# Nuralamsiddik16/Ultrafnd_git

Hardware: AMD Instinct MI355X
Metric: train-step samples/sec (FakeSV batch, seq128+224^2) (higher is better)
Workload: dtype bf16

## Files before the change

### include/ultrafnd_hip.h

```cpp
#ifndef ULTRAFND_HIP_H
#define ULTRAFND_HIP_H

#include <stddef.h>
#include <stdint.h>

#ifdef __cplusplus
extern "C" {
#endif

#define UFND_OK 0
#define UFND_ERR_INVALID 1
#define UFND_ERR_LAUNCH 2

#define UFND_ABI_VERSION 6

const char* ufnd_last_error(void);
int ufnd_abi_version(void);

typedef struct ufnd_step_state {
  uint64_t step;
  uint64_t seed;
  float lr;
  float weight_decay;
  float beta1, beta2, eps;
  float max_norm;
  float grad_scale;
  float loss;
  float grad_norm;
  float clip_coef;
  float bc1, bc2_sqrt;
  uint32_t micro;
  float reserved[2];
} ufnd_step_state;

typedef struct ufnd_dims {
  int hidden;
  int text_dim;
  int audio_dim;
  int visual_dim;
  int temporal_dim;
  int gnn_dim;
  int aux_dim;
  int trees;
  int depth;
  int classes;
  float fusion_dropout;
  float clf_dropout;
  float node_dropout;
} ufnd_dims;

typedef struct ufnd_fusion_params {
  float *text_w, *text_b;
  float *audio_w, *audio_b;
  float *visual_w, *visual_b;
  float *temporal_w, *temporal_b;
  float *gnn_w, *gnn_b;
  float *qkv_w, *qkv_b;
  float *ev0_w[3], *ev0_b[3];
  float *ev2_w[3], *ev2_b[3];
  float *fuse0_w, *fuse0_b;
  float *fuse3_w, *fuse3_b;
  float *cls_w, *cls_b;
} ufnd_fusion_params;

typedef struct ufnd_clf_params {
  float *pre0_w, *pre0_b;
  float *pre3_w, *pre3_b;
  float *gates, *thresh;
  float *leaf, *tau;
  float *bypass_w, *bypass_b;
  float *temperature;
} ufnd_clf_params;

size_t ufnd_fusion_workspace_floats(const ufnd_dims* d, int B);
size_t ufnd_clf_workspace_floats(const ufnd_dims* d, int B);

int ufnd_fusion_forward(const ufnd_dims* d, const ufnd_fusion_params* p, const float* text, const float* audio,
                        const float* visual, const float* temporal, const float* gnn, int B, int train,
                        float* workspace, float* fused, int ld_fused, float* logits, float* forensic,
                        const ufnd_step_state* state, void* stream);

int ufnd_fusion_backward(const ufnd_dims* d, const ufnd_fusion_params* p, const ufnd_fusion_params* g,
                         const float* text, const float* audio, const float* visual, const float* temporal,
                         const float* gnn, int B, int train, float* workspace, const float* d_fused,
                         int ld_dfused, const float* d_logits, const ufnd_step_state* state, void* stream,
                         void* side_stream, int join);

#define UFND_BWD_ALL 0
#define UFND_BWD_FUSE_MLP 1
#define UFND_BWD_REST 2
#define UFND_BWD_NO_LINEAR_GRADS 16
int ufnd_fusion_backward_phase(const ufnd_dims* d, const ufnd_fusion_params* p, const ufnd_fusion_params* g,
                               const float* text, const float* audio, const float* visual, const float* temporal,
                               const float* gnn, int B, int train, float* workspace, const float* d_fused,
                               int ld_dfused, const float* d_logits, const ufnd_step_state* state, void* stream,
                               void* side_stream, int join, int phase);

float* ufnd_clf_input_panel(const ufnd_dims* d, float* clf_workspace, int B, int* ld);
int ufnd_classifier_forward(const ufnd_dims* d, const ufnd_clf_params* p, const float* fused, int ld_fused,
                            const float* aux, int B, int train, float* workspace, float* logits, float* probs,
                            const ufnd_step_state* state, void* stream);
int ufnd_classifier_backward(const ufnd_dims* d, const ufnd_clf_params* p, const ufnd_clf_params* g, int B,
                             int train, float* workspace, const float* d_logits, float* d_fused, int ld_dfused,
                             const ufnd_step_state* state, void* stream, void* side_stream, int join);

int ufnd_classifier_backward_ex(const ufnd_dims* d, const ufnd_clf_params* p, const ufnd_clf_params* g, int B,
                                int train, float* workspace, const float* d_logits, float* d_fused, int ld_dfused,
                                const ufnd_step_state* state, void* stream, void* side_stream, int join, int flags);

size_t ufnd_head_factor_floats(const ufnd_dims* d, int B);
int ufnd_head_pack_factors(const ufnd_dims* d, const float* text, const float* audio, const float* visual, const float* temporal,
                           const float* gnn, int B, float* fusion_workspace, float* clf_workspace, float* pack, void* stream);
int ufnd_head_linear_grads_from_factors(const ufnd_dims* d, const ufnd_fusion_params* fusion_grads, const ufnd_clf_params* clf_grads,
                                        const float* packs, size_t rank_stride, int ranks, int B, void* stream);

typedef struct ufnd_head_io {
  const float *text, *audio, *visual, *temporal, *gnn, *aux;
  const int64_t* labels;
  float *fusion_workspace, *clf_workspace;
  float *logits, *probs, *forensic;
  float* d_logits;
} ufnd_head_io;
int ufnd_head_forward_loss(const ufnd_dims* d, const ufnd_fusion_params* fusion, const ufnd_clf_params* clf, const ufnd_head_io* io, int B,
                           int train, ufnd_step_state* state, void* stream);
int ufnd_head_backward(const ufnd_dims* d, const ufnd_fusion_params* fusion, const ufnd_fusion_params* fusion_grads, const ufnd_clf_params* clf,
                       const ufnd_clf_params* clf_grads, const ufnd_head_io* io, int B, int train, ufnd_step_state* state, void* stream,
                       void* side_stream, int join, int phase);

int ufnd_softmax_ce(const float* logits, const int64_t* labels, int B, float* loss_rows, float* d_logits,
                    ufnd_step_state* state, void* stream);

int ufnd_softmax_ce_weighted(const float* logits, const int64_t* labels, int B, float w0, float w1, float label_smoothing,
                             float* loss_rows, float* d_logits, ufnd_step_state* state, void* stream);

int ufnd_grad_norm(const float* grad, size_t n, float* partials, ufnd_step_state* state, void* stream);
int ufnd_adamw_step(float* param, const float* grad, float* exp_avg, float* exp_avg_sq, size_t n,
                    const ufnd_step_state* state, void* stream);
int ufnd_step_advance(ufnd_step_state* state, void* stream);
int ufnd_clip_adamw_step(float* param, const float* grad, float* exp_avg, float* exp_avg_sq, size_t n, float* partials,
                         ufnd_step_state* state, void* stream);
int ufnd_grad_accumulate(float* dst, const float* src, size_t n, int overwrite, ufnd_step_state* state ,
                         void* stream);

#define UFND_ACT_NONE 0
#define UFND_ACT_GELU 1
#define UFND_ACT_QUICK_GELU 2
#define UFND_ACT_GELU_BWD 3
#define UFND_ACT_QUICK_GELU_BWD 4

int ufnd_cast_bf16(const float* src, void* dst_bf16, size_t n, void* stream);

int ufnd_gemm_bf16(const void* A, const void* W, const float* bias, const float* residual, void* out_bf16,
                   float* out_f32, int M, int N, int K, int lda, int ldw, int ldr, int ldo, int ldf, int act,
                   void* stream);

#define UFND_GEMM_TILE_PERSISTENT 64
int ufnd_gemm_bf16_ex(const void* A, const void* W, const float* bias, const float* residual, void* out_bf16,
                      float* out_f32, int M, int N, int K, int lda, int ldw, int ldr, int ldo, int ldf, int act,
                      int tile_cfg, void* stream);

typedef struct ufnd_gemm_ln {
  const float* a_stats;
  const float* colsum;
  const float* r_stats;
  const float* r_gamma;
  const float* r_beta;
  float* out_stats;
  int a_parts, r_parts;
  float a_eps, r_eps;
  int width;
  int tile_cfg;
  const void* residual_bf16;
  int ldrb;
  float* guard;
} ufnd_gemm_ln;
#define UFND_FOLD_GUARD_SLOTS 1024
int ufnd_gemm_bf16_ln(const void* A, const void* W, const float* bias, const float* residual, void* out_bf16,
                      float* out_f32, int M, int N, int K, int lda, int ldw, int ldr, int ldo, int ldf, int act,
                      const ufnd_gemm_ln* ln, void* stream);
int ufnd_gemm_bf16_stat_parts(int M, int N, int K);

int ufnd_ln_fold_guard(const float* stats, int M, int parts, int width, float eps, float* guard, void* stream);

int ufnd_gemm_bf16_tile_count(void);
int ufnd_gemm_bf16_tile_info(int tile_cfg, int* bm, int* bn, int* ln_aware);

int ufnd_layernorm(const float* x, int ldx, const float* gamma, const float* beta, void* out_bf16, float* out_f32,
                   int M, int H, float eps, void* stream);

int ufnd_attention_bf16(const void* qkv, const int32_t* key_mask, void* ctx, int B, int L, int heads,
                        void* stream);

int ufnd_qkv_attention_bf16(const void* X, const void* Wqkv, const float* bqkv, const int32_t* key_mask, void* ctx, int B, int L,
                            int heads, int ldx, int ldw, const ufnd_gemm_ln* ln, void* stream);

int ufnd_text_pack(const int32_t* mask, int B, int L, int32_t* cu_seqlens, int32_t* row_src, void* stream);
int ufnd_text_pack_bins(const int32_t* mask, int B, int L, int32_t* cu_seqlens, int32_t* row_src, int32_t* bins, int32_t* nbins,
                        void* stream);
int ufnd_bert_embed_live(const int64_t* ids, const int32_t* row_src, const int* m_live, const float* word, const float* pos,
                         const float* type0, const float* gamma, const float* beta, void* x_bf16, float* x_f32, int capacity, int L,
                         int H, int vocab, float eps, void* stream);
int ufnd_gemm_bf16_live(const void* A, const void* W, const float* bias, const float* residual, void* out_bf16, float* out_f32,
                        int M, int N, int K, int lda, int ldw, int ldr, int ldo, int ldf, int act, int tile_cfg, const int* m_live,
                        void* stream);
int ufnd_gemm_bf16_ln_live(const void* A, const void* W, const float* bias, const float* residual, void* out_bf16, float* out_f32,
                           int M, int N, int K, int lda, int ldw, int ldr, int ldo, int ldf, int act, const ufnd_gemm_ln* ln,
                           const int* m_live, void* stream);
int ufnd_qkv_attention_bf16_packed(const void* X, const void* Wqkv, const float* bqkv, const int32_t* key_mask, const int32_t* cu_seqlens,
                                   void* ctx, int B, int L, int heads, int ldx, int ldw, const ufnd_gemm_ln* ln, void* stream);
int ufnd_qkv_attention_bf16_bins(const void* X, const void* Wqkv, const float* bqkv, const int32_t* key_mask, const int32_t* cu_seqlens,
                                 const int32_t* bins, const int32_t* nbins, void* ctx, int B, int L, int heads, int ldx, int ldw,
                                 const ufnd_gemm_ln* ln, void* stream);
int ufnd_attention_bf16_varlen_masked(const void* qkv, const int32_t* cu_seqlens, const int32_t* key_mask, void* ctx, int B, int max_len,
                                      int heads, void* stream);
#define UFND_TEXT_TILE_MAX_B 512
#define UFND_TEXT_TILE_SAMPLES 16
#define UFND_TEXT_TILE_UNITS 24
#define UFND_TEXT_TILE_UNIT0 36
#define UFND_TEXT_TILE_ROWMAP 64
#define UFND_TEXT_TILE_KBIAS 320
#define UFND_TEXT_TILE_INTS 576
int ufnd_text_pack_tiles(const int32_t* mask, int B, int L, int32_t* cu_seqlens, int32_t* row_src, int32_t* tiles, int32_t* ntiles,
                         int32_t* bins, int32_t* nbins, void* stream);
int ufnd_qkv_attention_bf16_tiles(const void* X, const void* Wqkv, const float* bqkv, const int32_t* tiles, const int32_t* ntiles, void* ctx,
                                  int cap_tiles, int heads, int ldx, int ldw, const ufnd_gemm_ln* ln, void* stream);

int ufnd_qkv_attention_bf16_vit(const void* X, const void* Wqkv, const float* bqkv, void* ctx, int N, int T, int heads, int ldx, int ldw,
                                const ufnd_gemm_ln* ln, void* stream);
int ufnd_layernorm_live(const float* x, int ldx, const float* gamma, const float* beta, void* out_bf16, float* out_f32, int capacity,
                        int H, float eps, const int* m_live, void* stream);
int ufnd_masked_meanpool_l2_live(const float* hidden, const int32_t* mask, const int32_t* cu_seqlens, float* out, int B, int L, int H,
                                 void* stream);
int ufnd_ln_masked_meanpool_l2_live(const float* y, const float* gamma, const float* beta, float eps, const int32_t* mask,
                                    const int32_t* cu_seqlens, float* out, int B, int L, int H, void* stream);

int ufnd_bert_embed(const int64_t* ids, const float* word, const float* pos, const float* type0, const float* gamma,
                    const float* beta, void* x_bf16, float* x_f32, int B, int L, int H, int vocab, float eps,
                    void* stream);

int ufnd_masked_meanpool_l2(const float* hidden, const int32_t* mask, float* out, int B, int L, int H,
                            void* stream);

int ufnd_field_mean_l2(const float* parts, const int32_t* valid, float* out, int N, int M, int D, void* stream);

int ufnd_vit_patchify(const float* frames, void* patches_bf16, int N, int image, int patch, void* stream);

int ufnd_vit_assemble(const float* patch_emb, const float* cls, const float* pos, const float* gamma,
                      const float* beta, float* x_f32, void* x_bf16, float* stats, int N, int P, int H, float eps,
                      void* stream);

int ufnd_l2norm_frames(const float* e, float* out, int B, int F, int D, void* stream);

#define UFND_GATHER_MAX_ITEMS 8
typedef struct ufnd_gather_item {
  const void* src;
  void* dst;
  int row_bytes;
  int64_t src_rows;
} ufnd_gather_item;
int ufnd_gather_rows(const int64_t* idx, int B, const ufnd_gather_item* items, int n_items, void* stream);

int ufnd_temporal_weight_ld(int in_dim);
size_t ufnd_temporal_workspace_floats(int B, int in_dim, int hidden);
int ufnd_temporal_align(const float* text, const float* visual, const float* w0, const float* b0, const float* w3,
                        const float* b3, float* workspace, float* out, int B, int in_dim, int vis_dim, int hidden,
                        int out_dim, float dropout_p, const ufnd_step_state* state, void* stream);

typedef struct ufnd_tcn_layer {
  const float *w, *b;
  const float *gamma, *beta;
  float *running_mean, *running_var;
} ufnd_tcn_layer;
int ufnd_tcn_weight_ld(int in_ch, int kernel);
size_t ufnd_tcn_workspace_floats(int B, int T, int in_ch, int hid, int kernel);
int ufnd_tcn_forward(const float* text_seq, int text_dim, const float* vis_seq, int vis_dim, int B, int T,
                     const ufnd_tcn_layer* layers, int n_layers, int kernel, int hid, const float* head_w,
                     const float* head_b, int out_dim, int train, float dropout_p, float momentum, float eps,
                     const ufnd_step_state* state, float* workspace, float* out, void* stream);


int ufnd_ocr_adjacency(const int32_t* offsets, const int32_t* tokens, int N, double thresh, float* adj, int ld, void* stream);

typedef struct ufnd_gcn_params {
  const float* w1;
  const float* b1;
  const float* w2;
  const float* b2;
} ufnd_gcn_params;

size_t ufnd_gcn_workspace_floats(int N, int in_dim, int hid, int out_dim, int train);

int ufnd_gcn_forward(const float* x, const float* adj, int ld_adj, const ufnd_gcn_params* p, float* z, float* workspace, int N,
                     int in_dim, int hid, int out_dim, float dropout_p, const ufnd_step_state* state, void* stream);

int ufnd_gcn_pretrain_step(const float* x, const float* adj, int ld_adj, const ufnd_gcn_params* p, float* exp_avg,
                           float* exp_avg_sq, const float* head_w, const float* head_b, float* z, float* workspace, int N,
                           int in_dim, int hid, int out_dim, float dropout_p, float lr, float weight_decay, int step,
                           const ufnd_step_state* state, float* loss, void* stream);


size_t ufnd_cosine_knn_workspace_floats(int N, int D, int k);

int ufnd_cosine_knn(const float* X, int ldx, int N, int D, int k, int32_t* idx, float* workspace, void* stream);

#define UFND_ADJ_KNN 1
#define UFND_ADJ_OCR 2
#define UFND_ADJ_TEMPORAL 4
int ufnd_dense_adj(const int32_t* idx, int k, const int32_t* offsets, const int32_t* tokens, const float* delay, double alpha,
                   double beta, int N, float* adj, int ld, int flags, void* stream);


int ufnd_ocr_adjacency_weighted(const int32_t* offsets, const int32_t* tokens, int N, double thresh, float* adj, int ld, void* stream);

int ufnd_node_features(const float* text, int ld_text, const float* audio, int ld_audio, const float* visual, int ld_visual,
                       const float* temporal, int ld_temporal, int n_text, int n_audio, int n_visual, int n_temporal, int B,
                       float* out, void* stream);

size_t ufnd_gnn_workspace_floats(int N, int in_dim, int hid, int out_dim);
int ufnd_gnn_forward(const float* x, const float* adj, int ld_adj, const ufnd_gcn_params* p, float* z, float* workspace, int N,
                     int in_dim, int hid, int out_dim, float dropout_p, const ufnd_step_state* state, void* stream);
int ufnd_gnn_backward(const float* x, const ufnd_gcn_params* p, float* g_w1, float* g_b1, float* g_w2, float* g_b2, const float* d_z,
                      float* workspace, int N, int in_dim, int hid, int out_dim, float dropout_p, const ufnd_step_state* state,
                      void* stream);
int ufnd_fusion_feature_grads(const ufnd_dims* d, const ufnd_fusion_params* p, float* workspace, int B, float* d_text, float* d_visual,
                              const ufnd_step_state* state, void* stream);

int ufnd_fusion_gnn_input_grad(const ufnd_dims* d, const ufnd_fusion_params* p, float* workspace, int B, float* d_gnn,
                               const ufnd_step_state* state, void* stream);

int ufnd_fusion_input_grads(const ufnd_dims* d, const ufnd_fusion_params* p, float* workspace, int B, float* d_text, float* d_audio,
                            float* d_visual, float* d_temporal, float* d_gnn, const ufnd_step_state* state, void* stream);

#define UFND_TARGET_LOGIT 0
#define UFND_TARGET_PROB 1
int ufnd_classifier_input_grad(const ufnd_dims* d, const ufnd_clf_params* p, const float* fused, int ld_fused, const float* aux,
                               int B, int train, int target, int class_idx, float* workspace, float* d_x, int ld_dx,
                               float* logits, float* probs, const ufnd_step_state* state, void* stream);

int ufnd_smoothgrad_points(const ufnd_dims* d, const float* x0, int ld_x0, const float* sigma, const float* noise, int ld_noise,
                           int B, int N, int step0, int steps, float* workspace, void* stream);

#define UFND_ATTR_SMOOTHGRAD 0
#define UFND_ATTR_GRAD_X_INPUT 1
#define UFND_ATTR_PATH_MEAN 3
int ufnd_attribution_reduce(int mode, const float* G, int ldg, const float* X, int ldx, int B, int W, int steps, int accumulate,
                            int divisor, float* out, int ldo, float* agg, float* partials, void* stream);

int ufnd_stream_create_cu_mask(const uint32_t* mask_words, int n_words, void** stream_out);
int ufnd_stream_destroy(void* stream);
int ufnd_device_cu_count(void);


int ufnd_gemm_bf16_dgrad(const void* dY, const void* Wt, const float* residual, const void* aux, void* out_bf16, float* out_f32,
                         int M, int N, int K, int lda, int ldw, int ldr, int ldaux, int ldo, int ldf, int act, void* stream);

size_t ufnd_gemm_bf16_wgrad_workspace_floats(int n_out, int k_in, int tokens);
int ufnd_gemm_bf16_wgrad(const void* dYt, const void* Xt, float* dW, int n_out, int k_in, int tokens, int lda, int ldb, int ldw,
                         float* workspace, int accumulate, void* stream);

typedef struct ufnd_partials_job {
  const float* part;
  int nblk, H;
  float *out0, *out1;
} ufnd_partials_job;
#define UFND_PARTIALS_DEFER 2

#define UFND_WGRAD_ALL 0
#define UFND_WGRAD_TRANSPOSE 1
#define UFND_WGRAD_PRODUCT 2
int ufnd_linear_wgrad(const void* dY, int lddy, const void* X, int ldx, int M, int N, int K, float* dW, float* db, void* dYt, void* Xt, int ldt,
                      float* slab_workspace, float* colsum_workspace, const ufnd_partials_job* extra, int part, void* stream);

typedef struct ufnd_refresh_item {
  const void* master;
  void* w;
  void* wt;
  int rows, cols, ld_master, ld_w, ld_wt, tile0;
} ufnd_refresh_item;
int ufnd_refresh_operands(const ufnd_refresh_item* items_device, int n_items, int total_tiles, void* stream);

size_t ufnd_transpose_colsum_workspace_floats(int rows_pad, int cols);
int ufnd_transpose_bf16(const void* src, int src_is_f32, int rows, int cols, int lds, void* dst, int ldd, int rows_pad, float* colsum,
                        float* colsum_ws, int colsum_accumulate, void* stream);

int ufnd_attention_bf16_lse(const void* qkv, const int32_t* key_mask, void* ctx, float* lse, int B, int L, int heads, void* stream);
size_t ufnd_attention_bwd_workspace_floats(int B, int L, int heads);
int ufnd_attention_bf16_bwd(const void* qkv, const void* ctx, const void* dctx, const float* lse, const int32_t* key_mask, void* dqkv,
                            float* workspace, int B, int L, int heads, void* stream);

size_t ufnd_layernorm_bwd_workspace_floats(int M, int H);
int ufnd_layernorm_bwd_blocks(int M);
int ufnd_row_partials_finish(const ufnd_partials_job* job, int accumulate, void* stream);
int ufnd_layernorm_bwd(const float* x, int ldx, const float* gamma, const float* dy, int lddy, const float* add, int ldadd, float* dx_f32,
                       void* dx_bf16, int lddx, float* dgamma, float* dbeta, float* workspace, int accumulate, int M, int H, float eps,
                       void* stream);

int ufnd_act_bf16(const void* x, void* out, size_t n, int act, void* stream);

int ufnd_masked_meanpool_l2_bwd(const float* hidden, const int32_t* mask, const float* dfeat, float* dhidden, int B, int L, int H, void* stream);
int ufnd_l2norm_frames_bwd(const float* e, const float* dfeat, float* de, int B, int F, int D, void* stream);
int ufnd_bert_embed_bwd(const int64_t* ids, const float* ds, float* dword, float* dpos, float* dtype, int B, int L, int H, int vocab,
                        int max_pos, int type_vocab, void* stream);
int ufnd_vit_assemble_bwd(const float* ds, float* dcls, float* dpos, void* dpe_bf16, int N, int P, int H, void* stream);

typedef struct ufnd_dropout {
  const ufnd_step_state* state;
  float p;
  uint32_t tag;
} ufnd_dropout;

#define UFND_LN_BWD_DROP_DXB 1
#define UFND_LN_BWD_DROP_DY 2

int ufnd_attention_bf16_lse_dropout(const void* qkv, const int32_t* key_mask, void* ctx, float* lse, int B, int L, int heads,
                                    const ufnd_dropout* drop, void* stream);
int ufnd_attention_bf16_bwd_dropout(const void* qkv, const void* ctx, const void* dctx, const float* lse, const int32_t* key_mask,
                                    void* dqkv, float* workspace, int B, int L, int heads, const ufnd_dropout* drop, void* stream);
int ufnd_dropout_residual_layernorm(const float* x, int ldx, const float* d, int ldd, const float* gamma, const float* beta, float* y,
                                    void* out_bf16, float* out_f32, int M, int H, float eps, const ufnd_dropout* drop, void* stream);
int ufnd_layernorm_dropout(const float* x, int ldx, const float* gamma, const float* beta, void* out_bf16, float* out_f32, int M, int H,
                           float eps, const ufnd_dropout* drop, void* stream);
int ufnd_layernorm_bwd_dropout(const float* x, int ldx, const float* gamma, const float* dy, int lddy, const float* add, int ldadd,
                               float* dx_f32, void* dx_bf16, int lddx, float* dgamma, float* dbeta, float* workspace, int accumulate,
                               int M, int H, float eps, const ufnd_dropout* drop, int where, void* stream);


#define UFND_PATH_MAX_POINTS 64
int ufnd_path_points(const float* x, const float* base, const float* alphas, int n_points, size_t rows, int width, float* out,
                     void* stream);

int ufnd_token_attribution(const float* g, int ldg, const float* s, int lds, const float* base, int ldb, const int32_t* mask, int R, int H,
                           float* score, float* grad_norm, void* stream);

int ufnd_vit_unpatchify_attribution(const float* dpatches, const float* x, const float* base, float* grad, float* pixels, float* patch_sums,
                                    int N, int image, int patch, void* stream);

#define UFND_AUDIO_MIN_SAMPLES 400
#define UFND_WAVE_CHUNK 4096
#define UFND_CONV0_CHUNK 256

int ufnd_wave_normalize(const float* wave, const int32_t* lengths, float* out, float* ws, int B, int n_max, void* stream);

int ufnd_w2v2_conv0(const float* wave, const int32_t* lengths, const float* w, const float* gamma, const float* beta, void* out_bf16,
                    float* out_f32, float* ws, int B, int n_max, int S1, float eps, void* stream);

int ufnd_conv1d_rows_bf16(const void* A, const void* W, const float* bias, void* out_bf16, float* out_f32, int M, int N, int K, int lda,
                          int ldw, int ldo, int ldf, int act, void* stream);

int ufnd_w2v2_pos_pack(const void* x_bf16, const int32_t* frames, void* packed, int B, int S, void* stream);
int ufnd_w2v2_pos_add(const float* x, const float* conv, const int32_t* frames, float* y, int B, int S, void* stream);

int ufnd_w2v2_frames(const int32_t* lengths, int32_t* frames, int32_t* key_mask, int B, int S, void* stream);

int ufnd_masked_meanpool(const float* hidden, const int32_t* mask, float* out, int B, int L, int H, void* stream);

int ufnd_linear_f32(const float* X, const float* W, const float* bias, float* Y, int M, int N, int K, void* stream);

int ufnd_attention_bf16_causal(const void* qkv, const int32_t* key_mask, void* ctx, int B, int L, int heads, void* stream);
int ufnd_attention_bf16_causal_varlen(const void* qkv, const int32_t* cu_seqlens, const int32_t* key_mask, void* ctx, int B, int max_len,
                                      int heads, void* stream);
int ufnd_clip_text_pack(const int64_t* ids, int B, int L, int eos_token_id, int32_t* e, int32_t* cu_seqlens, int32_t* row_src, void* stream);
int ufnd_clip_text_embed(const int64_t* ids, const float* token_embedding, const float* position_embedding, void* x_bf16, float* x_f32, int B,
                         int L, int H, int vocab, int max_position, void* stream);
int ufnd_clip_text_embed_live(const int64_t* ids, const int32_t* row_src, const int* m_live, const float* token_embedding,
                              const float* position_embedding, void* x_bf16, float* x_f32, int capacity, int L, int H, int vocab,
                              int max_position, void* stream);
int ufnd_clip_text_pool(const float* x, const int32_t* e, const int32_t* cu_seqlens, const float* gamma, const float* beta, void* out_bf16, int B,
                        int L, int H, float eps, void* stream);

int ufnd_semantic_head(const float* text, const float* image, const float* wt, const float* bt, const float* wi, const float* bi,
                       float* workspace, float* out_text, float* out_image, float* out_gap, int B, int D, int K, void* stream);

int ufnd_clip_similarity(const float* text, const float* image, float* similarity, float* conflict, int B, int D, void* stream);

int ufnd_roberta_pack(const int64_t* ids, const int32_t* mask, int B, int L, int pad_token_id, int32_t* cu_seqlens, int32_t* row_src,
                      int32_t* pos_ids, int32_t* valid, void* stream);
int ufnd_roberta_embed(const int64_t* ids, const int32_t* pos_ids, const float* word, const float* pos, const float* type0, const float* gamma,
                       const float* beta, void* x_bf16, float* x_f32, int B, int L, int H, int vocab, int max_position, int pad_token_id, float eps,
                       void* stream);
int ufnd_roberta_embed_live(const int64_t* ids, const int32_t* pos_ids, const int32_t* row_src, const int* m_live, const float* word, const float* pos,
                            const float* type0, const float* gamma, const float* beta, void* x_bf16, float* x_f32, int capacity, int L, int H,
                            int vocab, int max_position, int pad_token_id, float eps, void* stream);
int ufnd_gather_class_rows(const int32_t* cu_seqlens, const void* ctx, void* ctx_out, const void* res_bf16, void* res_bf16_out, const float* res_f32,
                           float* res_f32_out, const float* stats, float* stats_out, int B, int L, int H, int stat_floats, int capacity, void* stream);
int ufnd_emotion_head(const float* x, const float* wd, const float* bd, const float* wo, const float* bo, const int32_t* group,
                      const int32_t* text_valid, const float* arousal, float* workspace, float* logits, float* class_probs, float* probs,
                      float* text_intensity, float* intensity, float* valence, int B, int H, int C, void* stream);
int ufnd_audio_arousal(const float* waves, const int32_t* lengths, float* arousal, int B, int T, void* stream);

#ifdef __cplusplus
}
#endif
#endif
```

### ultrafnd_git_amd/_lib.py

```python
from __future__ import annotations

import ctypes as C
from pathlib import Path
from typing import Optional

import torch

_PKG = Path(__file__).resolve().parent
LIB_PATH = _PKG / "libultrafnd_hip.so"


class UltrafndHipError(RuntimeError):
    pass


class StepState(C.Structure):
    _fields_ = [("step", C.c_uint64), ("seed", C.c_uint64), ("lr", C.c_float), ("weight_decay", C.c_float),
                ("beta1", C.c_float), ("beta2", C.c_float), ("eps", C.c_float), ("max_norm", C.c_float),
                ("grad_scale", C.c_float), ("loss", C.c_float), ("grad_norm", C.c_float), ("clip_coef", C.c_float),
                ("bc1", C.c_float), ("bc2_sqrt", C.c_float), ("micro", C.c_uint32), ("reserved", C.c_float * 2)]


class Dims(C.Structure):
    _fields_ = [("hidden", C.c_int), ("text_dim", C.c_int), ("audio_dim", C.c_int), ("visual_dim", C.c_int),
                ("temporal_dim", C.c_int), ("gnn_dim", C.c_int), ("aux_dim", C.c_int), ("trees", C.c_int),
                ("depth", C.c_int), ("classes", C.c_int), ("fusion_dropout", C.c_float), ("clf_dropout", C.c_float),
                ("node_dropout", C.c_float)]


_FP = C.c_void_p


class FusionParams(C.Structure):
    _fields_ = [(n, _FP) for n in ("text_w", "text_b", "audio_w", "audio_b", "visual_w", "visual_b", "temporal_w",
                                   "temporal_b", "gnn_w", "gnn_b", "qkv_w", "qkv_b")] + \
               [("ev0_w", _FP * 3), ("ev0_b", _FP * 3), ("ev2_w", _FP * 3), ("ev2_b", _FP * 3)] + \
               [(n, _FP) for n in ("fuse0_w", "fuse0_b", "fuse3_w", "fuse3_b", "cls_w", "cls_b")]


class ClfParams(C.Structure):
    _fields_ = [(n, _FP) for n in ("pre0_w", "pre0_b", "pre3_w", "pre3_b", "gates", "thresh", "leaf", "tau",
                                   "bypass_w", "bypass_b", "temperature")]


class GcnParams(C.Structure):
    _fields_ = [(n, _FP) for n in ("w1", "b1", "w2", "b2")]


class GatherItem(C.Structure):
    _fields_ = [("src", _FP), ("dst", _FP), ("row_bytes", C.c_int), ("src_rows", C.c_int64)]


class TcnLayer(C.Structure):
    _fields_ = [(n, _FP) for n in ("w", "b", "gamma", "beta", "running_mean", "running_var")]


class HeadIO(C.Structure):
    _fields_ = [(n, C.c_void_p) for n in ("text", "audio", "visual", "temporal", "gnn", "aux", "labels", "fusion_workspace", "clf_workspace",
                                           "logits", "probs", "forensic", "d_logits")]


class PartialsJob(C.Structure):
    _fields_ = [("part", C.c_void_p), ("nblk", C.c_int), ("H", C.c_int), ("out0", C.c_void_p), ("out1", C.c_void_p)]


class RefreshItem(C.Structure):
    _fields_ = [("master", C.c_void_p), ("w", C.c_void_p), ("wt", C.c_void_p), ("rows", C.c_int), ("cols", C.c_int), ("ld_master", C.c_int),
                ("ld_w", C.c_int), ("ld_wt", C.c_int), ("tile0", C.c_int)]


class Dropout(C.Structure):
    _fields_ = [("state", C.c_void_p), ("p", C.c_float), ("tag", C.c_uint32)]


PARTIALS_DEFER = 2
LN_BWD_DROP_DXB, LN_BWD_DROP_DY = 1, 2
WGRAD_ALL, WGRAD_TRANSPOSE, WGRAD_PRODUCT = 0, 1, 2


class GemmLn(C.Structure):
    _fields_ = [("a_stats", _FP), ("colsum", _FP), ("r_stats", _FP), ("r_gamma", _FP), ("r_beta", _FP), ("out_stats", _FP),
                ("a_parts", C.c_int), ("r_parts", C.c_int), ("a_eps", C.c_float), ("r_eps", C.c_float), ("width", C.c_int),
                ("tile_cfg", C.c_int), ("residual_bf16", _FP), ("ldrb", C.c_int), ("guard", _FP)]

    def __init__(self, *a, **kw):
        super().__init__(*a, **kw)
        if "tile_cfg" not in kw:
            self.tile_cfg = -1


STEP_STATE_BYTES = C.sizeof(StepState)
BWD_ALL, BWD_FUSE_MLP, BWD_REST = 0, 1, 2
TARGET_LOGIT, TARGET_PROB = 0, 1
ATTR_SMOOTHGRAD, ATTR_GRAD_X_INPUT, ATTR_PATH_MEAN = 0, 1, 3
PATH_MAX_POINTS = 64
ATTR_SLICE_ROWS = 32
MAX_ROWS = 65536
BWD_NO_LINEAR_GRADS = 16
ADJ_KNN, ADJ_OCR, ADJ_TEMPORAL = 1, 2, 4
KNN_MAX_K = 64
ABI_VERSION = 6
FOLD_GUARD_SLOTS = 1024
AUDIO_MIN_SAMPLES, WAVE_CHUNK, CONV0_CHUNK = 400, 4096, 256

_lib: Optional[C.CDLL] = None


def _declare(lib: C.CDLL) -> None:
    P, I, S = C.c_void_p, C.c_int, C.c_size_t
    lib.ufnd_last_error.restype = C.c_char_p
    lib.ufnd_abi_version.restype = I
    lib.ufnd_fusion_workspace_floats.restype = S
    lib.ufnd_fusion_workspace_floats.argtypes = [C.POINTER(Dims), I]
    lib.ufnd_clf_workspace_floats.restype = S
    lib.ufnd_clf_workspace_floats.argtypes = [C.POINTER(Dims), I]
    lib.ufnd_clf_input_panel.restype = P
    lib.ufnd_clf_input_panel.argtypes = [C.POINTER(Dims), P, I, C.POINTER(I)]
    lib.ufnd_fusion_forward.argtypes = [C.POINTER(Dims), C.POINTER(FusionParams), P, P, P, P, P, I, I, P, P, I, P, P, P, P]
    lib.ufnd_fusion_backward.argtypes = [C.POINTER(Dims), C.POINTER(FusionParams), C.POINTER(FusionParams),
                                         P, P, P, P, P, I, I, P, P, I, P, P, P, P, I]
    lib.ufnd_fusion_backward_phase.argtypes = [C.POINTER(Dims), C.POINTER(FusionParams), C.POINTER(FusionParams),
                                               P, P, P, P, P, I, I, P, P, I, P, P, P, P, I, I]
    lib.ufnd_fusion_backward_phase.restype = I
    lib.ufnd_classifier_forward.argtypes = [C.POINTER(Dims), C.POINTER(ClfParams), P, I, P, I, I, P, P, P, P, P]
    lib.ufnd_classifier_backward.argtypes = [C.POINTER(Dims), C.POINTER(ClfParams), C.POINTER(ClfParams), I, I, P, P, P,
                                             I, P, P, P, I]
    lib.ufnd_classifier_backward_ex.argtypes = [C.POINTER(Dims), C.POINTER(ClfParams), C.POINTER(ClfParams), I, I, P, P, P,
                                                I, P, P, P, I, I]
    lib.ufnd_classifier_backward_ex.restype = I
    lib.ufnd_head_factor_floats.argtypes = [C.POINTER(Dims), I]
    lib.ufnd_head_factor_floats.restype = S
    lib.ufnd_head_pack_factors.argtypes = [C.POINTER(Dims), P, P, P, P, P, I, P, P, P, P]
    lib.ufnd_head_pack_factors.restype = I
    lib.ufnd_head_linear_grads_from_factors.argtypes = [C.POINTER(Dims), C.POINTER(FusionParams), C.POINTER(ClfParams), P, S, I, I, P]
    lib.ufnd_head_linear_grads_from_factors.restype = I
    lib.ufnd_head_forward_loss.argtypes = [C.POINTER(Dims), C.POINTER(FusionParams), C.POINTER(ClfParams), C.POINTER(HeadIO), I, I, P, P]
    lib.ufnd_head_forward_loss.restype = I
    lib.ufnd_head_backward.argtypes = [C.POINTER(Dims), C.POINTER(FusionParams), C.POINTER(FusionParams), C.POINTER(ClfParams), C.POINTER(ClfParams),
                                       C.POINTER(HeadIO), I, I, P, P, P, I, I]
    lib.ufnd_head_backward.restype = I
    lib.ufnd_softmax_ce.argtypes = [P, P, I, P, P, P, P]
    lib.ufnd_softmax_ce_weighted.argtypes = [P, P, I, C.c_float, C.c_float, C.c_float, P, P, P, P]
    lib.ufnd_softmax_ce_weighted.restype = I
    lib.ufnd_grad_norm.argtypes = [P, S, P, P, P]
    lib.ufnd_adamw_step.argtypes = [P, P, P, P, S, P, P]
    lib.ufnd_step_advance.argtypes = [P, P]
    lib.ufnd_clip_adamw_step.argtypes = [P, P, P, P, S, P, P, P]
    lib.ufnd_clip_adamw_step.restype = I
    lib.ufnd_grad_accumulate.argtypes = [P, P, S, I, P, P]
    lib.ufnd_grad_accumulate.restype = I
    for name in ("ufnd_fusion_forward", "ufnd_fusion_backward", "ufnd_classifier_forward", "ufnd_classifier_backward",
                 "ufnd_softmax_ce", "ufnd_grad_norm", "ufnd_adamw_step", "ufnd_step_advance"):
        getattr(lib, name).restype = I
    _declare_encoders(lib)


def _declare_encoders(lib: C.CDLL) -> None:
    P, I, S, F = C.c_void_p, C.c_int, C.c_size_t, C.c_float
    sigs = {
        "ufnd_cast_bf16": [P, P, S, P],
        "ufnd_gemm_bf16": [P] * 6 + [I] * 9 + [P],
        "ufnd_gemm_bf16_ex": [P] * 6 + [I] * 10 + [P],
        "ufnd_layernorm": [P, I, P, P, P, P, I, I, F, P],
        "ufnd_attention_bf16": [P, P, P, I, I, I, P],
        "ufnd_qkv_attention_bf16": [P, P, P, P, P, I, I, I, I, I, C.POINTER(GemmLn), P],
        "ufnd_bert_embed": [P] * 8 + [I, I, I, I, F, P],
        "ufnd_masked_meanpool_l2": [P, P, P, I, I, I, P],
        "ufnd_text_pack": [P, I, I, P, P, P],
        "ufnd_text_pack_bins": [P, I, I, P, P, P, P, P],
        "ufnd_text_pack_tiles": [P, I, I, P, P, P, P, P, P, P],
        "ufnd_bert_embed_live": [P] * 10 + [I, I, I, I, F, P],
        "ufnd_gemm_bf16_live": [P] * 6 + [I] * 10 + [P, P],
        "ufnd_gemm_bf16_ln_live": [P] * 6 + [I] * 9 + [C.POINTER(GemmLn), P, P],
        "ufnd_qkv_attention_bf16_packed": [P, P, P, P, P, P, I, I, I, I, I, C.POINTER(GemmLn), P],
        "ufnd_qkv_attention_bf16_bins": [P] * 8 + [I, I, I, I, I, C.POINTER(GemmLn), P],
        "ufnd_qkv_attention_bf16_tiles": [P] * 6 + [I, I, I, I, C.POINTER(GemmLn), P],
        "ufnd_qkv_attention_bf16_vit": [P, P, P, P, I, I, I, I, I, C.POINTER(GemmLn), P],
        "ufnd_attention_bf16_varlen_masked": [P, P, P, P, I, I, I, P],
        "ufnd_layernorm_live": [P, I, P, P, P, P, I, I, F, P, P],
        "ufnd_masked_meanpool_l2_live": [P, P, P, P, I, I, I, P],
        "ufnd_ln_masked_meanpool_l2_live": [P, P, P, F, P, P, P, I, I, I, P],
        "ufnd_vit_patchify": [P, P, I, I, I, P],
        "ufnd_vit_assemble": [P] * 8 + [I, I, I, F, P],
        "ufnd_gemm_bf16_ln": [P] * 6 + [I] * 9 + [C.POINTER(GemmLn), P],
        "ufnd_gemm_bf16_stat_parts": [I, I, I],
        "ufnd_ln_fold_guard": [P, I, I, I, F, P, P],
        "ufnd_gemm_bf16_tile_count": [],
        "ufnd_gemm_bf16_tile_info": [I, C.POINTER(I), C.POINTER(I), C.POINTER(I)],
        "ufnd_stream_create_cu_mask": [C.POINTER(C.c_uint32), I, C.POINTER(P)],
        "ufnd_stream_destroy": [P],
        "ufnd_device_cu_count": [],
        "ufnd_l2norm_frames": [P, P, I, I, I, P],
        "ufnd_field_mean_l2": [P, P, P, I, I, I, P],
        "ufnd_temporal_align": [P] * 8 + [I] * 5 + [F, P, P],
    }
    sigs.update({
        "ufnd_gemm_bf16_dgrad": [P] * 6 + [I] * 10 + [P],
        "ufnd_gemm_bf16_wgrad": [P, P, P, I, I, I, I, I, I, P, I, P],
        "ufnd_transpose_bf16": [P, I, I, I, I, P, I, I, P, P, I, P],
        "ufnd_linear_wgrad": [P, I, P, I, I, I, I, P, P, P, P, I, P, P, C.POINTER(PartialsJob), I, P],
        "ufnd_refresh_operands": [P, I, I, P],
        "ufnd_layernorm_bwd_blocks": [I],
        "ufnd_row_partials_finish": [C.POINTER(PartialsJob), I, P],
        "ufnd_attention_bf16_lse": [P, P, P, P, I, I, I, P],
        "ufnd_attention_bf16_bwd": [P, P, P, P, P, P, P, I, I, I, P],
        "ufnd_layernorm_bwd": [P, I, P, P, I, P, I, P, P, I, P, P, P, I, I, I, F, P],
        "ufnd_masked_meanpool_l2_bwd": [P, P, P, P, I, I, I, P],
        "ufnd_l2norm_frames_bwd": [P, P, P, I, I, I, P],
        "ufnd_bert_embed_bwd": [P, P, P, P, P, I, I, I, I, I, I, P],
        "ufnd_vit_assemble_bwd": [P, P, P, P, I, I, I, P],
        "ufnd_act_bf16": [P, P, S, I, P],
        "ufnd_attention_bf16_lse_dropout": [P, P, P, P, I, I, I, C.POINTER(Dropout), P],
        "ufnd_attention_bf16_bwd_dropout": [P, P, P, P, P, P, P, I, I, I, C.POINTER(Dropout), P],
        "ufnd_dropout_residual_layernorm": [P, I, P, I, P, P, P, P, P, I, I, F, C.POINTER(Dropout), P],
        "ufnd_layernorm_dropout": [P, I, P, P, P, P, I, I, F, C.POINTER(Dropout), P],
        "ufnd_layernorm_bwd_dropout": [P, I, P, P, I, P, I, P, P, I, P, P, P, I, I, I, F, C.POINTER(Dropout), I, P],
    })
    sigs.update({
        "ufnd_wave_normalize": [P, P, P, P, I, I, P],
        "ufnd_w2v2_conv0": [P] * 8 + [I, I, I, F, P],
        "ufnd_conv1d_rows_bf16": [P] * 5 + [I] * 8 + [P],
        "ufnd_w2v2_pos_pack": [P, P, P, I, I, P],
        "ufnd_w2v2_pos_add": [P, P, P, P, I, I, P],
        "ufnd_w2v2_frames": [P, P, P, I, I, P],
        "ufnd_masked_meanpool": [P, P, P, I, I, I, P],
        "ufnd_linear_f32": [P, P, P, P, I, I, I, P],
    })
    sigs.update({
        "ufnd_attention_bf16_causal": [P, P, P, I, I, I, P],
        "ufnd_attention_bf16_causal_varlen": [P, P, P, P, I, I, I, P],
        "ufnd_clip_text_pack": [P, I, I, I, P, P, P, P],
        "ufnd_clip_text_embed": [P] * 5 + [I] * 5 + [P],
        "ufnd_clip_text_embed_live": [P] * 7 + [I] * 5 + [P],
        "ufnd_clip_text_pool": [P] * 6 + [I, I, I, F, P],
        "ufnd_semantic_head": [P] * 10 + [I, I, I, P],
        "ufnd_clip_similarity": [P, P, P, P, I, I, P],
    })
    sigs.update({
        "ufnd_roberta_pack": [P, P, I, I, I, P, P, P, P, P],
        "ufnd_roberta_embed": [P] * 9 + [I] * 6 + [F, P],
        "ufnd_roberta_embed_live": [P] * 11 + [I] * 6 + [F, P],
        "ufnd_gather_class_rows": [P] * 9 + [I] * 5 + [P],
        "ufnd_emotion_head": [P] * 15 + [I, I, I, P],
        "ufnd_audio_arousal": [P, P, P, I, I, P],
    })
    for name, argtypes in sigs.items():
        fn = getattr(lib, name)
        fn.argtypes = argtypes
        fn.restype = I
    for name, argtypes in (("ufnd_gemm_bf16_wgrad_workspace_floats", [I, I, I]), ("ufnd_transpose_colsum_workspace_floats", [I, I]),
                           ("ufnd_attention_bwd_workspace_floats", [I, I, I]), ("ufnd_layernorm_bwd_workspace_floats", [I, I])):
        fn = getattr(lib, name)
        fn.argtypes = argtypes
        fn.restype = S
    D = C.c_double
    lib.ufnd_ocr_adjacency.argtypes = [P, P, I, D, P, I, P]
    lib.ufnd_ocr_adjacency.restype = I
    lib.ufnd_gcn_workspace_floats.argtypes = [I, I, I, I, I]
    lib.ufnd_gcn_workspace_floats.restype = S
    lib.ufnd_gcn_forward.argtypes = [P, P, I, C.POINTER(GcnParams), P, P, I, I, I, I, F, P, P]
    lib.ufnd_gcn_forward.restype = I
    lib.ufnd_gcn_pretrain_step.argtypes = [P, P, I, C.POINTER(GcnParams), P, P, P, P, P, P, I, I, I, I, F, F, F, I, P, P, P]
    lib.ufnd_gcn_pretrain_step.restype = I
    lib.ufnd_cosine_knn_workspace_floats.argtypes = [I, I, I]
    lib.ufnd_cosine_knn_workspace_floats.restype = S
    lib.ufnd_cosine_knn.argtypes = [P, I, I, I, I, P, P, P]
    lib.ufnd_cosine_knn.restype = I
    lib.ufnd_dense_adj.argtypes = [P, I, P, P, P, D, D, I, P, I, I, P]
    lib.ufnd_dense_adj.restype = I
    lib.ufnd_ocr_adjacency_weighted.argtypes = [P, P, I, D, P, I, P]
    lib.ufnd_ocr_adjacency_weighted.restype = I
    lib.ufnd_node_features.argtypes = [P, I, P, I, P, I, P, I, I, I, I, I, I, P, P]
    lib.ufnd_node_features.restype = I
    lib.ufnd_gnn_workspace_floats.argtypes = [I, I, I, I]
    lib.ufnd_gnn_workspace_floats.restype = S
    lib.ufnd_gnn_forward.argtypes = [P, P, I, C.POINTER(GcnParams), P, P, I, I, I, I, F, P, P]
    lib.ufnd_gnn_forward.restype = I
    lib.ufnd_gnn_backward.argtypes = [P, C.POINTER(GcnParams), P, P, P, P, P, P, I, I, I, I, F, P, P]
    lib.ufnd_gnn_backward.restype = I
    lib.ufnd_fusion_gnn_input_grad.argtypes = [C.POINTER(Dims), C.POINTER(FusionParams), P, I, P, P, P]
    lib.ufnd_fusion_gnn_input_grad.restype = I
    lib.ufnd_fusion_feature_grads.argtypes = [C.POINTER(Dims), C.POINTER(FusionParams), P, I, P, P, P, P]
    lib.ufnd_fusion_feature_grads.restype = I
    lib.ufnd_fusion_input_grads.argtypes = [C.POINTER(Dims), C.POINTER(FusionParams), P, I, P, P, P, P, P, P, P]
    lib.ufnd_fusion_input_grads.restype = I
    lib.ufnd_classifier_input_grad.argtypes = [C.POINTER(Dims), C.POINTER(ClfParams), P, I, P, I, I, I, I, P, P, I, P, P, P, P]
    lib.ufnd_classifier_input_grad.restype = I
    lib.ufnd_smoothgrad_points.argtypes = [C.POINTER(Dims), P, I, P, P, I, I, I, I, I, P, P]
    lib.ufnd_smoothgrad_points.restype = I
    lib.ufnd_attribution_reduce.argtypes = [I, P, I, P, I, I, I, I, I, I, P, I, P, P, P]
    lib.ufnd_attribution_reduce.restype = I
    lib.ufnd_path_points.argtypes = [P, P, C.POINTER(C.c_float), I, S, I, P, P]
    lib.ufnd_path_points.restype = I
    lib.ufnd_token_attribution.argtypes = [P, I, P, I, P, I, P, I, I, P, P, P]
    lib.ufnd_token_attribution.restype = I
    lib.ufnd_vit_unpatchify_attribution.argtypes = [P, P, P, P, P, P, I, I, I, P]
    lib.ufnd_vit_unpatchify_attribution.restype = I
    lib.ufnd_gather_rows.argtypes = [P, I, C.POINTER(GatherItem), I, P]
    lib.ufnd_gather_rows.restype = I
    lib.ufnd_tcn_weight_ld.argtypes = [I, I]
    lib.ufnd_tcn_weight_ld.restype = I
    lib.ufnd_tcn_workspace_floats.argtypes = [I, I, I, I, I]
    lib.ufnd_tcn_workspace_floats.restype = S
    lib.ufnd_tcn_forward.argtypes = [P, I, P, I, I, I, C.POINTER(TcnLayer), I, I, I, P, P, I, I, F, F, F, P, P, P, P]
    lib.ufnd_tcn_forward.restype = I
    lib.ufnd_temporal_weight_ld.argtypes = [I]
    lib.ufnd_temporal_weight_ld.restype = I
    lib.ufnd_temporal_workspace_floats.argtypes = [I, I, I]
    lib.ufnd_temporal_workspace_floats.restype = S


def lib() -> C.CDLL:
    global _lib
    if _lib is None:
        if not LIB_PATH.exists():
            raise UltrafndHipError(
                f"{LIB_PATH} is missing: run `python -m ultrafnd_git_amd.build` (hipcc, gfx950). "
                "This package has no CPU fallback.")
        l = C.CDLL(str(LIB_PATH))
        _declare(l)
        if l.ufnd_abi_version() != ABI_VERSION:
            raise UltrafndHipError("libultrafnd_hip.so ABI version mismatch; rebuild")
        _lib = l
    return _lib


def check(rc: int, what: str) -> None:
    if rc != 0:
        raise UltrafndHipError(f"{what} failed (code {rc}): {lib().ufnd_last_error().decode()}")


def ptr(t: Optional[torch.Tensor]) -> Optional[int]:
    return None if t is None else t.data_ptr()


def require_hip(*tensors: Optional[torch.Tensor]) -> torch.device:
    dev = None
    for t in tensors:
        if t is None:
            continue
        if t.device.type != "cuda":
            raise UltrafndHipError(
                f"tensor on {t.device}: the fusion hot path runs on a HIP device only (no CPU fallback); "
                "move the module and its inputs to 'cuda'")
        dev = dev or t.device
        if t.device != dev:
            raise UltrafndHipError("all tensors of one call must live on the same device")
    return dev


def stream_ptr(device: torch.device) -> int:
    return torch.cuda.current_stream(device).cuda_stream


def f32c(t: torch.Tensor) -> torch.Tensor:
    if t.dtype != torch.float32:
        t = t.float()
    return t if t.is_contiguous() else t.contiguous()
```

### ultrafnd_git_amd/csrc/diag/gemm_diag.hip

```cpp
#define UFND_DIAG 1
#include "../gemm_bf16_kernel.hpp"
#include "../gemm_bf16_checks.hpp"

extern "C" int ufnd_diag_gemm_bf16_ex(const void* A, const void* W, const float* bias, const float* residual, void* out_bf16,
                                      float* out_f32, int M, int N, int K, int lda, int ldw, int ldr, int ldo, int ldf, int act,
                                      int tile_cfg, void* stream_) {
  UFND_REQUIRE(A && W && (out_bf16 || out_f32), "diag gemm: null operand");
  UFND_REQUIRE(M >= 1 && N >= 64 && K >= 64 && N % 64 == 0 && K % 64 == 0, "diag gemm: M=%d N=%d K=%d", M, N, K);
  GemmArgs a{(const __bf16*)A, (const __bf16*)W, bias, residual, (__bf16*)out_bf16, out_f32, M, N, K, lda, ldw, ldr, ldo, ldf, act, 0, 0, nullptr};
  int mode = 0, cfg = tile_cfg < 0 ? auto_cfg(M, N, K) : tile_cfg;
  if (cfg >= 200) { mode = 2; cfg -= 200; } else if (cfg >= 100) { mode = 1; cfg -= 100; }
  UFND_REQUIRE(cfg < kNumTiles, "diag gemm: unknown tile config %d", cfg);
  UFND_REQUIRE(N % kTiles[cfg].bn == 0, "diag gemm: tile config %d needs N %% %d == 0", cfg, kTiles[cfg].bn);
  int rc = launch_cfg(cfg, mode, a, (hipStream_t)stream_);
  if (rc != UFND_OK) return rc;
  UFND_CHECK_LAUNCH();
  return UFND_OK;
}

extern "C" int ufnd_diag_gemm_bf16_stamps(const void* A, const void* W, void* out_bf16, int M, int N, int K, int tile_cfg,
                                     unsigned long long* stamps, const ufnd_gemm_ln* ln, const float* bias, const float* residual,
                                     float* out_f32, void* stream_) {
  UFND_REQUIRE(A && W && out_bf16 && stamps, "gemm_bf16_stamps: null operand");
  UFND_REQUIRE(M >= 1 && N >= 64 && K >= 64 && N % 64 == 0 && K % 64 == 0, "gemm_bf16_stamps: M=%d N=%d K=%d", M, N, K);
  UFND_REQUIRE(tile_cfg >= 0 && tile_cfg < kNumTiles && N % kTiles[tile_cfg].bn == 0, "gemm_bf16_stamps: tile config %d", tile_cfg);
  GemmArgs a{(const __bf16*)A, (const __bf16*)W, bias, residual, (__bf16*)out_bf16, out_f32, M, N, K, K, K, N, N, N, 0, 0, 0, stamps};
  int abl = 3;
  if (ln) {
    UFND_REQUIRE(kTiles[tile_cfg].lnx, "gemm_bf16_stamps: tile %d has no LayerNorm-aware kernel", tile_cfg);
    a.a_stats = ln->a_stats; a.colsum = ln->colsum; a.r_stats = ln->r_stats; a.r_gamma = ln->r_gamma; a.r_beta = ln->r_beta;
    a.out_stats = ln->out_stats; a.a_parts = ln->a_parts; a.r_parts = ln->r_parts; a.a_eps = ln->a_eps; a.r_eps = ln->r_eps;
    a.inv_h = 1.0f / (float)ln->width;
    a.residual_b = (const __bf16*)ln->residual_bf16;
    a.ldrb = ln->ldrb;
    a.guard = ln->a_stats ? ln->guard : nullptr;
    if (ln->tile_cfg > 0) a.act = ln->tile_cfg;
    abl = 5;
  }
  int rc = launch_cfg(tile_cfg, abl, a, (hipStream_t)stream_);
  if (rc != UFND_OK) return rc;
  UFND_CHECK_LAUNCH();
  return UFND_OK;
}

extern "C" int ufnd_diag_qkv_attention_stamps(const void* X, const void* Wqkv, const float* bqkv, const int32_t* key_mask, void* ctx, int B,
                                              int heads, const ufnd_gemm_ln* ln, unsigned long long* stamps, void* stream_) {
  UFND_REQUIRE(X && Wqkv && ctx && stamps && heads % 2 == 0, "diag qkv_attention: bad argument");
  const int H = heads * 64;
  GemmArgs a{(const __bf16*)X, (const __bf16*)Wqkv, bqkv, nullptr, nullptr, nullptr, B * 128, 3 * H, H, H, H, 0, 0, 0, UFND_ACT_NONE, 0, 0, stamps};
  if (ln && ln->a_stats) {
    a.a_stats = ln->a_stats; a.colsum = ln->colsum; a.a_parts = ln->a_parts; a.a_eps = ln->a_eps;
    a.inv_h = 1.0f / (float)ln->width;
    a.guard = ln->guard;
  }
  a.att_mask = key_mask;
  a.att_ctx = (__bf16*)ctx;
  a.att_h = H;
  a.att_scale_log2e = 0.125f * 1.44269504088896340736f;
  a.m_tiles = B;
  a.n_tiles = heads / 2;
  a.xcd_cols = (a.n_tiles % 2 == 0 && a.m_tiles >= 4) ? 2 : 1;
  hipLaunchKernelGGL((gemm_bf16_kernel<128, 384, 2, 4, 3, 2, 16, 0, 1, 1, 1>), dim3(a.m_tiles * a.n_tiles), dim3(512), 0, (hipStream_t)stream_, a);
  UFND_CHECK_LAUNCH();
  return UFND_OK;
}

extern "C" int ufnd_diag_qkv_attention_tiles_stamps(const void* X, const void* Wqkv, const float* bqkv, const int32_t* tiles, const int32_t* ntiles,
                                                    void* ctx, int cap_tiles, int heads, const ufnd_gemm_ln* ln, unsigned long long* stamps,
                                                    void* stream_) {
  UFND_REQUIRE(X && Wqkv && ctx && stamps && tiles && ntiles && cap_tiles >= 1 && heads >= 1, "diag qkv_attention_tiles: bad argument");
  const int H = heads * 64;
  GemmArgs a{(const __bf16*)X, (const __bf16*)Wqkv, bqkv, nullptr, nullptr, nullptr, cap_tiles * 256, 3 * H, H, H, H, 0, 0, 0, UFND_ACT_NONE, 0, 0, stamps};
  if (ln && ln->a_stats) {
    a.a_stats = ln->a_stats; a.colsum = ln->colsum; a.a_parts = ln->a_parts; a.a_eps = ln->a_eps;
    a.inv_h = 1.0f / (float)ln->width;
    a.guard = ln->guard;
  }
  a.att_bins = tiles;
  a.att_nbins = ntiles;
  a.att_ctx = (__bf16*)ctx;
  a.att_h = H;
  a.att_scale_log2e = 0.125f * 1.44269504088896340736f;
  a.m_tiles = cap_tiles;
  a.n_tiles = heads;
  a.xcd_cols = 1;
  hipLaunchKernelGGL((gemm_bf16_kernel<256, 192, 4, 2, 3, 2, 16, 0, 1, 1, 2>), dim3(a.m_tiles * a.n_tiles), dim3(512), 0, (hipStream_t)stream_, a);
  UFND_CHECK_LAUNCH();
  return UFND_OK;
}

int ufnd_diag_pp_shape_ok(int M, int N, int K);
extern "C" int ufnd_diag_gemm_bf16_plan(int entry, const void* A, const void* W, const float* bias, const float* residual, const void* aux,
                                        const void* out_bf16, const float* out_f32, int M, int N, int K, int lda, int ldw, int ldr, int ldaux,
                                        int ldo, int ldf, int act, int tile_cfg, const ufnd_gemm_ln* ln, int* out) {
  UFND_REQUIRE(out, "gemm_bf16_plan: null result pointer");
  UFND_REQUIRE(entry >= -1 && entry <= 3, "gemm_bf16_plan: entry %d", entry);
  int cfg = tile_cfg, rc = UFND_OK, parts = 0;
  if (entry == -1) {
    UFND_REQUIRE(cfg >= 0 && cfg < kNumTiles, "gemm_bf16_plan: no tile %d", cfg);
    M = N = K = 0;
  } else if (entry == 3) {
    rc = gemm_bf16_dgrad_check_args(A, W, residual, aux, out_bf16, out_f32, M, N, K, lda, ldw, ldr, ldaux, ldo, ldf, act);
    if (rc != UFND_OK) return rc;
    cfg = auto_cfg(M, N, K);
    rc = gemm_bf16_dgrad_check_tile(cfg, N);
    if (rc != UFND_OK) return rc;
  } else {
    if (entry == 2) {
      rc = gemm_bf16_ln_check_args(A, W, bias, residual, out_bf16, out_f32, M, N, K, lda, ldw, ldr, ldo, ldf, act, ln);
      if (rc != UFND_OK) return rc;
      cfg = ln->tile_cfg;
    } else {
      rc = gemm_bf16_check_args(A, W, bias, residual, out_bf16, out_f32, M, N, K, lda, ldw, ldr, ldo, ldf, act);
      if (rc != UFND_OK) return rc;
      if (entry == 0) cfg = -1;
    }
    UFND_REQUIRE(cfg != UFND_GEMM_TILE_PERSISTENT && !(cfg < 0 && ufnd_diag_pp_shape_ok(M, N, K)),
                 "gemm_bf16_plan: the persistent form may take this call (its choice needs the device): not planned here");
    if (cfg < 0) cfg = auto_cfg(M, N, K);
    rc = entry == 2 ? gemm_bf16_ln_check_tile(cfg, M, N, K, ln) : gemm_bf16_check_tile(cfg, N);
    if (rc != UFND_OK) return rc;
    if (entry == 2 && ln->out_stats) parts = stat_parts_for(cfg, N);
  }
  const TileCfg& t = kTiles[cfg];
  const int m_tiles = entry < 0 ? 0 : ufnd_cdiv(M, t.bm), n_tiles = entry < 0 ? 0 : N / t.bn;
  out[0] = cfg;
  out[1] = m_tiles;
  out[2] = n_tiles;
  out[3] = entry < 0 ? 0 : xcd_cols_for(M, N, K, m_tiles, n_tiles);
  out[4] = parts;
  out[5] = t.bm; out[6] = t.bn; out[7] = t.sta; out[8] = t.stb; out[9] = t.lnx; out[10] = t.prod; out[11] = gemm_bwd_tile(cfg) ? 1 : 0;
  return UFND_OK;
}
```

### ultrafnd_git_amd/csrc/gemm_bf16.hip

```cpp
#include "gemm_bf16_kernel.hpp"
#include "gemm_bf16_checks.hpp"

#define UFND_GEMM_TILE_PP UFND_GEMM_TILE_PERSISTENT
int ufnd_pp_pick(const void* gemm_args);
int ufnd_pp_launch(void* gemm_args, void* stream);
int ufnd_pp_stat_parts(int N);

namespace {
__global__ __launch_bounds__(256) void cast_bf16_kernel(const float* src, __bf16* dst, size_t n) {
  for (size_t i = (blockIdx.x * (size_t)256 + threadIdx.x) * 4; i < n; i += (size_t)gridDim.x * 256 * 4) {
    if (i + 4 <= n) {
      const f32x4 v = *reinterpret_cast<const f32x4*>(src + i);
      bf16x4 o = {(__bf16)v[0], (__bf16)v[1], (__bf16)v[2], (__bf16)v[3]};
      *reinterpret_cast<bf16x4*>(dst + i) = o;
    } else {
      for (size_t j = i; j < n; ++j) dst[j] = (__bf16)src[j];
    }
  }
}

}

extern "C" int ufnd_gemm_bf16_live(const void* A, const void* W, const float* bias, const float* residual, void* out_bf16,
                                   float* out_f32, int M, int N, int K, int lda, int ldw, int ldr, int ldo, int ldf, int act,
                                   int tile_cfg, const int* m_live, void* stream_) {
  int rc = gemm_bf16_check_args(A, W, bias, residual, out_bf16, out_f32, M, N, K, lda, ldw, ldr, ldo, ldf, act);
  if (rc != UFND_OK) return rc;
  GemmArgs a{(const __bf16*)A, (const __bf16*)W, bias, residual, (__bf16*)out_bf16, out_f32, M, N, K, lda, ldw, ldr, ldo, ldf, act, 0, 0, nullptr};
  a.m_live = m_live;
  if (tile_cfg == UFND_GEMM_TILE_PP || (tile_cfg < 0 && ufnd_pp_pick(&a))) return ufnd_pp_launch(&a, stream_);
  const int cfg = tile_cfg < 0 ? auto_cfg(M, N, K) : tile_cfg;
  rc = gemm_bf16_check_tile(cfg, N);
  if (rc != UFND_OK) return rc;
  rc = launch_cfg(cfg, 0, a, (hipStream_t)stream_);
  if (rc != UFND_OK) return rc;
  UFND_CHECK_LAUNCH();
  return UFND_OK;
}

extern "C" int ufnd_gemm_bf16_ex(const void* A, const void* W, const float* bias, const float* residual, void* out_bf16,
                                 float* out_f32, int M, int N, int K, int lda, int ldw, int ldr, int ldo, int ldf, int act,
                                 int tile_cfg, void* stream_) {
  return ufnd_gemm_bf16_live(A, W, bias, residual, out_bf16, out_f32, M, N, K, lda, ldw, ldr, ldo, ldf, act, tile_cfg, nullptr, stream_);
}

extern "C" int ufnd_conv1d_rows_bf16(const void* A, const void* W, const float* bias, void* out_bf16, float* out_f32, int M, int N, int K, int lda,
                                     int ldw, int ldo, int ldf, int act, void* stream_) {
  UFND_REQUIRE(A && W && (out_bf16 || out_f32), "conv1d_rows: null operand");
  UFND_REQUIRE(M >= 1 && N >= 64 && K >= 64 && N % 64 == 0 && K % 64 == 0, "conv1d_rows: M=%d N=%d K=%d (need N%%64==0, K%%64==0)", M, N, K);
  UFND_REQUIRE(lda >= 8 && lda % 8 == 0 && ldw % 8 == 0 && ldw >= K && ufnd_aligned(A, 16) && ufnd_aligned(W, 16),
               "conv1d_rows: lda=%d ldw=%d (multiples of 8, ldw >= K) and 16-B aligned pointers", lda, ldw);
  UFND_REQUIRE((long long)M * lda + K < (1ll << 31), "conv1d_rows: M=%d lda=%d K=%d (the A operand must stay below 2^31 elements)", M, lda, K);
  UFND_REQUIRE(!out_f32 || (ldf % 4 == 0 && ldf >= N && ufnd_aligned(out_f32, 16)), "conv1d_rows: out_f32 alignment");
  UFND_REQUIRE(!out_bf16 || (ldo % 8 == 0 && ldo >= N && ufnd_aligned(out_bf16, 16)), "conv1d_rows: out_bf16 alignment");
  UFND_REQUIRE(!bias || ufnd_aligned(bias, 4), "conv1d_rows: bias alignment");
  UFND_REQUIRE(act >= 0 && act <= 2, "conv1d_rows: act=%d", act);
  GemmArgs a{(const __bf16*)A, (const __bf16*)W, bias, nullptr, (__bf16*)out_bf16, out_f32, M, N, K, lda, ldw, 0, ldo, ldf, act, 0, 0, nullptr};
  const int cfg = auto_cfg(M, N, K);
  int rc = gemm_bf16_check_tile(cfg, N);
  if (rc != UFND_OK) return rc;
  rc = launch_cfg(cfg, 0, a, (hipStream_t)stream_);
  if (rc != UFND_OK) return rc;
  UFND_CHECK_LAUNCH();
  return UFND_OK;
}

extern "C" int ufnd_gemm_bf16_tile_info(int tile_cfg, int* bm, int* bn, int* ln_aware) {
  if (tile_cfg < 0 || tile_cfg >= kNumTiles || !kTiles[tile_cfg].built) return 0;
  if (bm) *bm = kTiles[tile_cfg].bm;
  if (bn) *bn = kTiles[tile_cfg].bn;
  if (ln_aware) *ln_aware = kTiles[tile_cfg].lnx;
  return 1;
}
extern "C" int ufnd_gemm_bf16_tile_count(void) { return kNumTiles; }

extern "C" int ufnd_gemm_bf16_stat_parts(int M, int N, int K) {
  static const __bf16 probe[8] = {};
  GemmArgs a{};
  a.A = a.W = probe;
  a.out_bf16 = const_cast<__bf16*>(probe);
  a.residual_b = probe;
  a.out_stats = reinterpret_cast<float*>(const_cast<__bf16*>(probe));
  a.M = M; a.N = N; a.K = K; a.lda = a.ldw = K; a.ldo = a.ldrb = N;
  if (ufnd_pp_pick(&a)) return ufnd_pp_stat_parts(N);
  return stat_parts_for(auto_cfg(M, N, K), N);
}

extern "C" int ufnd_gemm_bf16_ln_live(const void* A, const void* W, const float* bias, const float* residual, void* out_bf16,
                                      float* out_f32, int M, int N, int K, int lda, int ldw, int ldr, int ldo, int ldf, int act,
                                      const ufnd_gemm_ln* ln, const int* m_live, void* stream_) {
  int rc = gemm_bf16_ln_check_args(A, W, bias, residual, out_bf16, out_f32, M, N, K, lda, ldw, ldr, ldo, ldf, act, ln);
  if (rc != UFND_OK) return rc;
  GemmArgs a{(const __bf16*)A, (const __bf16*)W, bias, residual, (__bf16*)out_bf16, out_f32, M, N, K, lda, ldw, ldr, ldo, ldf, act, 0, 0, nullptr};
  a.a_stats = ln->a_stats; a.colsum = ln->colsum; a.r_stats = ln->r_stats; a.r_gamma = ln->r_gamma; a.r_beta = ln->r_beta;
  a.out_stats = ln->out_stats; a.a_parts = ln->a_parts; a.r_parts = ln->r_parts; a.a_eps = ln->a_eps; a.r_eps = ln->r_eps;
  a.inv_h = 1.0f / (float)ln->width;
  a.residual_b = (const __bf16*)ln->residual_bf16;
  a.ldrb = ln->ldrb;
  a.guard = ln->a_stats ? ln->guard : nullptr;
  a.m_live = m_live;
  if (ln->tile_cfg == UFND_GEMM_TILE_PP || (ln->tile_cfg < 0 && ufnd_pp_pick(&a))) return ufnd_pp_launch(&a, stream_);
  const int cfg = ln->tile_cfg < 0 ? auto_cfg(M, N, K) : ln->tile_cfg;
  rc = gemm_bf16_ln_check_tile(cfg, M, N, K, ln);
  if (rc != UFND_OK) return rc;
  rc = launch_cfg(cfg, 4, a, (hipStream_t)stream_);
  if (rc != UFND_OK) return rc;
  UFND_CHECK_LAUNCH();
  return UFND_OK;
}

extern "C" int ufnd_gemm_bf16_ln(const void* A, const void* W, const float* bias, const float* residual, void* out_bf16,
                                 float* out_f32, int M, int N, int K, int lda, int ldw, int ldr, int ldo, int ldf, int act,
                                 const ufnd_gemm_ln* ln, void* stream_) {
  return ufnd_gemm_bf16_ln_live(A, W, bias, residual, out_bf16, out_f32, M, N, K, lda, ldw, ldr, ldo, ldf, act, ln, nullptr, stream_);
}

static int qkv_attention_args(const char* name, GemmArgs& a, const void* X, const void* Wqkv, const float* bqkv, void* ctx, int M, int heads, int ldx,
                              int ldw, const ufnd_gemm_ln* ln) {
  const int H = heads * 64;
  UFND_REQUIRE(ldx % 8 == 0 && ldw % 8 == 0 && ldx >= H && ldw >= H && ufnd_aligned(X, 16) && ufnd_aligned(Wqkv, 16) && ufnd_aligned(ctx, 16),
               "%s: strides must be multiples of 8 and pointers 16-B aligned", name);
  UFND_REQUIRE(!bqkv || ufnd_aligned(bqkv, 16), "%s: bias alignment", name);
  a = GemmArgs{(const __bf16*)X, (const __bf16*)Wqkv, bqkv, nullptr, nullptr, nullptr, M, 3 * H, H, ldx, ldw, 0, 0, 0, UFND_ACT_NONE, 0, 0, nullptr};
  if (ln && ln->a_stats) {
    UFND_REQUIRE(ln->colsum && ufnd_aligned(ln->colsum, 16) && ufnd_aligned(ln->a_stats, 16), "%s: colsum / a_stats alignment", name);
    UFND_REQUIRE(ln->a_parts >= 2 && ln->a_parts <= 24 && ln->a_parts % 2 == 0 && ln->width > 0, "%s: a_parts=%d width=%d", name, ln->a_parts, ln->width);
    a.a_stats = ln->a_stats; a.colsum = ln->colsum; a.a_parts = ln->a_parts; a.a_eps = ln->a_eps;
    a.inv_h = 1.0f / (float)ln->width;
    a.guard = ln->guard;
  }
  a.att_ctx = (__bf16*)ctx;
  a.att_h = H;
  a.att_scale_log2e = 0.125f * 1.44269504088896340736f;
  return UFND_OK;
}

extern "C" int ufnd_qkv_attention_bf16_bins(const void* X, const void* Wqkv, const float* bqkv, const int32_t* key_mask,
                                            const int32_t* cu_seqlens, const int32_t* bins, const int32_t* nbins, void* ctx, int B,
                                            int L, int heads, int ldx, int ldw, const ufnd_gemm_ln* ln, void* stream_) {
  UFND_REQUIRE(X && Wqkv && ctx, "qkv_attention: null operand");
  UFND_REQUIRE(!bins == !nbins && (!bins || cu_seqlens), "qkv_attention: slot bins need cu_seqlens, bins and nbins");
  UFND_REQUIRE(L == 128 && heads >= 2 && heads % 2 == 0 && heads <= 64 && B >= 1 && B <= 16384,
               "qkv_attention: B=%d L=%d heads=%d (this kernel is built for 128-token samples and an even head count; "
               "use ufnd_gemm_bf16[_ln] + ufnd_attention_bf16 otherwise)", B, L, heads);
  GemmArgs a;
  const int rc = qkv_attention_args("qkv_attention", a, X, Wqkv, bqkv, ctx, B * L, heads, ldx, ldw, ln);
  if (rc != UFND_OK) return rc;
  a.att_mask = key_mask;
  a.att_cu = cu_seqlens;
  a.att_bins = bins;
  a.att_nbins = nbins;
  a.m_live = cu_seqlens ? cu_seqlens + B : nullptr;
  a.m_tiles = B;
  a.n_tiles = heads / 2;
  a.xcd_cols = (a.n_tiles % 2 == 0 && a.m_tiles >= 4) ? 2 : 1;
  hipLaunchKernelGGL((gemm_bf16_kernel<128, 384, 2, 4, 3, 2, 16, 0, 0, 1, 1>), dim3(a.m_tiles * a.n_tiles), dim3(512), 0, (hipStream_t)stream_, a);
  UFND_CHECK_LAUNCH();
  return UFND_OK;
}

extern "C" int ufnd_qkv_attention_bf16_packed(const void* X, const void* Wqkv, const float* bqkv, const int32_t* key_mask,
                                              const int32_t* cu_seqlens, void* ctx, int B, int L, int heads, int ldx, int ldw,
                                              const ufnd_gemm_ln* ln, void* stream_) {
  return ufnd_qkv_attention_bf16_bins(X, Wqkv, bqkv, key_mask, cu_seqlens, nullptr, nullptr, ctx, B, L, heads, ldx, ldw, ln, stream_);
}

extern "C" int ufnd_qkv_attention_bf16(const void* X, const void* Wqkv, const float* bqkv, const int32_t* key_mask, void* ctx,
                                       int B, int L, int heads, int ldx, int ldw, const ufnd_gemm_ln* ln, void* stream_) {
  return ufnd_qkv_attention_bf16_packed(X, Wqkv, bqkv, key_mask, nullptr, ctx, B, L, heads, ldx, ldw, ln, stream_);
}

extern "C" int ufnd_qkv_attention_bf16_tiles(const void* X, const void* Wqkv, const float* bqkv, const int32_t* tiles, const int32_t* ntiles,
                                             void* ctx, int cap_tiles, int heads, int ldx, int ldw, const ufnd_gemm_ln* ln, void* stream_) {
  UFND_REQUIRE(X && Wqkv && ctx && tiles && ntiles, "qkv_attention_tiles: null operand");
  UFND_REQUIRE(heads >= 1 && heads <= 64 && cap_tiles >= 1 && cap_tiles <= (UFND_TEXT_TILE_MAX_B + 1) / 2, "qkv_attention_tiles: cap_tiles=%d heads=%d",
               cap_tiles, heads);
  GemmArgs a;
  const int rc = qkv_attention_args("qkv_attention_tiles", a, X, Wqkv, bqkv, ctx, cap_tiles * 256, heads, ldx, ldw, ln);
  if (rc != UFND_OK) return rc;
  a.att_bins = tiles;
  a.att_nbins = ntiles;
  a.m_tiles = cap_tiles;
  a.n_tiles = heads;
  a.xcd_cols = 1;
  hipLaunchKernelGGL((gemm_bf16_kernel<256, 192, 4, 2, 3, 2, 16, 0, 0, 1, 2>), dim3(a.m_tiles * a.n_tiles), dim3(512), 0, (hipStream_t)stream_, a);
  UFND_CHECK_LAUNCH();
  return UFND_OK;
}

extern "C" int ufnd_qkv_attention_bf16_vit(const void* X, const void* Wqkv, const float* bqkv, void* ctx, int N, int T, int heads, int ldx,
                                           int ldw, const ufnd_gemm_ln* ln, void* stream_) {
  UFND_REQUIRE(X && Wqkv && ctx, "qkv_attention_vit: null operand");
  UFND_REQUIRE(T >= 1 && T <= 64, "qkv_attention_vit: T=%d (this kernel is built for samples of 1 to 64 rows; use ufnd_gemm_bf16[_ln] + "
               "ufnd_attention_bf16 otherwise)", T);
  UFND_REQUIRE(heads >= 1 && heads <= 64 && N >= 1 && (long long)N * T <= (1 << 24), "qkv_attention_vit: N=%d T=%d heads=%d", N, T, heads);
  GemmArgs a;
  const int rc = qkv_attention_args("qkv_attention_vit", a, X, Wqkv, bqkv, ctx, N * T, heads, ldx, ldw, ln);
  if (rc != UFND_OK) return rc;
  a.att_t = T;
  a.m_tiles = ufnd_cdiv(N, 256 / T);
  a.n_tiles = heads;
  a.xcd_cols = 1;
  hipLaunchKernelGGL((gemm_bf16_kernel<256, 192, 4, 2, 3, 2, 16, 0, 0, 1, 1>), dim3(a.m_tiles * a.n_tiles), dim3(512), 0, (hipStream_t)stream_, a);
  UFND_CHECK_LAUNCH();
  return UFND_OK;
}

extern "C" int ufnd_gemm_bf16(const void* A, const void* W, const float* bias, const float* residual, void* out_bf16,
                              float* out_f32, int M, int N, int K, int lda, int ldw, int ldr, int ldo, int ldf, int act,
                              void* stream_) {
  return ufnd_gemm_bf16_ex(A, W, bias, residual, out_bf16, out_f32, M, N, K, lda, ldw, ldr, ldo, ldf, act, -1, stream_);
}

extern "C" int ufnd_cast_bf16(const float* src, void* dst, size_t n, void* stream_) {
  UFND_REQUIRE(src && dst && n > 0, "cast_bf16: null argument");
  UFND_REQUIRE(ufnd_aligned(src, 16) && ufnd_aligned(dst, 8), "cast_bf16: alignment");
  size_t want = (n / 4 + 255) / 256;
  const int blocks = (int)(want < 1 ? 1 : (want > 4096 ? 4096 : want));
  hipLaunchKernelGGL(cast_bf16_kernel, dim3(blocks), dim3(256), 0, (hipStream_t)stream_, src, (__bf16*)dst, n);
  UFND_CHECK_LAUNCH();
  return UFND_OK;
}
```

### ultrafnd_git_amd/csrc/gemm_bf16_kernel.hpp

```cpp
#pragma once
#ifndef UFND_GEMM_OUT_NT
#define UFND_GEMM_OUT_NT 0
#endif

#include <type_traits>

#include "common.hpp"
#include "attn_softmax.hpp"

#pragma clang fp contract(off)

#ifndef UFND_GEMM_ILV
#define UFND_GEMM_ILV 1
#endif

namespace {

constexpr int BK = 64;

struct GemmArgs {
  const __bf16* A;
  const __bf16* W;
  const float* bias;
  const float* residual;
  __bf16* out_bf16;
  float* out_f32;
  int M, N, K, lda, ldw, ldr, ldo, ldf, act;
  int m_tiles, n_tiles;
  unsigned long long* stamps;
  const float* a_stats;
  const float* colsum;
  const float* r_stats;
  const float* r_gamma;
  const float* r_beta;
  float* out_stats;
  int a_parts, r_parts;
  float a_eps, r_eps, inv_h;
  const int32_t* att_mask;
  __bf16* att_ctx;
  int att_h;
  int xcd_cols;
  float att_scale_log2e;
  const __bf16* residual_b;
  int ldrb;
  int ksplit;
  size_t slab_stride;
  const __bf16* aux;
  int ldaux;
  float* guard;
  int pp_rows;
  const int* m_live;
  const int32_t* att_cu;
  const int32_t* att_bins;
  const int* att_nbins;
  int att_t;
};

__device__ __forceinline__ void dma16(const void* gsrc, void* lds_dst) {
  __builtin_amdgcn_global_load_lds((const void __attribute__((address_space(1)))*)gsrc,
                                   (void __attribute__((address_space(3)))*)lds_dst, 16, 0, 0);
}

__device__ __forceinline__ float opaque_f(float x) {
  asm volatile("" : "+v"(x));
  return x;
}
__device__ __forceinline__ f32x2 opaque_f2(f32x2 x) {
  asm volatile("" : "+v"(x));
  return x;
}


template <int N>
__device__ __forceinline__ void wait_vmcnt() {
  static_assert(N >= 0 && N <= 63, "vmcnt range");
  asm volatile("s_waitcnt vmcnt(%0)" ::"n"(N) : "memory");
}

template <int V> struct IntC { static constexpr int value = V; };

constexpr int gemm_waves_per_simd(int BM, int BN, int WM, int WN, int STA, int STB, int MI, int LNX, int ATT) {
  const int ring = (STA * BM + STB * BN) * 128, cbytes = WM * WN * MI * (BN / WN + 4) * 4;
  const int smem = (ring > cbytes ? ring : cbytes) + (LNX ? BM * 8 + 64 : 0);
  return (!ATT && smem <= 80 * 1024 ? 2 : 1) * WM * WN / 4;
}
template <int BM, int BN, int WM, int WN, int STA, int STB, int MI, int ABL = 0, int DBG = 0, int LNX = 0, int ATT = 0, int BWD = 0>
__global__ __launch_bounds__(WM * WN * 64) __attribute__((amdgpu_waves_per_eu(gemm_waves_per_simd(BM, BN, WM, WN, STA, STB, MI, LNX, ATT))))
void gemm_bf16_kernel(const GemmArgs a) {
  static_assert(!BWD || (!LNX && !ATT && !ABL && !DBG), "backward forms are plain kernels");
  static_assert(MI == 16 || MI == 32, "MFMA shape");
  static_assert(!ATT || (((BM == 128 && BN == 384 && ATT == 1) || (BM == 256 && BN == 192)) && MI == 16 && WM * WN == 8 && LNX == 1 && ATT <= 2),
                "fused attention tile");
  constexpr bool VIT = ATT == 1 && BM == 256;
  constexpr bool TIL = ATT == 2;
  constexpr bool ONEH = VIT || TIL;
  using acc_t = typename std::conditional<MI == 16, f32x4, f32x16>::type;
  constexpr int AR = MI * MI / 64;
  constexpr int KQ = MI == 16 ? 1 : 2;
  constexpr int NW = WM * WN;
  constexpr int TM = BM / WM, TN = BN / WN;
  constexpr int MT = TM / MI, NT = TN / MI;
  constexpr int ASLOT = BM * 128, BSLOT = BN * 128;
  constexpr int DA = STA - 1, DB = STB - 1;
  constexpr int APIECES = BM / 8, BPIECES = BN / 8;
  constexpr int PWA = APIECES / NW, PWB = (BPIECES + NW - 1) / NW;
  constexpr int WAITN = PWA * (DA - 1 > 0 ? DA - 1 : 0) + PWB * (DB - 1 > 0 ? DB - 1 : 0);
  constexpr int CP = TN + 4;
  constexpr int CBYTES = NW * MI * CP * 4;
  constexpr int RING = STA * ASLOT + STB * BSLOT;
  constexpr int ATT_OFF = (CBYTES + 1023) & ~1023;
  constexpr int ATT_IMG = BM * 128;
  constexpr int ATT_END = ATT ? ATT_OFF + (TIL ? 3 * ATT_IMG + 1024 + 8 * 512 : VIT ? 3 * ATT_IMG + 256 : 6 * ATT_IMG + 2048) : 0;
  constexpr int STAT_OFF0 = (RING > CBYTES) ? RING : CBYTES;
  constexpr int STAT_OFF = STAT_OFF0 > ATT_END ? STAT_OFF0 : ATT_END;
  constexpr int SMEM = STAT_OFF + (LNX ? BM * 8 + 64 : 0);
  static_assert(SMEM <= 160 * 1024, "LDS budget");
  static_assert(APIECES % NW == 0 && TM % MI == 0 && TN % MI == 0, "tile split");
  static_assert(STB >= 2 && (STA == STB || STA == STB + 1), "ring depths");
  static_assert(WAITN <= 63, "vmcnt range");
  __shared__ __attribute__((aligned(16))) char smem[SMEM];

  unsigned long long stamp[10];
  if constexpr (DBG) {
    stamp[0] = __builtin_amdgcn_s_memtime();
    stamp[1] = __builtin_amdgcn_s_memrealtime();
  }

  int mlive = a.M, m_tiles = a.m_tiles;
  if constexpr (!BWD && !ATT) {
    if (a.m_live) {
      const int v = __builtin_amdgcn_readfirstlane(*a.m_live);
      mlive = v < a.M ? (v > 0 ? v : 0) : a.M;
      m_tiles = (mlive + BM - 1) / BM;
      if ((int)blockIdx.x >= m_tiles * a.n_tiles) return;
    }
  }
  if constexpr (ATT) {
    if (a.att_bins) {
      const int v = __builtin_amdgcn_readfirstlane(*a.att_nbins);
      m_tiles = v < a.m_tiles ? (v > 0 ? v : 0) : a.m_tiles;
      if ((int)blockIdx.x >= m_tiles * a.n_tiles) return;
    }
  }
  const int nblk = m_tiles * a.n_tiles;
  int bid, kslice = 0;
  {
    const int ngrid = BWD ? nblk * (a.ksplit > 1 ? a.ksplit : 1) : nblk;
    const int q = ngrid >> 3, r = ngrid & 7, xcd = blockIdx.x & 7, idx = blockIdx.x >> 3;
    bid = (xcd < r ? xcd * (q + 1) : r * (q + 1) + (xcd - r) * q) + idx;
    if constexpr (BWD) {
      kslice = bid / nblk;
      bid -= kslice * nblk;
    }
  }
  int tm = bid / a.n_tiles, tn = bid % a.n_tiles;
  if (a.xcd_cols == 2) {
    const int nh = a.n_tiles >> 1, per_half = m_tiles * nh;
    const int half = bid / per_half, rem = bid - half * per_half;
    tm = rem / nh;
    tn = half * nh + (rem - tm * nh);
  }
  const int m0 = tm * BM, n0 = tn * BN;
  int arow0 = m0, alen = BM;
  int srow[4] = {0, 0, 0, 0}, scnt[4] = {0, 0, 0, 0}, smeta[4] = {-1, -1, -1, -1};
  const bool slots = ATT == 1 && !VIT && a.att_bins != nullptr;
  const int vit_s = VIT ? BM / a.att_t : 0, vit_st = vit_s * a.att_t;
  const int32_t* til = TIL ? a.att_bins + (size_t)tm * UFND_TEXT_TILE_INTS : nullptr;
  int til_rows = 0;
  if constexpr (TIL) til_rows = __builtin_amdgcn_readfirstlane(til[1]);
  if constexpr (VIT) {
    arow0 = tm * vit_st;
    alen = mlive - arow0 < vit_st ? mlive - arow0 : vit_st;
  } else if constexpr (TIL) {
  } else if constexpr (ATT) {
    if (slots) {
      const int32_t* bd = a.att_bins + (size_t)tm * 8;
#pragma unroll
      for (int j = 0; j < 4; ++j) {
        srow[j] = __builtin_amdgcn_readfirstlane(bd[2 * j]);
        smeta[j] = __builtin_amdgcn_readfirstlane(bd[2 * j + 1]);
        const int n = smeta[j] & 255, rest = n - 32 * ((smeta[j] >> 8) & 3);
        scnt[j] = smeta[j] < 0 ? 0 : (rest < 32 ? rest : 32);
      }
#pragma unroll
      for (int j = 1; j < 4; ++j) srow[j] = scnt[j] > 0 ? srow[j] : srow[0];
    } else if (a.att_cu) {
      mlive = __builtin_amdgcn_readfirstlane(*a.m_live);
      arow0 = __builtin_amdgcn_readfirstlane(a.att_cu[tm]);
      alen = __builtin_amdgcn_readfirstlane(a.att_cu[tm + 1]) - arow0;
      if (alen <= 0) return;
    }
  } else {
    alen = mlive - m0;
  }
  auto tile_row = [&](int tr) {
    if constexpr (TIL) return (int)til[UFND_TEXT_TILE_ROWMAP + tr];
    if (slots) {
      const int j = tr >> 5, q = tr & 31;
      const int r0 = j == 0 ? srow[0] : j == 1 ? srow[1] : j == 2 ? srow[2] : srow[3];
      const int c = j == 0 ? scnt[0] : j == 1 ? scnt[1] : j == 2 ? scnt[2] : scnt[3];
      return r0 + (q < c ? q : (c > 0 ? c - 1 : 0));
    }
    const int gr = arow0 + tr;
    return gr < mlive ? gr : mlive - 1;
  };
  auto tile_row_live = [&](int tr) {
    if constexpr (TIL) return tr < til_rows;
    if (slots) {
      const int j = tr >> 5;
      return (tr & 31) < (j == 0 ? scnt[0] : j == 1 ? scnt[1] : j == 2 ? scnt[2] : scnt[3]);
    }
    return tr < alen;
  };
  const int wave = __builtin_amdgcn_readfirstlane(threadIdx.x >> 6), lane = threadIdx.x & 63;
  const int wm = wave / WN, wn = wave % WN, fr = lane & (MI - 1), g = lane / MI;

  acc_t acc[MT][NT];
#pragma unroll
  for (int i = 0; i < MT; ++i)
#pragma unroll
    for (int j = 0; j < NT; ++j)
#pragma unroll
      for (int r = 0; r < AR; ++r) acc[i][j][r] = 0.f;

  int nk = a.K / BK, kbase = 0;
  if constexpr (BWD) {
    if (a.ksplit > 1) {
      const int per = (nk + a.ksplit - 1) / a.ksplit;
      kbase = kslice * per * BK;
      nk = nk - kslice * per < per ? nk - kslice * per : per;
    }
  }
  const int prow = lane >> 3, ppos = lane & 7;
  int arow_att[ATT ? PWA : 1];
  if constexpr (ATT) {
#pragma unroll
    for (int ii = 0; ii < PWA; ++ii) arow_att[ii] = tile_row(8 * (wave + NW * ii) + prow);
  }
  auto issueA = [&](int t, int kt) {
    char* buf = smem + (t % STA) * ASLOT;
    const int k0 = kbase + kt * BK;
#pragma unroll
    for (int ii = 0; ii < PWA; ++ii) {
      const int p = wave + NW * ii;
      const int r = 8 * p + prow;
      const int c = ppos ^ ((r >> 1) & 7);
      int gr = arow0 + r;
      gr = gr < mlive ? gr : mlive - 1;
      if constexpr (ATT) gr = arow_att[ii];
      dma16(a.A + (size_t)gr * a.lda + k0 + c * 8, buf + p * 1024);
    }
  };
  auto issueB = [&](int t, int kt) {
    char* buf = smem + STA * ASLOT + (t % STB) * BSLOT;
    const int k0 = kbase + kt * BK;
#pragma unroll
    for (int ii = 0; ii < PWB; ++ii) {
      int p = wave + NW * ii;
      if constexpr (BPIECES % NW != 0) p = p < BPIECES ? p : p - BPIECES;
      const int r = 8 * p + prow;
      const int c = ppos ^ ((r >> 1) & 7);
      int gr = n0 + r;
      gr = gr < a.N ? gr : a.N - 1;
      if constexpr (ONEH) gr = (r >> 6) * a.att_h + tn * 64 + (r & 63);
      else if constexpr (ATT) gr = (r >> 7) * a.att_h + tn * 128 + (r & 127);
      dma16(a.W + (size_t)gr * a.ldw + k0 + c * 8, buf + p * 1024);
    }
  };
  constexpr int TPR = NW * 64 / BM;
  static_assert(!LNX || TPR == 2 || TPR == 4, "threads per tile row");
  constexpr int GPT = 4 / (TPR < 4 ? TPR : 4);
  f32x4 sv[GPT][3];
  f32x2* st_lds = reinterpret_cast<f32x2*>(smem + STAT_OFF);
  const float* sp = nullptr;
  if constexpr (LNX) {
    sp = a.a_stats ? a.a_stats : a.r_stats;
    if (sp) {
      const int parts = a.a_stats ? a.a_parts : a.r_parts;
      int row = arow0 + (int)threadIdx.x / TPR;
      row = row < mlive ? row : mlive - 1;
      if constexpr (ATT) row = tile_row((int)threadIdx.x / TPR);
      const f32x4* base = reinterpret_cast<const f32x4*>(sp + (size_t)row * parts * 2);
      const int nq = parts >> 1, sub = threadIdx.x % TPR;
#pragma unroll
      for (int gi = 0; gi < GPT; ++gi)
#pragma unroll
        for (int u = 0; u < 3; ++u) {
          const int q = (sub + gi * TPR) + 4 * u;
          asm volatile("global_load_dwordx4 %0, %1, off" : "=v"(sv[gi][u]) : "v"(base + (q < nq ? q : 0)) : "memory");
        }
    }
  }
  float til_kb = 0.0f;
  if constexpr (TIL) {
    if (threadIdx.x < BM) til_kb = __int_as_float(til[UFND_TEXT_TILE_KBIAS + threadIdx.x]);
  }
  int att_mk = 1;
  if constexpr (ATT == 1 && !VIT) {
    if (slots) {
      const int j = (int)threadIdx.x >> 7, k = threadIdx.x & 127;
      const int mt = j == 0 ? smeta[0] : j == 1 ? smeta[1] : j == 2 ? smeta[2] : smeta[3];
      att_mk = mt >= 0 && k < (mt & 255);
      if (att_mk && a.att_mask) att_mk = a.att_mask[(size_t)(mt >> 10) * BM + k];
    } else if (a.att_mask && threadIdx.x < BM) {
      att_mk = a.att_mask[m0 + threadIdx.x];
    }
  }
#pragma unroll
  for (int s = 0; s < STA; ++s) {
    const int ks = s < nk ? s : nk - 1;
    if (s < STB && (LNX || s < nk)) issueB(s, ks);
    if (LNX || s < nk) issueA(s, ks);
  }

  if constexpr (LNX) {
    if (sp) {
      constexpr int NPRO = STA * PWA + STB * PWB;
      static_assert(NPRO <= 63, "vmcnt range");
      if constexpr (GPT == 1)
        asm volatile("s_waitcnt vmcnt(%3) ; STATRETIRE %0 %1 %2" : "+v"(sv[0][0]), "+v"(sv[0][1]), "+v"(sv[0][2]) : "n"(NPRO) : "memory");
      else
        asm volatile("s_waitcnt vmcnt(%6) ; STATRETIRE %0 %1 %2 %3 %4 %5" : "+v"(sv[0][0]), "+v"(sv[0][1]), "+v"(sv[0][2]), "+v"(sv[GPT - 1][0]),
                     "+v"(sv[GPT - 1][1]), "+v"(sv[GPT - 1][2]) : "n"(NPRO) : "memory");
      const int nq_ = (a.a_stats ? a.a_parts : a.r_parts) >> 1, sub_ = threadIdx.x % TPR;
      float gs[GPT], gq[GPT];
#pragma unroll
      for (int gi = 0; gi < GPT; ++gi) {
#pragma unroll
        for (int u = 0; u < 3; ++u) {
          if ((sub_ + gi * TPR) + 4 * u >= nq_) sv[gi][u] = f32x4{0.f, 0.f, 0.f, 0.f};
        }
        gs[gi] = sv[gi][0][0] + sv[gi][0][2];
        gq[gi] = sv[gi][0][1] + sv[gi][0][3];
#pragma unroll
        for (int u = 1; u < 3; ++u) { gs[gi] += sv[gi][u][0] + sv[gi][u][2]; gq[gi] += sv[gi][u][1] + sv[gi][u][3]; }
      }
      float sm, sq;
      if constexpr (TPR == 4) {
        sm = gs[0] + quad_xor1(gs[0]);
        sq = gq[0] + quad_xor1(gq[0]);
        sm += quad_xor2(sm);
        sq += quad_xor2(sq);
      } else {
        const float s01 = gs[0] + quad_xor1(gs[0]), s23 = gs[1] + quad_xor1(gs[1]);
        const float q01 = gq[0] + quad_xor1(gq[0]), q23 = gq[1] + quad_xor1(gq[1]);
        sm = s01 + s23;
        sq = q01 + q23;
      }
      const float mean = __fmul_rn(sm, a.inv_h);
      const float var = fmaxf(__fmaf_rn(-mean, mean, __fmul_rn(sq, a.inv_h)), 0.f);
      const float rstd = __builtin_amdgcn_rsqf(__fadd_rn(var, a.a_stats ? a.a_eps : a.r_eps));
      if (threadIdx.x % TPR == 0) st_lds[threadIdx.x / TPR] = f32x2{mean, rstd};
      if (a.guard && a.a_stats) {
        float ratio = __fmul_rn(fabsf(mean), rstd);
        ratio = ratio == ratio ? ratio : INFINITY;
        const float worst = wave_max(threadIdx.x % TPR == 0 && tile_row_live((int)threadIdx.x / TPR) ? ratio : 0.0f);
        if (lane == 0) reinterpret_cast<float*>(smem + STAT_OFF + BM * 8)[wave] = worst;
      }
      asm volatile("s_waitcnt lgkmcnt(0)" ::: "memory");
    }
  }

  bf16x8 af0[KQ][MT], bf0[KQ][NT], af1[KQ][MT], bf1[KQ][NT];
  auto read_half = [&](int t, auto kk_, bf16x8 (&af)[KQ][MT], bf16x8 (&bfr)[KQ][NT]) {
    constexpr int kk = decltype(kk_)::value;
    const char* At = smem + (t % STA) * ASLOT;
    const char* Bt = smem + STA * ASLOT + (t % STB) * BSLOT;
#pragma unroll
    for (int q = 0; q < KQ; ++q) {
      const int chunk = MI == 16 ? g + 4 * kk : g + 2 * q + 4 * kk;
#pragma unroll
      for (int i = 0; i < MT; ++i) af[q][i] = lds_frag(At, wm * TM + i * MI + fr, chunk);
#pragma unroll
      for (int j = 0; j < NT; ++j) bfr[q][j] = lds_frag(Bt, wn * TN + j * MI + fr, chunk);
    }
  };
  auto mma_half = [&](const bf16x8 (&af)[KQ][MT], const bf16x8 (&bfr)[KQ][NT]) {
#pragma unroll
    for (int q = 0; q < KQ; ++q)
#pragma unroll
      for (int i = 0; i < MT; ++i)
#pragma unroll
        for (int j = 0; j < NT; ++j) {
          if constexpr (MI == 16) acc[i][j] = __builtin_amdgcn_mfma_f32_16x16x32_bf16(af[q][i], bfr[q][j], acc[i][j], 0, 0, 0);
          else acc[i][j] = __builtin_amdgcn_mfma_f32_32x32x16_bf16(af[q][i], bfr[q][j], acc[i][j], 0, 0, 0);
        }
  };
  constexpr int NMF = KQ * MT * NT, NRD = KQ * (MT + NT);
  constexpr bool ILV = UFND_GEMM_ILV != 0;
  auto body = [&](int t, auto ia_, auto ib_, auto next_) {
    constexpr bool IA = decltype(ia_)::value != 0, IB = decltype(ib_)::value != 0, NEXT = decltype(next_)::value != 0;
    if constexpr (ABL != 1) {
      read_half(t, IntC<1>{}, af1, bf1);
      mma_half(af0, bf0);
      if constexpr (ILV) {
#pragma unroll
        for (int q = 0; q < (NRD < NMF ? NRD : NMF - 1); ++q) {
          __builtin_amdgcn_sched_group_barrier(0x008, 1, 0);
          __builtin_amdgcn_sched_group_barrier(0x100, 1, 0);
        }
        __builtin_amdgcn_sched_group_barrier(0x100, NRD - (NRD < NMF ? NRD : NMF - 1), 0);
        __builtin_amdgcn_sched_group_barrier(0x008, NMF - (NRD < NMF ? NRD : NMF - 1), 0);
      } else {
        __builtin_amdgcn_sched_group_barrier(0x008, 1, 0);
        __builtin_amdgcn_sched_group_barrier(0x100, NRD, 0);
        __builtin_amdgcn_sched_group_barrier(0x008, NMF - 1, 0);
      }
    }
    if constexpr (NEXT) {
      __builtin_amdgcn_sched_barrier(0);
      if (t + STA - 1 < nk) wait_vmcnt<WAITN>();
      else wait_vmcnt<0>();
      asm volatile("s_waitcnt lgkmcnt(0)" ::: "memory");
      __builtin_amdgcn_s_barrier();
      __builtin_amdgcn_sched_barrier(0);
      if constexpr (ABL != 1) read_half(t + 1, IntC<0>{}, af0, bf0);
      if constexpr (ABL != 2) {
        if constexpr (IB) issueB(t + STB, t + STB);
        if constexpr (IA) issueA(t + STA, t + STA);
      }
    }
    if constexpr (ABL != 1) {
      mma_half(af1, bf1);
      constexpr int PW = (ABL == 2 || !NEXT) ? 0 : (IA ? PWA : 0) + (IB ? PWB : 0);
      constexpr int GRP = (NMF - 1) / (PW + 1) > 0 ? (NMF - 1) / (PW + 1) : 1;
      if constexpr (ILV && NEXT && NRD + PW < NMF) {
#pragma unroll
        for (int q = 0; q < NRD; ++q) {
          __builtin_amdgcn_sched_group_barrier(0x008, 1, 0);
          __builtin_amdgcn_sched_group_barrier(0x100, 1, 0);
        }
        constexpr int REST = NMF - NRD, G2 = REST / (PW + 1) > 0 ? REST / (PW + 1) : 1;
#pragma unroll
        for (int q = 0; q < PW; ++q) {
          __builtin_amdgcn_sched_group_barrier(0x008, G2, 0);
          __builtin_amdgcn_sched_group_barrier(0x020, 1, 0);
        }
        __builtin_amdgcn_sched_group_barrier(0x008, REST - G2 * PW > 0 ? REST - G2 * PW : 0, 0);
      } else {
        __builtin_amdgcn_sched_group_barrier(0x008, 1, 0);
        if constexpr (NEXT) __builtin_amdgcn_sched_group_barrier(0x100, NRD, 0);
#pragma unroll
        for (int q = 0; q < PW; ++q) {
          __builtin_amdgcn_sched_group_barrier(0x008, GRP, 0);
          __builtin_amdgcn_sched_group_barrier(0x020, 1, 0);
        }
        __builtin_amdgcn_sched_group_barrier(0x008, NMF - 1 - GRP * PW > 0 ? NMF - 1 - GRP * PW : 0, 0);
      }
    }
  };

  if (STA <= nk) wait_vmcnt<PWA * (STA - 1) + PWB * (STB - 1)>();
  else wait_vmcnt<0>();
  __builtin_amdgcn_sched_barrier(0);
  __builtin_amdgcn_s_barrier();
  __builtin_amdgcn_sched_barrier(0);
  if constexpr (DBG) {
    stamp[2] = __builtin_amdgcn_s_memtime();
    stamp[3] = __builtin_amdgcn_s_memrealtime();
  }
  if constexpr (ABL != 1) read_half(0, IntC<0>{}, af0, bf0);
  int t = 0;
  for (; t + STA < nk; ++t) body(t, IntC<1>{}, IntC<1>{}, IntC<1>{});
  for (; t + STB < nk; ++t) body(t, IntC<0>{}, IntC<1>{}, IntC<1>{});
  for (; t + 1 < nk; ++t) body(t, IntC<0>{}, IntC<0>{}, IntC<1>{});
  body(t, IntC<0>{}, IntC<0>{}, IntC<0>{});
  __builtin_amdgcn_sched_barrier(0);
  __builtin_amdgcn_s_barrier();
  __builtin_amdgcn_sched_barrier(0);
  if constexpr (DBG) {
    stamp[4] = __builtin_amdgcn_s_memtime();
    stamp[5] = __builtin_amdgcn_s_memrealtime();
  }

  float bj[NT], csj[NT];
#pragma unroll
  for (int j = 0; j < NT; ++j) { bj[j] = 0.f; csj[j] = 0.f; }
  auto gcol = [&](int c) { return ONEH ? (c >> 6) * a.att_h + tn * 64 + (c & 63) : ATT ? (c >> 7) * a.att_h + tn * 128 + (c & 127) : n0 + c; };
  if (a.bias) {
#pragma unroll
    for (int j = 0; j < NT; ++j) bj[j] = a.bias[gcol(wn * TN + j * MI + fr)];
  }
  bool fold = false, rln = false;
  if constexpr (LNX) {
    fold = a.a_stats != nullptr;
    rln = a.r_stats != nullptr;
    if (fold) {
#pragma unroll
      for (int j = 0; j < NT; ++j) csj[j] = a.colsum[gcol(wn * TN + j * MI + fr)];
    }
  }
  float* cst = reinterpret_cast<float*>(smem) + wave * MI * CP;
  float* const outf = (BWD && a.out_f32) ? a.out_f32 + (size_t)kslice * a.slab_stride : a.out_f32;
  constexpr int CPR = TN / 8;
  constexpr int CHUNKS = MI * CPR;
  constexpr int NIT = (CHUNKS + 63) / 64;
  constexpr bool FIXCOL = (64 % CPR) == 0;
  auto ld8 = [&](const float* ptr, float (&o)[8]) {
    const f32x4 x0 = *reinterpret_cast<const f32x4*>(ptr), x1 = *reinterpret_cast<const f32x4*>(ptr + 4);
#pragma unroll
    for (int q = 0; q < 4; ++q) { o[q] = x0[q]; o[4 + q] = x1[q]; }
  };
  float g8[8], b8[8];
  if constexpr (LNX && FIXCOL) {
    if (rln) {
      const int col = n0 + wn * TN + (lane % CPR) * 8;
      ld8(a.r_gamma + col, g8);
      ld8(a.r_beta + col, b8);
    }
  }
  auto epilogue = [&](auto act_, auto mode_) {
    constexpr int ACT = decltype(act_)::value;
    constexpr bool FOLD = LNX && decltype(mode_)::value == 1, RLN = LNX && decltype(mode_)::value == 2;
    constexpr bool RES = !FOLD;
#pragma unroll
    for (int i = 0; i < MT; ++i) {
      float rr8[RES ? NIT : 1][8];
      if constexpr (RES) if (a.residual && !(BWD && a.aux)) {
#pragma unroll
        for (int it = 0; it < NIT; ++it) {
          const int id = lane + 64 * it;
          if (id < CHUNKS) {
            int row = m0 + wm * TM + i * MI + id / CPR;
            row = row < a.M ? row : a.M - 1;
            ld8(a.residual + (size_t)row * a.ldr + n0 + wn * TN + (id % CPR) * 8, rr8[it]);
          }
        }
      }
      if constexpr (BWD) {
        if (a.aux) {
#pragma unroll
          for (int it = 0; it < NIT; ++it) {
            const int id = lane + 64 * it;
            if (id < CHUNKS) {
              int row = m0 + wm * TM + i * MI + id / CPR;
              row = row < a.M ? row : a.M - 1;
              const bf16x8 xb = *reinterpret_cast<const bf16x8*>(a.aux + (size_t)row * a.ldaux + n0 + wn * TN + (id % CPR) * 8);
#pragma unroll
              for (int q = 0; q < 8; ++q) rr8[it][q] = (float)xb[q];
            }
          }
        }
      }
      if constexpr (LNX && RES) {
        if (a.residual_b) {
#pragma unroll
          for (int it = 0; it < NIT; ++it) {
            const int id = lane + 64 * it;
            if (id < CHUNKS) {
              int row = m0 + wm * TM + i * MI + id / CPR;
              row = row < a.M ? row : a.M - 1;
              const bf16x8 rb = *reinterpret_cast<const bf16x8*>(a.residual_b + (size_t)row * a.ldrb + n0 + wn * TN + (id % CPR) * 8);
#pragma unroll
              for (int q = 0; q < 8; ++q) rr8[it][q] = (float)rb[q];
            }
          }
        }
      }
#pragma unroll
      for (int r = 0; r < AR; r += 2) {
        const int prow_ = MI == 16 ? 4 * g + r : 8 * (r >> 2) + 4 * g + (r & 3);
        f32x2 mean2 = {0.f, 0.f}, rstd2 = {1.f, 1.f};
        if constexpr (FOLD) {
          const f32x2 a0 = st_lds[wm * TM + i * MI + prow_], a1 = st_lds[wm * TM + i * MI + prow_ + 1];
          mean2 = f32x2{a0[0], a1[0]};
          rstd2 = f32x2{a0[1], a1[1]};
        }
#pragma unroll
        for (int j = 0; j < NT; ++j) {
          f32x2 v = {acc[i][j][r], acc[i][j][r + 1]};
          if constexpr (FOLD) v = opaque_f2(rstd2 * __builtin_elementwise_fma(-mean2, f32x2{csj[j], csj[j]}, v));
          v = v + f32x2{bj[j], bj[j]};
          if constexpr (ACT == UFND_ACT_GELU) v = gelu_fast_f2(v);
          else if constexpr (ACT == UFND_ACT_QUICK_GELU) v = quick_gelu_fast_f2(v);
          cst[prow_ * CP + j * MI + fr] = v.x;
          cst[(prow_ + 1) * CP + j * MI + fr] = v.y;
        }
      }
      asm volatile("s_waitcnt lgkmcnt(0)" ::: "memory");
#pragma unroll
      for (int it = 0; it < NIT; ++it) {
        const int id = lane + 64 * it;
        if (id >= CHUNKS) break;
        const int rr = id / CPR, cl = (id % CPR) * 8;
        const int row = m0 + wm * TM + i * MI + rr;
        const int col = n0 + wn * TN + cl;
        const bool live = row < mlive;
        const f32x4 v0 = *reinterpret_cast<const f32x4*>(cst + rr * CP + cl);
        const f32x4 v1 = *reinterpret_cast<const f32x4*>(cst + rr * CP + cl + 4);
        float v[8] = {v0[0], v0[1], v0[2], v0[3], v1[0], v1[1], v1[2], v1[3]};
        if constexpr (BWD) {
          if (a.aux) {
            if (a.act == UFND_ACT_GELU_BWD) {
#pragma unroll
              for (int q = 0; q < 8; ++q) v[q] = v[q] * gelu_grad_f(rr8[it][q]);
            } else {
#pragma unroll
              for (int q = 0; q < 8; ++q) v[q] = v[q] * quick_gelu_grad_f(rr8[it][q]);
            }
          }
        }
        if constexpr (RES) if ((a.residual && !(BWD && a.aux)) || (LNX && a.residual_b)) {
          if constexpr (RLN) {
            const f32x2 ms = st_lds[wm * TM + i * MI + rr];
            if constexpr (!FIXCOL) {
              ld8(a.r_gamma + col, g8);
              ld8(a.r_beta + col, b8);
            }
#pragma unroll
            for (int q = 0; q < 8; ++q) rr8[it][q] = __fmaf_rn(__fmul_rn(__fsub_rn(rr8[it][q], ms[0]), ms[1]), g8[q], b8[q]);
          }
#pragma unroll
          for (int q = 0; q < 8; ++q) v[q] = __fadd_rn(v[q], rr8[it][q]);
        }
        if constexpr (LNX && RES) {
          if (a.out_stats) {
            if constexpr (CPR % 4 == 0) {
              float sm = 0.f, sq = 0.f;
#pragma unroll
              for (int q = 0; q < 8; ++q) { sm = __fadd_rn(sm, v[q]); sq = __fmaf_rn(v[q], v[q], sq); }
              sm += quad_xor1(sm);
              sq += quad_xor1(sq);
              sm += quad_xor2(sm);
              sq += quad_xor2(sq);
              if (live && (id & 3) == 0)
                *reinterpret_cast<f32x2*>(a.out_stats + ((size_t)row * (a.N >> 5) + (col >> 5)) * 2) = f32x2{sm, sq};
            }
          }
        }
        if constexpr (ATT) {
          const int ct = wn * TN + cl;
          const int trow = wm * TM + i * MI + rr, img = ct >> 6, ch = (ct & 63) >> 3;
          bf16x8 o;
#pragma unroll
          for (int q = 0; q < 8; ++q) o[q] = (__bf16)v[q];
          const int sw = img >= (ONEH ? 2 : 4) ? (ch ^ (((trow >> 1) & 3) << 1)) : (ch ^ ((trow >> 1) & 7));
          *reinterpret_cast<bf16x8*>(smem + ATT_OFF + img * ATT_IMG + trow * 128 + (sw << 4)) = o;
          continue;
        }
        if (!live) continue;
        if (a.out_f32) {
          float* op = outf + (size_t)row * a.ldf + col;
          *reinterpret_cast<f32x4*>(op) = f32x4{v[0], v[1], v[2], v[3]};
          *reinterpret_cast<f32x4*>(op + 4) = f32x4{v[4], v[5], v[6], v[7]};
        }
        if (a.out_bf16) {
          bf16x8 o;
#pragma unroll
          for (int q = 0; q < 8; ++q) o[q] = (__bf16)v[q];
          if constexpr (UFND_GEMM_OUT_NT && !BWD) __builtin_nontemporal_store(o, reinterpret_cast<bf16x8*>(a.out_bf16 + (size_t)row * a.ldo + col));
          else *reinterpret_cast<bf16x8*>(a.out_bf16 + (size_t)row * a.ldo + col) = o;
        }
      }
      asm volatile("s_waitcnt lgkmcnt(0)" ::: "memory");
    }
  };
  if constexpr (LNX) {
    if (fold) {
      if (a.act == UFND_ACT_GELU) epilogue(IntC<UFND_ACT_GELU>{}, IntC<1>{});
      else if (a.act == UFND_ACT_QUICK_GELU) epilogue(IntC<UFND_ACT_QUICK_GELU>{}, IntC<1>{});
      else epilogue(IntC<UFND_ACT_NONE>{}, IntC<1>{});
    } else if (rln) {
      epilogue(IntC<UFND_ACT_NONE>{}, IntC<2>{});
    } else {
      epilogue(IntC<UFND_ACT_NONE>{}, IntC<0>{});
    }
  } else {
    if (a.act == UFND_ACT_GELU) epilogue(IntC<UFND_ACT_GELU>{}, IntC<0>{});
    else if (a.act == UFND_ACT_QUICK_GELU) epilogue(IntC<UFND_ACT_QUICK_GELU>{}, IntC<0>{});
    else epilogue(IntC<UFND_ACT_NONE>{}, IntC<0>{});
  }
  if constexpr (ATT && DBG) {
    stamp[8] = __builtin_amdgcn_s_memtime();
    stamp[9] = __builtin_amdgcn_s_memrealtime();
  }
  if constexpr (VIT) {
    const int T = a.att_t;
    float* kbias = reinterpret_cast<float*>(smem + ATT_OFF + 3 * ATT_IMG);
    if (threadIdx.x < 64) kbias[threadIdx.x] = (int)threadIdx.x < T ? 0.0f : -INFINITY;
    __syncthreads();
    const int g4 = lane >> 4, f16 = lane & 15;
    const char* qimg = smem + ATT_OFF;
    const char* kimg = smem + ATT_OFF + ATT_IMG;
    const char* vimg = smem + ATT_OFF + 2 * ATT_IMG;
    const int nqb = (T + 31) >> 5, nsamp = alen > 0 ? alen / T : 0;
    const bool any_masked = __any(kbias[lane] != 0.0f);
    constexpr int KT = 4;
    for (int u = wave; u < nsamp * nqb; u += NW) {
      const int smp = u / nqb, q0 = (u - smp * nqb) * 32, r0 = smp * T;
      const auto row = [&](int k) { return r0 + (k < T ? k : T - 1); };
      bf16x8 qf[2][2];
      attn_q_frags(qimg, [&](int q) { return row(q0 + q); }, f16, g4, qf);
      f32x4 o[4][2], sc[KT][2];
      float m_run[2], l_run[2];
      bf16x8 pf[KT / 2][2];
      attn_init(o, m_run, l_run);
      attn_scores<KT>(kimg, row, qf, f16, g4, sc);
#pragma unroll
      for (int qt = 0; qt < 2; ++qt) attn_softmax_rescale<KT>(sc, qt, kbias, any_masked, g4, a.att_scale_log2e, m_run, l_run, pf, o);
      attn_pv<KT>(vimg, row, pf, o, f16, g4);
#pragma unroll
      for (int qt = 0; qt < 2; ++qt) {
        const float inv = attn_finish(l_run[qt]);
        const int q = q0 + qt * 16 + f16;
        if (q < T) attn_store_ctx(a.att_ctx + (size_t)(arow0 + r0 + q) * a.att_h + tn * 64 + 4 * g4, o, qt, inv);
      }
    }
  } else if constexpr (TIL) {
    constexpr float NEG_MASK = -3.0e38f;
    float* kbias = reinterpret_cast<float*>(smem + ATT_OFF + 3 * ATT_IMG);
    float* wbias = kbias + BM + wave * 128;
    if (threadIdx.x < BM) kbias[threadIdx.x] = til_kb;
    __syncthreads();
    const int g4 = lane >> 4, f16 = lane & 15;
    const char* qimg = smem + ATT_OFF;
    const char* kimg = smem + ATT_OFF + ATT_IMG;
    const char* vimg = smem + ATT_OFF + 2 * ATT_IMG;
    int nunits = __builtin_amdgcn_readfirstlane(til[2]);
    nunits = nunits < UFND_TEXT_TILE_UNITS ? nunits : UFND_TEXT_TILE_UNITS;
    constexpr int KB = 64, KT = KB / 16;
    for (int u = wave; u < nunits; u += NW) {
      const int unit = __builtin_amdgcn_readfirstlane(til[UFND_TEXT_TILE_UNIT0 + u]);
      const int sj = unit & (UFND_TEXT_TILE_SAMPLES - 1), q0 = ((unit >> 8) & 3) * 32;
      const int grow0 = __builtin_amdgcn_readfirstlane(til[4 + 2 * sj]);
      const int meta = __builtin_amdgcn_readfirstlane(til[5 + 2 * sj]);
      const int r0 = (meta >> 8) & 255;
      int n = meta & 255;
      n = n < 1 ? 1 : (n < BM - r0 ? n : BM - r0);
      n = n < 128 ? n : 128;
#pragma unroll
      for (int h = 0; h < 2; ++h) {
        const int k = lane + 64 * h;
        wbias[k] = k < n ? kbias[r0 + k] : NEG_MASK;
      }
      asm volatile("s_waitcnt lgkmcnt(0)" ::: "memory");
      const auto row = [&](int k) { return r0 + (k < n ? k : n - 1); };
      bf16x8 qf[2][2];
      attn_q_frags(qimg, [&](int q) { return row(q0 + q); }, f16, g4, qf);
      f32x4 o[4][2];
      float m_run[2], l_run[2];
      attn_init(o, m_run, l_run);
#pragma unroll
      for (int kb0 = 0; kb0 < 128; kb0 += KB) {
        if (masked_block_is_noop(wbias + kb0, lane, m_run)) continue;
        const auto key_row = [&](int k) { return row(kb0 + k); };
        f32x4 sc[KT][2];
        attn_scores<KT>(kimg, key_row, qf, f16, g4, sc);
        const bool any_masked = __any(wbias[kb0 + lane] != 0.0f);
        bf16x8 pf[KT / 2][2];
#pragma unroll
        for (int qt = 0; qt < 2; ++qt) attn_softmax_rescale<KT>(sc, qt, wbias + kb0, any_masked, g4, a.att_scale_log2e, m_run, l_run, pf, o);
        attn_pv<KT>(vimg, key_row, pf, o, f16, g4);
      }
#pragma unroll
      for (int qt = 0; qt < 2; ++qt) {
        const float inv = attn_finish(l_run[qt]);
        const int q = q0 + qt * 16 + f16;
        if (q < n) attn_store_ctx(a.att_ctx + (size_t)(grow0 + q) * a.att_h + tn * 64 + 4 * g4, o, qt, inv);
      }
    }
  } else if constexpr (ATT) {
    constexpr float NEG_MASK = -3.0e38f;
    float* kbias = reinterpret_cast<float*>(smem + ATT_OFF + 6 * 16384);
    if (slots || threadIdx.x < BM) kbias[threadIdx.x] = att_mk != 0 ? 0.0f : NEG_MASK;
    __syncthreads();
    const int hh = wave >> 2, wq = wave & 3, g4 = lane >> 4, f16 = lane & 15;
    int wrow0 = arow0 + 32 * wq, wcnt = alen - 32 * wq, koff = 0;
    const float* wbias = kbias;
    if (slots) {
      const int mt = wq == 0 ? smeta[0] : wq == 1 ? smeta[1] : wq == 2 ? smeta[2] : smeta[3];
      wrow0 = wq == 0 ? srow[0] : wq == 1 ? srow[1] : wq == 2 ? srow[2] : srow[3];
      wcnt = wq == 0 ? scnt[0] : wq == 1 ? scnt[1] : wq == 2 ? scnt[2] : scnt[3];
      koff = 32 * (wq - ((mt >> 8) & 3));
      wbias = kbias + wq * BM;
    }
    const char* qimg = smem + ATT_OFF + hh * 16384;
    const char* kimg = smem + ATT_OFF + (2 + hh) * 16384;
    const char* vimg = smem + ATT_OFF + (4 + hh) * 16384;
    bf16x8 qf[2][2];
    attn_q_frags(qimg, [&](int q) { return wq * 32 + q; }, f16, g4, qf);
    f32x4 o[4][2];
    float m_run[2], l_run[2];
    attn_init(o, m_run, l_run);
    constexpr int KB = 64, KT = KB / 16;
    if (wcnt > 0) {
#pragma unroll
      for (int kb0 = 0; kb0 < BM; kb0 += KB) {
        if (masked_block_is_noop(wbias + kb0, lane, m_run)) continue;
        const int kr0 = koff + kb0;
        const auto key_row = [&](int k) { return (kr0 + k) & (BM - 1); };
        f32x4 sc[KT][2];
        attn_scores<KT>(kimg, key_row, qf, f16, g4, sc);
        const bool any_masked = __any(wbias[kb0 + lane] != 0.0f);
        bf16x8 pf[KT / 2][2];
#pragma unroll
        for (int qt = 0; qt < 2; ++qt) attn_softmax_rescale<KT>(sc, qt, wbias + kb0, any_masked, g4, a.att_scale_log2e, m_run, l_run, pf, o);
        attn_pv<KT>(vimg, key_row, pf, o, f16, g4);
      }
    }
#pragma unroll
    for (int qt = 0; qt < 2; ++qt) {
      const float inv = attn_finish(l_run[qt]);
      const int q = qt * 16 + f16;
      if (q < wcnt) attn_store_ctx(a.att_ctx + (size_t)(wrow0 + q) * a.att_h + (tn * 2 + hh) * 64 + 4 * g4, o, qt, inv);
    }
  }
  if constexpr (LNX) {
    if (a.guard && a.a_stats && threadIdx.x == 0) {
      const float* gw = reinterpret_cast<const float*>(smem + STAT_OFF + BM * 8);
      float worst = gw[0];
#pragma unroll
      for (int w = 1; w < NW; ++w) worst = fmaxf(worst, gw[w]);
      atomicMax(reinterpret_cast<int*>(a.guard + (blockIdx.x & 1023)), __float_as_int(worst));
    }
  }
  if constexpr (DBG) {
    asm volatile("s_waitcnt vmcnt(0)" ::: "memory");
    stamp[6] = __builtin_amdgcn_s_memtime();
    stamp[7] = __builtin_amdgcn_s_memrealtime();
    if (threadIdx.x == 0) {
      constexpr int NS = ATT ? 10 : 8;
#pragma unroll
      for (int i = 0; i < NS; ++i) a.stamps[(size_t)blockIdx.x * NS + i] = stamp[i];
    }
  }
}

}

#define UFND_GEMM_TILES(X)                                                                             \
  X(0, 128, 128, 2, 2, 3, 3, 16, 0, 0)                                                              \
  X(1, 128, 64, 2, 2, 3, 3, 16, 0, 0)                                                 \
  X(2, 256, 128, 4, 2, 3, 3, 16, 1, 1)                                                              \
  X(3, 128, 128, 2, 2, 2, 2, 16, 1, 0)                                                \
  X(4, 128, 64, 2, 2, 4, 4, 16, 0, 0)                                                               \
  X(5, 256, 64, 4, 2, 3, 3, 16, 0, 0)                                                               \
  X(6, 128, 288, 2, 2, 3, 3, 16, 0, 0)                                   \
  X(7, 128, 96, 2, 2, 3, 3, 16, 0, 0)                                     \
  X(8, 256, 192, 4, 2, 2, 2, 16, 1, 1)                                  \
  X(9, 128, 384, 2, 2, 2, 2, 16, 0, 0)                                                              \
  X(10, 128, 192, 2, 2, 3, 3, 16, 0, 0)                                                             \
  X(11, 128, 96, 2, 2, 4, 4, 16, 0, 0)                                                              \
  X(12, 64, 96, 1, 2, 4, 4, 16, 0, 0)                     \
  X(13, 64, 192, 1, 2, 3, 3, 16, 0, 0)                                                              \
  X(14, 128, 256, 2, 2, 2, 2, 16, 0, 0)                                                             \
  X(15, 256, 256, 4, 2, 2, 2, 16, 1, 1)                                                             \
  X(16, 128, 128, 4, 2, 3, 3, 16, 1, 1)                                  \
  X(17, 128, 192, 4, 2, 3, 3, 16, 1, 1)                                  \
  X(18, 256, 64, 4, 2, 4, 4, 16, 0, 0)                                                              \
  X(19, 64, 64, 1, 2, 4, 4, 16, 0, 0)                                                 \
  X(20, 128, 64, 4, 2, 4, 4, 16, 1, 1)                                   \
  X(21, 256, 192, 2, 4, 2, 2, 16, 0, 0)                                          \
  X(22, 256, 192, 4, 2, 3, 2, 16, 1, 1)                                 \
  X(23, 256, 256, 4, 2, 3, 2, 16, 0, 0)                                                             \
  X(24, 128, 192, 4, 2, 4, 4, 16, 0, 0)                                                             \
  X(25, 128, 256, 4, 2, 3, 3, 16, 0, 0)                                 \
  X(26, 256, 192, 4, 2, 2, 2, 32, 0, 0)   \
  X(27, 128, 128, 4, 2, 3, 3, 32, 0, 0)                                                                    \
  X(28, 256, 144, 8, 1, 2, 2, 16, 1, 1)   \
  X(29, 128, 128, 4, 2, 2, 2, 16, 1, 0)

#ifdef UFND_DIAG
#define UFND_TILE_BUILT(PROD_) 1
#else
#define UFND_TILE_BUILT(PROD_) (PROD_)
#endif

struct TileCfg { int bm, bn, threads, wn, lnx, built, sta, stb, prod; };
static const TileCfg kTiles[] = {
#define X(id, BM_, BN_, WM_, WN_, SA_, SB_, MI_, LN_, PROD_) {BM_, BN_, WM_ * WN_ * 64, WN_, LN_, UFND_TILE_BUILT(PROD_), SA_, SB_, PROD_},
    UFND_GEMM_TILES(X)
#undef X
};
constexpr int kNumTiles = sizeof(kTiles) / sizeof(kTiles[0]);
constexpr bool gemm_bwd_tile(int id) { return id == 15 || id == 16 || id == 17 || id == 20 || id == 22; }

static int xcd_cols_for(int M, int N, int K, int m_tiles, int n_tiles) {
#ifdef UFND_DIAG
  static const int forced = [] { const char* e = getenv("UFND_GEMM_XCD_COLS"); return e ? atoi(e) : 0; }();
  if (forced == 1) return 1;
  if (forced == 2) return (n_tiles % 2 == 0) ? 2 : 1;
#endif
  (void)K;
  return (4LL * N > (long long)M && n_tiles % 2 == 0 && m_tiles >= 4) ? 2 : 1;
}

static int launch_cfg(int cfg, int mode, GemmArgs& a, hipStream_t stream) {
  if (cfg < 0 || cfg >= kNumTiles || !kTiles[cfg].built) {
    ufnd_set_error("gemm_bf16: tile config %d is not part of this library", cfg);
    return UFND_ERR_INVALID;
  }
  const TileCfg& t = kTiles[cfg];
  a.m_tiles = ufnd_cdiv(a.M, t.bm);
  a.n_tiles = a.N / t.bn;
  a.xcd_cols = xcd_cols_for(a.M, a.N, a.K, a.m_tiles, a.n_tiles);
  const dim3 grid(a.m_tiles * a.n_tiles * (mode == 6 && a.ksplit > 1 ? a.ksplit : 1)), block(t.threads);
#ifdef UFND_GEMM_ONLY_BWD
#define X(id, BM_, BN_, WM_, WN_, SA_, SB_, MI_, LN_, PROD_)                                                                      \
  case id:                                                                                                                        \
    if constexpr (gemm_bwd_tile(id)) {                                                                                            \
      hipLaunchKernelGGL((gemm_bf16_kernel<BM_, BN_, WM_, WN_, SA_, SB_, MI_, 0, 0, 0, 0, 1>), grid, block, 0, stream, a);        \
    } else {                                                                                                                      \
      ufnd_set_error("gemm_bf16 backward: tile %d has no backward kernel", id);                                                   \
      return UFND_ERR_INVALID;                                                                                                    \
    }                                                                                                                             \
    break;
  (void)mode;
  switch (cfg) {
    UFND_GEMM_TILES(X)
    default: ufnd_set_error("gemm_bf16: unknown tile config %d", cfg); return UFND_ERR_INVALID;
  }
#undef X
  return UFND_OK;
#else
#ifdef UFND_DIAG
#define UFND_DIAG_LAUNCH(BM_, BN_, WM_, WN_, SA_, SB_, MI_)                                                                             \
  else if (mode == 5) hipLaunchKernelGGL((gemm_bf16_kernel<BM_, BN_, WM_, WN_, SA_, SB_, MI_, 0, 1, 1>), grid, block, 0, stream, a);   \
  else if (mode == 1) hipLaunchKernelGGL((gemm_bf16_kernel<BM_, BN_, WM_, WN_, SA_, SB_, MI_, 1, 0>), grid, block, 0, stream, a);      \
  else if (mode == 2) hipLaunchKernelGGL((gemm_bf16_kernel<BM_, BN_, WM_, WN_, SA_, SB_, MI_, 2, 0>), grid, block, 0, stream, a);      \
  else if (mode == 3) hipLaunchKernelGGL((gemm_bf16_kernel<BM_, BN_, WM_, WN_, SA_, SB_, MI_, 0, 1>), grid, block, 0, stream, a);
#else
#define UFND_DIAG_LAUNCH(BM_, BN_, WM_, WN_, SA_, SB_, MI_)
#endif
#define X(id, BM_, BN_, WM_, WN_, SA_, SB_, MI_, LN_, PROD_)                                                        \
  case id:                                                                                                          \
    if constexpr (UFND_TILE_BUILT(PROD_) != 0) {                                                                    \
      if (mode == 0) {                                                                                              \
        hipLaunchKernelGGL((gemm_bf16_kernel<BM_, BN_, WM_, WN_, SA_, SB_, MI_, 0, 0>), grid, block, 0, stream, a); \
      } else if constexpr (LN_ != 0) {    \
        if (mode == 4) hipLaunchKernelGGL((gemm_bf16_kernel<BM_, BN_, WM_, WN_, SA_, SB_, MI_, 0, 0, 1>), grid, block, 0, stream, a); \
        UFND_DIAG_LAUNCH(BM_, BN_, WM_, WN_, SA_, SB_, MI_)                                                         \
        else {                                                                                                      \
          ufnd_set_error("gemm_bf16: tile %d has no kernel for mode %d in this library", id, mode);                 \
          return UFND_ERR_INVALID;                                                                                  \
        }                                                                                                           \
      } else {                                                                                                      \
        ufnd_set_error("gemm_bf16: tile %d has no diagnostics / LayerNorm-aware build", id);                        \
        return UFND_ERR_INVALID;                                                                                    \
      }                                                                                                             \
    }                                                                                                               \
    break;
  switch (cfg) {
    UFND_GEMM_TILES(X)
    default: ufnd_set_error("gemm_bf16: unknown tile config %d", cfg); return UFND_ERR_INVALID;
  }
#undef X
#undef UFND_DIAG_LAUNCH
  return UFND_OK;
#endif
}

static int auto_cfg(int M, int N, int K) {
#ifdef UFND_DIAG
  static const int forced = [] { const char* e = getenv("UFND_GEMM_FORCE_CFG"); return e ? atoi(e) : -1; }();
  if (forced >= 0 && forced < kNumTiles && N % kTiles[forced].bn == 0) return forced;
#endif
  auto tiles = [&](int cfg) { return (long long)ufnd_cdiv(M, kTiles[cfg].bm) * (N / kTiles[cfg].bn); };
  if (N % 256 == 0 && N >= 3072 && tiles(15) >= 512) return 15;
  if (N % 256 == 0 && N >= 2048 && tiles(15) >= 190 && tiles(15) <= 256) return 15;
  if (N % 192 == 0 && tiles(22) >= 160) return 22;
  if (N >= 2048) {
    if (N % 192 == 0 && N >= 3072) return 17;
    if (N % 128 == 0) return 16;
  }
  if (N < 2048 && N % 192 == 0 && tiles(17) >= 150 && tiles(17) <= 256) return 17;
  if (N % 128 == 0 && tiles(16) >= 150) return 16;
  return 20;
}
```

### ultrafnd_git_amd/encoders.py

```python
from __future__ import annotations

import ctypes
import warnings
from collections import OrderedDict
from typing import Dict, Optional, Tuple

import torch
import torch.nn as nn

from . import _lib as L

ACT_NONE, ACT_GELU, ACT_QUICK_GELU = 0, 1, 2


def _bf16(t: torch.Tensor) -> torch.Tensor:
    t = t.contiguous()
    out = torch.empty(t.shape, dtype=torch.bfloat16, device=t.device)
    L.check(L.lib().ufnd_cast_bf16(t.data_ptr(), out.data_ptr(), t.numel(), L.stream_ptr(t.device)), "ufnd_cast_bf16")
    return out


def dropout_prob(name: str, p) -> float:
    p = float(p)
    if not 0.0 <= p < 1.0:
        raise ValueError(f"{name}={p!r}: a dropout probability in [0, 1)")
    return p


def text_slot_bins(n_rows) -> list:
    cls = {c: [b for b, n in enumerate(n_rows) if (int(n) + 31) // 32 == c] for c in (1, 2, 3, 4)}
    one, two, three = cls[1], cls[2], cls[3]
    p = min(len(one), len(three))
    ones = one[p:]
    u = min(2, len(ones)) if len(two) % 2 else 0
    slots = lambda *bs: [(b, s) for b in bs for s in range((int(n_rows[b]) + 31) // 32)]
    full = [slots(b) for b in cls[4]] + [slots(three[k], one[k]) for k in range(p)]
    full += [slots(two[k], two[k + 1]) for k in range(0, len(two) - 1, 2)]
    odd = slots(two[-1], *ones[:u]) if len(two) % 2 else None
    rest = ones[u:]
    if odd is not None and u == 2:
        full.append(odd)
    full += [slots(*rest[k:k + 4]) for k in range(0, len(rest) - len(rest) % 4, 4)]
    part = [slots(b) for b in three[p:]]
    if odd is not None and u < 2:
        part.append(odd)
    if len(rest) % 4:
        part.append(slots(*rest[len(rest) - len(rest) % 4:]))
    return [x + [None] * (4 - len(x)) for x in full + part]


def text_slot_bin_count(n_rows) -> int:
    return len(text_slot_bins(n_rows))


TEXT_TILE_ROWS, TEXT_TILE_SAMPLES, TEXT_TILE_MAX_B = 256, 16, 512
TEXT_TILE_INTS, TEXT_TILE_UNIT0, TEXT_TILE_ROWMAP, TEXT_TILE_KBIAS = 576, 36, 64, 320


def text_tiles(n_rows) -> list:
    tiles, used = [], []
    for b in sorted((b for b, n in enumerate(n_rows) if int(n) > 0), key=lambda b: (-int(n_rows[b]), b)):
        n = int(n_rows[b])
        if n > 128:
            raise ValueError(f"text_tiles: n_b={n} (samples of at most 128 rows)")
        for t, u in enumerate(used):
            if u + n <= TEXT_TILE_ROWS and len(tiles[t]) < TEXT_TILE_SAMPLES:
                break
        else:
            t = len(tiles)
            tiles.append([])
            used.append(0)
        tiles[t].append((b, used[t]))
        used[t] += n
    return tiles


def text_tile_count(n_rows) -> int:
    return len(text_tiles(n_rows))


class _EncoderBase(nn.Module):

    FOLD_GUARD_MAX = 4.0

    def __init__(self, hidden: int, heads: int, fold_ln: bool, residual_dtype: str):
        super().__init__()
        if residual_dtype not in ("fp32", "bf16"):
            raise ValueError(f"residual_dtype={residual_dtype!r}: 'fp32' or 'bf16'")
        if hidden != heads * 64:
            raise ValueError("head_dim must be 64 (hidden == heads * 64)")
        self.hidden, self.heads, self.fold_ln, self.residual_dtype = hidden, heads, fold_ln, residual_dtype
        self.tiles: Dict[str, int] = {}
        self._guard: Optional[torch.Tensor] = None
        self._w: "OrderedDict[str, torch.Tensor]" = OrderedDict()
        self._packed: Optional[dict] = None
        self._layer_keys: Dict[int, dict] = {}
        self._bufs: Dict[Tuple, dict] = {}
        self.weights_version = 0

    @staticmethod
    def _seeded_init():
        g = torch.Generator().manual_seed(0)

        def init(shape, std=0.02):
            return torch.randn(shape, generator=g) * std
        return init

    LAYER_PREFIX: str
    LAYER_NAMES: Dict[str, list]

    def layer_keys(self, i: int) -> Dict[str, list]:
        k = self._layer_keys.get(i)
        if k is None:
            P = self.LAYER_PREFIX.format(i)
            k = self._layer_keys[i] = {name: [P + sfx for sfx in sfxs] for name, sfxs in self.LAYER_NAMES.items()}
        return k

    def _pack_layers(self, extra=None) -> list:
        w, layers = self._w, []
        for i in range(self.layers):
            k = self.layer_keys(i)
            wq = torch.cat([w[n] for n in k["qkv_w"]], 0)
            layers.append({"wqkv": _bf16(wq), "bqkv": torch.cat([w[n] for n in k["qkv_b"]], 0).contiguous(),
                           "wo": _bf16(w[k["o_w"][0]]), "bo": w[k["o_b"][0]], "g1": w[k["g1"][0]], "b1": w[k["b1n"][0]],
                           "w1": _bf16(w[k["w1"][0]]), "bi": w[k["b1"][0]], "w2": _bf16(w[k["w2"][0]]), "b2": w[k["b2"][0]],
                           "g2": w[k["g2"][0]], "b2n": w[k["b2n"][0]]})
            if extra is not None:
                extra(layers, wq, w[k["w1"][0]])
        return layers

    def state_dict(self, *args, **kwargs):
        return OrderedDict((k, v.detach().clone()) for k, v in self._w.items())

    def load_state_dict(self, sd, strict: bool = True):
        missing = [k for k in self._w if k not in sd]
        unexpected = [k for k in sd if k not in self._w]
        if strict and missing:
            raise RuntimeError(f"missing keys: {missing[:5]}{'...' if len(missing) > 5 else ''}")
        for k in self._w:
            if k in sd:
                if tuple(sd[k].shape) != tuple(self._w[k].shape):
                    raise RuntimeError(f"shape mismatch for {k}: {tuple(sd[k].shape)} vs {tuple(self._w[k].shape)}")
                self._w[k].copy_(sd[k].to(self._w[k].device, torch.float32))
        self._packed = None
        self.weights_version += 1
        return missing, unexpected

    def _apply(self, fn, recurse=True):
        super()._apply(fn, recurse)
        for k in self._w:
            self._w[k] = fn(self._w[k]).float()
        self._packed = None
        self._bufs.clear()
        self.weights_version += 1
        return self

    @property
    def device(self) -> torch.device:
        return next(iter(self._w.values())).device

    def _require_hip(self):
        if self.device.type != "cuda":
            raise L.UltrafndHipError(f"{type(self).__name__} runs on a HIP device only: call .to('cuda') (no CPU fallback)")

    def _strict(self, run):
        rd, self.residual_dtype = self.residual_dtype, "fp32"
        try:
            if self.fold_ln:
                out = run()
                if not self.check_fold():
                    return out
            return run()
        finally:
            self.residual_dtype = rd

    def _fold_parts(self, M: int) -> int:
        p1 = L.lib().ufnd_gemm_bf16_stat_parts(M, self.hidden, self.hidden)
        p2 = L.lib().ufnd_gemm_bf16_stat_parts(M, self.hidden, self.inter)
        return p1 if (self.fold_ln and p1 > 0 and p1 == p2 and p1 % 2 == 0) else 0

    def _gemm(self, A, W, bias, out_bf16=None, out_f32=None, residual=None, act=ACT_NONE, which=None, m_live=None):
        M = A.shape[0]
        N, K = W.shape
        L.check(L.lib().ufnd_gemm_bf16_live(A.data_ptr(), W.data_ptr(), L.ptr(bias), L.ptr(residual), L.ptr(out_bf16),
                                            L.ptr(out_f32), M, N, K, A.stride(0), W.stride(0),
                                            residual.stride(0) if residual is not None else 0,
                                            out_bf16.stride(0) if out_bf16 is not None else 0,
                                            out_f32.stride(0) if out_f32 is not None else 0, act, self.tiles.get(which, -1),
                                            m_live, L.stream_ptr(A.device)), "ufnd_gemm_bf16_live")

    def _gemm_ln(self, A, W, bias, out_bf16=None, out_f32=None, residual=None, act=ACT_NONE, a_stats=None, colsum=None,
                 r_stats=None, r_gamma=None, r_beta=None, out_stats=None, eps=1e-5, which=None, residual_bf16=None, m_live=None):
        M = A.shape[0]
        N, K = W.shape
        ln = L.GemmLn()
        ln.a_stats, ln.colsum = L.ptr(a_stats), L.ptr(colsum)
        ln.r_stats, ln.r_gamma, ln.r_beta = L.ptr(r_stats), L.ptr(r_gamma), L.ptr(r_beta)
        ln.out_stats = L.ptr(out_stats)
        ln.a_parts = a_stats.shape[1] if a_stats is not None else 0
        ln.r_parts = r_stats.shape[1] if r_stats is not None else 0
        ln.a_eps = ln.r_eps = eps
        ln.width = self.hidden
        ln.tile_cfg = self.tiles.get(which, -1)
        if residual_bf16 is not None:
            ln.residual_bf16, ln.ldrb = residual_bf16.data_ptr(), residual_bf16.stride(0)
        if a_stats is not None:
            ln.guard = self._guard_buf(A.device).data_ptr()
        L.check(L.lib().ufnd_gemm_bf16_ln_live(A.data_ptr(), W.data_ptr(), L.ptr(bias), L.ptr(residual), L.ptr(out_bf16),
                                               L.ptr(out_f32), M, N, K, A.stride(0), W.stride(0),
                                               residual.stride(0) if residual is not None else 0,
                                               out_bf16.stride(0) if out_bf16 is not None else 0,
                                               out_f32.stride(0) if out_f32 is not None else 0, act, ctypes.byref(ln),
                                               m_live, L.stream_ptr(A.device)), "ufnd_gemm_bf16_ln_live")

    def _guard_buf(self, dev) -> torch.Tensor:
        if self._guard is None or self._guard.device != dev:
            self._guard = torch.zeros(L.FOLD_GUARD_SLOTS, dtype=torch.float32, device=dev)
        return self._guard

    def fold_ratio(self) -> float:
        return 0.0 if self._guard is None else float(self._guard.max().cpu())

    def check_fold(self, reset: bool = True, ratio: Optional[float] = None) -> bool:
        r = self.fold_ratio() if ratio is None else float(ratio)
        if reset and self._guard is not None:
            self._guard.zero_()
        if self.fold_ln and r > self.FOLD_GUARD_MAX:
            warnings.warn(f"{type(self).__name__}: a residual-stream row with |mean|/std = {r:.1f} (> {self.FOLD_GUARD_MAX}) went through a "
                          "folded LayerNorm; switching to materialised LayerNorms (fold_ln=False)")
            self.fold_ln = False
            self._bufs.clear()
            return True
        return False

    @staticmethod
    def _fold(W, b, gamma, beta):
        Wp = _bf16(W * gamma[None, :])
        return Wp, Wp.float().sum(1).contiguous(), (b + (W * beta[None, :]).sum(1)).contiguous()

    def _ln(self, x, ldx, gamma, beta, out_bf16, out_f32, M, H, eps, m_live=None):
        if m_live is not None:
            L.check(L.lib().ufnd_layernorm_live(x.data_ptr(), ldx, gamma.data_ptr(), beta.data_ptr(), L.ptr(out_bf16),
                                                L.ptr(out_f32), M, H, eps, m_live, L.stream_ptr(x.device)), "ufnd_layernorm_live")
            return
        L.check(L.lib().ufnd_layernorm(x.data_ptr(), ldx, gamma.data_ptr(), beta.data_ptr(), L.ptr(out_bf16),
                                       L.ptr(out_f32), M, H, eps, L.stream_ptr(x.device)), "ufnd_layernorm")

    def _qkv_attn(self, A, W, bias, mask_i32, ctx, B, Lq, heads, a_stats=None, colsum=None, eps=1e-5, cu=None, bins=None, nbins=None, tiles=None,
                  ntiles=None):
        ln = None
        if a_stats is not None:
            ln = L.GemmLn()
            ln.a_stats, ln.colsum, ln.a_parts, ln.a_eps, ln.r_eps, ln.width = a_stats.data_ptr(), colsum.data_ptr(), a_stats.shape[1], eps, eps, self.hidden
            ln.guard = self._guard_buf(A.device).data_ptr()
        if Lq <= 64:
            if mask_i32 is not None or cu is not None or bins is not None:
                raise L.UltrafndHipError("_qkv_attn: the short-sample kernel (Lq <= 64) takes no key mask, cu or bins")
            L.check(L.lib().ufnd_qkv_attention_bf16_vit(A.data_ptr(), W.data_ptr(), L.ptr(bias), ctx.data_ptr(), B, Lq, heads, A.stride(0),
                                                        W.stride(0), ctypes.byref(ln) if ln is not None else None, L.stream_ptr(A.device)),
                    "ufnd_qkv_attention_bf16_vit")
            return
        if tiles is not None:
            L.check(L.lib().ufnd_qkv_attention_bf16_tiles(A.data_ptr(), W.data_ptr(), L.ptr(bias), tiles.data_ptr(), ntiles.data_ptr(), ctx.data_ptr(),
                                                          tiles.shape[0], heads, A.stride(0), W.stride(0),
                                                          ctypes.byref(ln) if ln is not None else None, L.stream_ptr(A.device)),
                    "ufnd_qkv_attention_bf16_tiles")
            return
        L.check(L.lib().ufnd_qkv_attention_bf16_bins(A.data_ptr(), W.data_ptr(), L.ptr(bias), L.ptr(mask_i32), L.ptr(cu), L.ptr(bins),
                                                     L.ptr(nbins), ctx.data_ptr(), B, Lq, heads, A.stride(0), W.stride(0),
                                                     ctypes.byref(ln) if ln is not None else None, L.stream_ptr(A.device)),
                "ufnd_qkv_attention_bf16_bins")

    def _two_launch(self, b, entry: str, operands: tuple, B: int, Lq: int, live=None):
        fn = getattr(L.lib(), entry)
        call = (b["qkv"].data_ptr(), *(L.ptr(t) for t in operands), b["ctx"].data_ptr(), B, Lq, self.heads, L.stream_ptr(self.device))

        def attend(A, W, bias, a_stats=None, colsum=None):
            if a_stats is None:
                self._gemm(A, W, bias, out_bf16=b["qkv"], which="qkv", m_live=live)
            else:
                self._gemm_ln(A, W, bias, out_bf16=b["qkv"], a_stats=a_stats, colsum=colsum, eps=self.eps, which="qkv", m_live=live)
            L.check(fn(*call), entry)
        return attend

    def _post_ln_layers(self, layers, b, attend, M: int, live=None, tail=None) -> None:
        H, eps = self.hidden, self.eps
        for i, ly in enumerate(layers):
            attend(b["xb"], ly["wqkv"], ly["bqkv"])
            r, res = b, b["xf"]
            if tail is not None and i == len(layers) - 1:
                r = tail(None, b["xf"], None)
                res, M, live = r["rf"], r["y"].shape[0], None
            self._gemm(r["ctx"], ly["wo"], ly["bo"], out_f32=r["y"], residual=res, which="out", m_live=live)
            self._ln(r["y"], H, ly["g1"], ly["b1"], r["x1b"], r["x1f"], M, H, eps, m_live=live)
            self._gemm(r["x1b"], ly["w1"], ly["bi"], out_bf16=r["h"], act=ACT_GELU, which="ffn1", m_live=live)
            self._gemm(r["h"], ly["w2"], ly["b2"], out_f32=r["y"], residual=r["x1f"], which="ffn2", m_live=live)
            self._ln(r["y"], H, ly["g2"], ly["b2n"], r["xb"], r["xf"], M, H, eps, m_live=live)

    def _pre_ln_blocks(self, layers, b, attend, M: int, act: int, live=None, tail=None) -> None:
        H, eps = self.hidden, self.eps
        for i, ly in enumerate(layers):
            self._ln(b["xf"], H, ly["g1"], ly["b1"], b["hb"], None, M, H, eps, m_live=live)
            attend(b["hb"], ly["wqkv"], ly["bqkv"])
            r = tail() if (tail is not None and i == len(layers) - 1) else b
            xf = r["xf"]
            self._gemm(r["ctx"], ly["wo"], ly["bo"], out_f32=xf, residual=xf, which="out", m_live=live)
            self._ln(xf, xf.stride(0), ly["g2"], ly["b2n"], r["hb"], None, xf.shape[0], H, eps, m_live=live)
            self._gemm(r["hb"], ly["w1"], ly["bi"], out_bf16=r["m"], act=act, which="ffn1", m_live=live)
            self._gemm(r["m"], ly["w2"], ly["b2"], out_f32=xf, residual=xf, which="ffn2", m_live=live)


def _live_ptr(cu: torch.Tensor) -> int:
    return cu.data_ptr() + 4 * (cu.numel() - 1)


_CLIP_LAYER = {"qkv_w": [f"self_attn.{n}.weight" for n in ("q_proj", "k_proj", "v_proj")],
               "qkv_b": [f"self_attn.{n}.bias" for n in ("q_proj", "k_proj", "v_proj")],
               "o_w": ["self_attn.out_proj.weight"], "o_b": ["self_attn.out_proj.bias"], "g1": ["layer_norm1.weight"], "b1n": ["layer_norm1.bias"],
               "w1": ["mlp.fc1.weight"], "b1": ["mlp.fc1.bias"], "w2": ["mlp.fc2.weight"], "b2": ["mlp.fc2.bias"],
               "g2": ["layer_norm2.weight"], "b2n": ["layer_norm2.bias"]}


class BertTextEncoder(_EncoderBase):
    LAYER_PREFIX = "encoder.layer.{}."
    LAYER_NAMES = {"qkv_w": [f"attention.self.{n}.weight" for n in ("query", "key", "value")],
                   "qkv_b": [f"attention.self.{n}.bias" for n in ("query", "key", "value")],
                   "o_w": ["attention.output.dense.weight"], "o_b": ["attention.output.dense.bias"],
                   "g1": ["attention.output.LayerNorm.weight"], "b1n": ["attention.output.LayerNorm.bias"],
                   "w1": ["intermediate.dense.weight"], "b1": ["intermediate.dense.bias"], "w2": ["output.dense.weight"], "b2": ["output.dense.bias"],
                   "g2": ["output.LayerNorm.weight"], "b2n": ["output.LayerNorm.bias"]}

    def __init__(self, layers: int = 12, hidden: int = 768, heads: int = 12, intermediate: int = 3072,
                 vocab_size: int = 30522, max_position: int = 512, type_vocab: int = 2, eps: float = 1e-12,
                 fold_ln: bool = True, residual_dtype: str = "bf16", hidden_dropout_prob: float = 0.0,
                 attention_probs_dropout_prob: float = 0.0):
        super().__init__(hidden, heads, fold_ln, residual_dtype)
        self.hidden_dropout_prob = dropout_prob("hidden_dropout_prob", hidden_dropout_prob)
        self.attention_probs_dropout_prob = dropout_prob("attention_probs_dropout_prob", attention_probs_dropout_prob)
        self.fuse_qkv_attention = True
        self.text_sample_tiles = True
        self.text_tile_min_grid = 257
        self.layers, self.inter, self.vocab, self.eps = layers, intermediate, vocab_size, eps
        self.max_position = max_position
        w, init = self._w, self._seeded_init()
        w["embeddings.word_embeddings.weight"] = init((vocab_size, hidden))
        w["embeddings.position_embeddings.weight"] = init((max_position, hidden))
        w["embeddings.token_type_embeddings.weight"] = init((type_vocab, hidden))
        w["embeddings.LayerNorm.weight"] = torch.ones(hidden)
        w["embeddings.LayerNorm.bias"] = torch.zeros(hidden)
        for i in range(layers):
            P = f"encoder.layer.{i}."
            for n in ("query", "key", "value"):
                w[P + f"attention.self.{n}.weight"] = init((hidden, hidden))
                w[P + f"attention.self.{n}.bias"] = torch.zeros(hidden)
            w[P + "attention.output.dense.weight"] = init((hidden, hidden))
            w[P + "attention.output.dense.bias"] = torch.zeros(hidden)
            w[P + "attention.output.LayerNorm.weight"] = torch.ones(hidden)
            w[P + "attention.output.LayerNorm.bias"] = torch.zeros(hidden)
            w[P + "intermediate.dense.weight"] = init((intermediate, hidden))
            w[P + "intermediate.dense.bias"] = torch.zeros(intermediate)
            w[P + "output.dense.weight"] = init((hidden, intermediate))
            w[P + "output.dense.bias"] = torch.zeros(hidden)
            w[P + "output.LayerNorm.weight"] = torch.ones(hidden)
            w[P + "output.LayerNorm.bias"] = torch.zeros(hidden)

    def _fold_layer(self, layers, wq, w1) -> None:
        ly = layers[-1]
        ly["w1f"], ly["cs1"], ly["bif"] = self._fold(w1, ly["bi"], ly["g1"], ly["b1"])
        if len(layers) > 1:
            prev = layers[-2]
            ly["wqkvf"], ly["csqkv"], ly["bqkvf"] = self._fold(wq, ly["bqkv"], prev["g2"], prev["b2n"])

    def _pack(self):
        if self._packed is None:
            self._packed = {"layers": self._pack_layers(self._fold_layer)}
        return self._packed

    def _workbufs(self, B: int, Lq: int) -> dict:
        key = (B, Lq)
        if key not in self._bufs:
            dev, M, H = self.device, B * Lq, self.hidden
            bf, f32 = dict(dtype=torch.bfloat16, device=dev), dict(dtype=torch.float32, device=dev)
            self._bufs[key] = {"xb": torch.empty(M, H, **bf), "xf": torch.empty(M, H, **f32), "y": torch.empty(M, H, **f32),
                               "x1b": torch.empty(M, H, **bf), "x1f": torch.empty(M, H, **f32),
                               "qkv": torch.empty(M, 3 * H, **bf), "ctx": torch.empty(M, H, **bf),
                               "h": torch.empty(M, self.inter, **bf), "feat": torch.empty(B, H, **f32),
                               "cu": torch.zeros(B + 1, dtype=torch.int32, device=dev), "row_src": torch.zeros(M, dtype=torch.int32, device=dev),
                               "bins": torch.zeros(B, 8, dtype=torch.int32, device=dev), "nbins": torch.zeros(1, dtype=torch.int32, device=dev)}
            if Lq <= 128 and B <= TEXT_TILE_MAX_B:
                self._bufs[key].update({"tiles": torch.zeros((B + 1) // 2, TEXT_TILE_INTS, dtype=torch.int32, device=dev),
                                        "ntiles": torch.zeros(1, dtype=torch.int32, device=dev)})
            p1 = self._fold_parts(M)
            if p1:
                self._bufs[key].update({"y2": torch.empty(M, H, **f32), "y1b": torch.empty(M, H, **bf), "y2b": torch.empty(M, H, **bf),
                                        "st": torch.zeros(2 * self.layers, M, p1, 2, **f32)})
                self._guard_buf(dev)
        return self._bufs[key]

    def _check_length(self, Lq: int) -> None:
        if Lq > self.max_position:
            raise RuntimeError(f"sequence length {Lq} exceeds max_position_embeddings {self.max_position}")

    def _pass(self, input_ids: torch.Tensor, attention_mask: torch.Tensor, packed: bool, n_layers: Optional[int] = None, pool: bool = True,
              tail=None) -> dict:
        self._require_hip()
        dev = self.device
        B, Lq = input_ids.shape
        self._check_length(Lq)
        ids = input_ids.to(dev, torch.int64).contiguous()
        mask = attention_mask.to(dev, torch.int32).contiguous()
        p, b = self._pack(), self._workbufs(B, Lq)
        M = B * Lq
        fuse = self.fuse_qkv_attention and Lq == 128 and self.heads % 2 == 0
        cu = b["cu"] if packed else None
        live = _live_ptr(cu) if packed else None
        tiled = packed and fuse and self.text_sample_tiles and "tiles" in b and B * (self.heads // 2) >= self.text_tile_min_grid
        self._pack_embed(ids, mask, b, B, Lq, packed, fuse, tiled, live)
        layers = p["layers"] if n_layers is None else p["layers"][:max(1, int(n_layers))]
        ln_pool = pool and packed and "st" in b
        if tiled:
            attend = lambda A, W, bias, **fold: self._qkv_attn(A, W, bias, None, b["ctx"], B, Lq, self.heads, eps=self.eps, tiles=b["tiles"],
                                                               ntiles=b["ntiles"], **fold)
        elif fuse:
            bins, nbins = (b["bins"], b["nbins"]) if packed else (None, None)
            attend = lambda A, W, bias, **fold: self._qkv_attn(A, W, bias, mask, b["ctx"], B, Lq, self.heads, eps=self.eps, cu=cu, bins=bins,
                                                               nbins=nbins, **fold)
        elif packed:
            attend = self._two_launch(b, "ufnd_attention_bf16_varlen_masked", operands=(cu, mask), B=B, Lq=Lq, live=live)
        else:
            attend = self._two_launch(b, "ufnd_attention_bf16", operands=(mask,), B=B, Lq=Lq)
        tail = None if tail is None else tail(b, cu, B, Lq)
        if "st" in b:
            self._layers_folded(layers, b, attend, M, live, final_ln=not ln_pool, tail=tail)
        else:
            self._post_ln_layers(layers, b, attend, M, live, tail=tail)
        H, s = self.hidden, L.stream_ptr(dev)
        if ln_pool:
            L.check(L.lib().ufnd_ln_masked_meanpool_l2_live(b["y2"].data_ptr(), layers[-1]["g2"].data_ptr(), layers[-1]["b2n"].data_ptr(), self.eps,
                                                            mask.data_ptr(), b["cu"].data_ptr(), b["feat"].data_ptr(), B, Lq, H, s),
                    "ufnd_ln_masked_meanpool_l2_live")
        elif pool and packed:
            L.check(L.lib().ufnd_masked_meanpool_l2_live(b["xf"].data_ptr(), mask.data_ptr(), b["cu"].data_ptr(), b["feat"].data_ptr(), B, Lq, H, s),
                    "ufnd_masked_meanpool_l2_live")
        elif pool:
            L.check(L.lib().ufnd_masked_meanpool_l2(b["xf"].data_ptr(), mask.data_ptr(), b["feat"].data_ptr(), B, Lq, H, s), "ufnd_masked_meanpool_l2")
        return b

    def _pack_rows(self, mask, b, B: int, Lq: int, fuse: bool, tiled: bool) -> None:
        s = L.stream_ptr(self.device)
        cu = b["cu"]
        if tiled:
            L.check(L.lib().ufnd_text_pack_tiles(mask.data_ptr(), B, Lq, cu.data_ptr(), b["row_src"].data_ptr(), b["tiles"].data_ptr(),
                                                 b["ntiles"].data_ptr(), b["bins"].data_ptr(), b["nbins"].data_ptr(), s), "ufnd_text_pack_tiles")
        elif fuse:
            L.check(L.lib().ufnd_text_pack_bins(mask.data_ptr(), B, Lq, cu.data_ptr(), b["row_src"].data_ptr(), b["bins"].data_ptr(),
                                                b["nbins"].data_ptr(), s), "ufnd_text_pack_bins")
        else:
            L.check(L.lib().ufnd_text_pack(mask.data_ptr(), B, Lq, cu.data_ptr(), b["row_src"].data_ptr(), s), "ufnd_text_pack")

    def _embed_outs(self, b) -> tuple:
        return b["xb"].data_ptr(), None if ("st" in b and self.residual_dtype == "bf16") else b["xf"].data_ptr()

    def _pack_embed(self, ids, mask, b, B: int, Lq: int, packed: bool, fuse: bool, tiled: bool, live) -> None:
        w, H, s = self._w, self.hidden, L.stream_ptr(self.device)
        if packed:
            self._pack_rows(mask, b, B, Lq, fuse, tiled)
        tables = [w["embeddings." + n].data_ptr() for n in ("word_embeddings.weight", "position_embeddings.weight", "token_type_embeddings.weight",
                                                            "LayerNorm.weight", "LayerNorm.bias")]
        outs = self._embed_outs(b)
        if packed:
            L.check(L.lib().ufnd_bert_embed_live(ids.data_ptr(), b["row_src"].data_ptr(), live, *tables, *outs, B * Lq, Lq, H, self.vocab, self.eps, s),
                    "ufnd_bert_embed_live")
        else:
            L.check(L.lib().ufnd_bert_embed(ids.data_ptr(), *tables, *outs, B, Lq, H, self.vocab, self.eps, s), "ufnd_bert_embed")

    def _layers_folded(self, layers, b, attend, M: int, live=None, final_ln: bool = True, tail=None) -> None:
        H, eps = self.hidden, self.eps
        st = b["st"]
        rb = self.residual_dtype == "bf16"
        prev, r = None, b
        for i, ly in enumerate(layers):
            st1, st2 = st[2 * i], st[2 * i + 1]
            last = i == len(layers) - 1
            if prev is None:
                attend(b["xb"], ly["wqkv"], ly["bqkv"])
                res_b, res_f, stp, rg, rbeta = b["xb"], b["xf"], None, None, None
            else:
                stp = st[2 * i - 1]
                attend(b["y2b"], ly["wqkvf"], ly["bqkvf"], a_stats=stp, colsum=ly["csqkv"])
                res_b, res_f, rg, rbeta = b["y2b"], b["y2"], prev["g2"], prev["b2n"]
            if last and tail is not None:
                r = tail(res_b if rb else None, None if rb else res_f, stp)
                res_b, res_f, stp = r["rb"], r["rf"], (r["rst"] if stp is not None else None)
                st1, st2, M, live = r["st1"], r["st2"], r["y"].shape[0], None
            y1, y2 = r["y"], r["y2"]
            self._gemm_ln(r["ctx"], ly["wo"], ly["bo"], out_f32=None if rb else y1, out_bf16=r["y1b"], residual=None if rb else res_f,
                          residual_bf16=res_b if rb else None, r_stats=stp, r_gamma=rg, r_beta=rbeta, out_stats=st1,
                          eps=eps, which="out", m_live=live)
            self._gemm_ln(r["y1b"], ly["w1f"], ly["bif"], out_bf16=r["h"], act=ACT_GELU, a_stats=st1, colsum=ly["cs1"], eps=eps, which="ffn1",
                          m_live=live)
            self._gemm_ln(r["h"], ly["w2"], ly["b2"], out_f32=y2 if (last or not rb) else None, out_bf16=r["y2b"], residual=None if rb else y1,
                          residual_bf16=r["y1b"] if rb else None, r_stats=st1, r_gamma=ly["g1"], r_beta=ly["b1"], out_stats=st2, eps=eps,
                          which="ffn2", m_live=live)
            prev = ly
        if final_ln:
            self._ln(r["y2"], H, prev["g2"], prev["b2n"], None, r["xf"], M, H, eps, m_live=live)

    @torch.no_grad()
    def last_hidden_state(self, input_ids: torch.Tensor, attention_mask: torch.Tensor, n_layers: Optional[int] = None) -> torch.Tensor:
        b = self._pass(input_ids, attention_mask, packed=False, n_layers=n_layers, pool=False)
        return b["xf"].view(*input_ids.shape, self.hidden)

    @torch.no_grad()
    def forward(self, input_ids: torch.Tensor, attention_mask: torch.Tensor, unpad: bool = True, strict: bool = False) -> torch.Tensor:
        if strict:
            return self._strict(lambda: self.forward(input_ids, attention_mask, unpad=unpad))
        return self._pass(input_ids, attention_mask, packed=unpad)["feat"]

    encode_batch = forward

    @torch.no_grad()
    def encode_fields(self, input_ids: torch.Tensor, attention_mask: torch.Tensor, part_valid: torch.Tensor,
                      chunk: int = 1024, unpad: bool = True) -> torch.Tensor:
        self._require_hip()
        dev = self.device
        N, Mx, Lq = input_ids.shape
        valid = part_valid.to(dev, torch.int32).contiguous()
        ids = input_ids.to(dev, torch.int64).reshape(N * Mx, Lq)
        mask = attention_mask.to(dev, torch.int32).reshape(N * Mx, Lq)
        rows = torch.nonzero(valid.reshape(-1), as_tuple=False).flatten()
        parts = torch.zeros(N * Mx, self.hidden, dtype=torch.float32, device=dev)
        for s0 in range(0, rows.numel(), chunk):
            r = rows[s0:s0 + chunk]
            parts[r] = self.forward(ids[r], mask[r], unpad=unpad, strict=True)
        out = torch.empty(N, self.hidden, dtype=torch.float32, device=dev)
        L.check(L.lib().ufnd_field_mean_l2(parts.data_ptr(), valid.data_ptr(), out.data_ptr(), N, Mx, self.hidden,
                                           L.stream_ptr(dev)), "ufnd_field_mean_l2")
        return out


class ClipVisualEncoder(_EncoderBase):
    LAYER_PREFIX, LAYER_NAMES = "vision_model.encoder.layers.{}.", _CLIP_LAYER

    def __init__(self, layers: int = 12, hidden: int = 768, heads: int = 12, intermediate: int = 3072, patch: int = 32,
                 image: int = 224, projection_dim: int = 512, eps: float = 1e-5, fold_ln: bool = True, residual_dtype: str = "bf16",
                 attention_dropout: float = 0.0):
        super().__init__(hidden, heads, fold_ln, residual_dtype)
        self.attention_dropout = dropout_prob("attention_dropout", attention_dropout)
        self.layers, self.inter = layers, intermediate
        self.patch, self.image, self.proj, self.eps = patch, image, projection_dim, eps
        self.n_patches = (image // patch) ** 2
        self.fuse_qkv_attention = True
        self.cls_tail = True
        w, V, init = self._w, "vision_model.", self._seeded_init()
        w[V + "embeddings.class_embedding"] = init((hidden,))
        w[V + "embeddings.patch_embedding.weight"] = init((hidden, 3, patch, patch))
        w[V + "embeddings.position_embedding.weight"] = init((self.n_patches + 1, hidden))
        w[V + "pre_layrnorm.weight"], w[V + "pre_layrnorm.bias"] = torch.ones(hidden), torch.zeros(hidden)
        for i in range(layers):
            P = V + f"encoder.layers.{i}."
            for n in ("k_proj", "v_proj", "q_proj", "out_proj"):
                w[P + f"self_attn.{n}.weight"] = init((hidden, hidden))
                w[P + f"self_attn.{n}.bias"] = torch.zeros(hidden)
            w[P + "layer_norm1.weight"], w[P + "layer_norm1.bias"] = torch.ones(hidden), torch.zeros(hidden)
            w[P + "mlp.fc1.weight"], w[P + "mlp.fc1.bias"] = init((intermediate, hidden)), torch.zeros(intermediate)
            w[P + "mlp.fc2.weight"], w[P + "mlp.fc2.bias"] = init((hidden, intermediate)), torch.zeros(hidden)
            w[P + "layer_norm2.weight"], w[P + "layer_norm2.bias"] = torch.ones(hidden), torch.zeros(hidden)
        w[V + "post_layernorm.weight"], w[V + "post_layernorm.bias"] = torch.ones(hidden), torch.zeros(hidden)
        w["visual_projection.weight"] = init((projection_dim, hidden))

    def _fold_layer(self, layers, wq, w1) -> None:
        ly = layers[-1]
        ly["wqkvf"], ly["csqkv"], ly["bqkvf"] = self._fold(wq, ly["bqkv"], ly["g1"], ly["b1"])
        ly["w1f"], ly["cs1"], ly["bif"] = self._fold(w1, ly["bi"], ly["g2"], ly["b2n"])

    def _pack(self):
        if self._packed is None:
            w = self._w
            self._packed = {"layers": self._pack_layers(self._fold_layer),
                            "wpatch": _bf16(w["vision_model.embeddings.patch_embedding.weight"].reshape(self.hidden, -1)),
                            "wproj": _bf16(w["visual_projection.weight"])}
        return self._packed

    def _workbufs(self, B: int, Fr: int) -> dict:
        key = (B, Fr)
        if key not in self._bufs:
            dev, H, N = self.device, self.hidden, B * Fr
            T = self.n_patches + 1
            M = N * T
            bf, f32 = dict(dtype=torch.bfloat16, device=dev), dict(dtype=torch.float32, device=dev)
            self._bufs[key] = {"patches": torch.empty(N * self.n_patches, 3 * self.patch ** 2, **bf),
                               "pe": torch.empty(N * self.n_patches, H, **f32), "xf": torch.empty(M, H, **f32),
                               "hb": torch.empty(M, H, **bf), "qkv": torch.empty(M, 3 * H, **bf),
                               "ctx": torch.empty(M, H, **bf), "m": torch.empty(M, self.inter, **bf),
                               "pooled": torch.empty(N, H, **bf), "e": torch.empty(N, self.proj, **f32),
                               "feat": torch.empty(B, self.proj, **f32)}
            p1 = self._fold_parts(M)
            if p1:
                self._bufs[key].update({"st0": torch.zeros(M, 2, 2, **f32), "st": torch.zeros(2 * self.layers, M, p1, 2, **f32),
                                        "stc": torch.zeros(2, N, p1, 2, **f32)})
                self._guard_buf(dev)
            else:
                self._bufs[key]["hc"] = torch.empty(N, H, **bf)
        return self._bufs[key]

    @torch.no_grad()
    def image_embeds(self, frames: torch.Tensor) -> torch.Tensor:
        return self._run(frames[:, None], cls_tail=self.cls_tail)[0]

    @torch.no_grad()
    def hidden_state(self, frames: torch.Tensor, n_layers: Optional[int] = None) -> torch.Tensor:
        if frames.dim() == 4:
            frames = frames[:, None]
        _, b = self._run(frames, n_layers)
        N = frames.shape[0] * frames.shape[1]
        return b["xf"].view(N, self.n_patches + 1, self.hidden)

    def _embed(self, fr, p, b, N) -> None:
        w, V, s = self._w, "vision_model.", L.stream_ptr(self.device)
        L.check(L.lib().ufnd_vit_patchify(fr.data_ptr(), b["patches"].data_ptr(), N, self.image, self.patch, s), "ufnd_vit_patchify")
        self._gemm(b["patches"], p["wpatch"], None, out_f32=b["pe"])
        L.check(L.lib().ufnd_vit_assemble(b["pe"].data_ptr(), w[V + "embeddings.class_embedding"].data_ptr(),
                                          w[V + "embeddings.position_embedding.weight"].data_ptr(),
                                          w[V + "pre_layrnorm.weight"].data_ptr(), w[V + "pre_layrnorm.bias"].data_ptr(),
                                          None if ("st0" in b and self.residual_dtype == "bf16") else b["xf"].data_ptr(),
                                          L.ptr(b["hb"]) if "st0" in b else None, L.ptr(b.get("st0")),
                                          N, self.n_patches, self.hidden, self.eps, s), "ufnd_vit_assemble")

    def _cls_rows(self, b, N) -> dict:
        T = self.n_patches + 1
        r = {k: b[k].view(N, T * self.hidden)[:, :self.hidden] for k in ("ctx", "hb", "xf")}
        r["m"] = b["m"][:N]
        if "stc" in b:
            r["st1"], r["st2"] = b["stc"][0], b["stc"][1]
        else:
            r["hb"] = b["hc"]
        return r

    def _blocks_folded(self, layers, b, attend, tail=None) -> None:
        eps, stA, st = self.eps, b["st0"], b["st"]
        rb = self.residual_dtype == "bf16"
        for i, ly in enumerate(layers):
            st1, st2 = st[2 * i], st[2 * i + 1]
            last = i == len(layers) - 1
            attend(b["hb"], ly["wqkvf"], ly["bqkvf"], a_stats=stA, colsum=ly["csqkv"])
            r = b
            if last and tail is not None:
                r = tail()
                st1, st2 = r["st1"], r["st2"]
            self._gemm_ln(r["ctx"], ly["wo"], ly["bo"], out_f32=None if rb else r["xf"], out_bf16=r["hb"], residual=None if rb else r["xf"],
                          residual_bf16=r["hb"] if rb else None, out_stats=st1, eps=eps, which="out")
            self._gemm_ln(r["hb"], ly["w1f"], ly["bif"], out_bf16=r["m"], act=ACT_QUICK_GELU, a_stats=st1, colsum=ly["cs1"], eps=eps, which="ffn1")
            self._gemm_ln(r["m"], ly["w2"], ly["b2"], out_f32=r["xf"] if (last or not rb) else None, out_bf16=r["hb"],
                          residual=None if rb else r["xf"], residual_bf16=r["hb"] if rb else None, out_stats=st2, eps=eps, which="ffn2")
            stA = st2

    def _pooled_projection(self, p, b, N) -> None:
        w, V, H = self._w, "vision_model.", self.hidden
        self._ln(b["xf"], (self.n_patches + 1) * H, w[V + "post_layernorm.weight"], w[V + "post_layernorm.bias"], b["pooled"], None, N, H, self.eps)
        self._gemm(b["pooled"], p["wproj"], None, out_f32=b["e"])

    def _run(self, frames5: torch.Tensor, n_layers: Optional[int] = None, cls_tail: bool = False):
        self._require_hip()
        B, Fr = frames5.shape[:2]
        if tuple(frames5.shape[2:]) != (3, self.image, self.image):
            raise RuntimeError(f"frames: expected (B,F,3,{self.image},{self.image}), got {tuple(frames5.shape)}")
        fr = L.f32c(frames5.to(self.device)).view(B * Fr, 3, self.image, self.image)
        p, b = self._pack(), self._workbufs(B, Fr)
        layers = p["layers"] if n_layers is None else p["layers"][:max(1, int(n_layers))]
        N, T = B * Fr, self.n_patches + 1
        self._embed(fr, p, b, N)
        if self.fuse_qkv_attention and T <= 64:
            attend = lambda A, W, bias, **fold: self._qkv_attn(A, W, bias, None, b["ctx"], N, T, self.heads, eps=self.eps, **fold)
        else:
            attend = self._two_launch(b, "ufnd_attention_bf16", operands=(None,), B=N, Lq=T)
        tail = (lambda: self._cls_rows(b, N)) if cls_tail else None
        if "st0" in b:
            self._blocks_folded(layers, b, attend, tail)
        else:
            self._pre_ln_blocks(layers, b, attend, N * T, ACT_QUICK_GELU, tail=tail)
        self._pooled_projection(p, b, N)
        return b["e"], b

    @torch.no_grad()
    def forward(self, frames: torch.Tensor, strict: bool = False) -> torch.Tensor:
        if frames.dim() == 4:
            frames = frames[:, None]
        if strict:
            return self._strict(lambda: self.forward(frames))
        B, Fr = frames.shape[:2]
        e, b = self._run(frames, cls_tail=self.cls_tail)
        L.check(L.lib().ufnd_l2norm_frames(e.data_ptr(), b["feat"].data_ptr(), B, Fr, self.proj, L.stream_ptr(self.device)),
                "ufnd_l2norm_frames")
        return b["feat"]
```

Measured before the change: 30540.

## Process two attention heads per workgroup in fused QKV-attention kernels

Adds a head-pair mode to the one-head fused QKV+attention kernels (ViT and text tiles). Each workgroup loops over two heads, reusing the already-loaded row tiles, LN stats and key bias, and reissues the weight and activation loads for the second head. The host picks pairing when the one-head grid exceeds the CU count, halving the grid to cut workgroup launch and tail-wave overhead. In exchange, per-workgroup serial work doubles and register pressure rises from the goto-based loop, which could hurt occupancy or load balance.

```diff
diff --git a/include/ultrafnd_hip.h b/include/ultrafnd_hip.h
--- a/include/ultrafnd_hip.h
+++ b/include/ultrafnd_hip.h
@@ -224,9 +224,13 @@
                          int32_t* bins, int32_t* nbins, void* stream);
 int ufnd_qkv_attention_bf16_tiles(const void* X, const void* Wqkv, const float* bqkv, const int32_t* tiles, const int32_t* ntiles, void* ctx,
                                   int cap_tiles, int heads, int ldx, int ldw, const ufnd_gemm_ln* ln, void* stream);
+int ufnd_qkv_attention_bf16_tiles_hp(const void* X, const void* Wqkv, const float* bqkv, const int32_t* tiles, const int32_t* ntiles, void* ctx,
+                                     int cap_tiles, int heads, int heads_per_wg, int ldx, int ldw, const ufnd_gemm_ln* ln, void* stream);
 
 int ufnd_qkv_attention_bf16_vit(const void* X, const void* Wqkv, const float* bqkv, void* ctx, int N, int T, int heads, int ldx, int ldw,
                                 const ufnd_gemm_ln* ln, void* stream);
+int ufnd_qkv_attention_bf16_vit_hp(const void* X, const void* Wqkv, const float* bqkv, void* ctx, int N, int T, int heads, int heads_per_wg,
+                                   int ldx, int ldw, const ufnd_gemm_ln* ln, void* stream);
 int ufnd_layernorm_live(const float* x, int ldx, const float* gamma, const float* beta, void* out_bf16, float* out_f32, int capacity,
                         int H, float eps, const int* m_live, void* stream);
 int ufnd_masked_meanpool_l2_live(const float* hidden, const int32_t* mask, const int32_t* cu_seqlens, float* out, int B, int L, int H,
diff --git a/ultrafnd_git_amd/_lib.py b/ultrafnd_git_amd/_lib.py
--- a/ultrafnd_git_amd/_lib.py
+++ b/ultrafnd_git_amd/_lib.py
@@ -176,6 +176,8 @@
         "ufnd_qkv_attention_bf16_bins": [P] * 8 + [I, I, I, I, I, C.POINTER(GemmLn), P],
         "ufnd_qkv_attention_bf16_tiles": [P] * 6 + [I, I, I, I, C.POINTER(GemmLn), P],
         "ufnd_qkv_attention_bf16_vit": [P, P, P, P, I, I, I, I, I, C.POINTER(GemmLn), P],
+        "ufnd_qkv_attention_bf16_tiles_hp": [P] * 6 + [I, I, I, I, I, C.POINTER(GemmLn), P],
+        "ufnd_qkv_attention_bf16_vit_hp": [P, P, P, P, I, I, I, I, I, I, C.POINTER(GemmLn), P],
         "ufnd_attention_bf16_varlen_masked": [P, P, P, P, I, I, I, P],
         "ufnd_layernorm_live": [P, I, P, P, P, P, I, I, F, P, P],
         "ufnd_masked_meanpool_l2_live": [P, P, P, P, I, I, I, P],
diff --git a/ultrafnd_git_amd/csrc/diag/gemm_diag.hip b/ultrafnd_git_amd/csrc/diag/gemm_diag.hip
--- a/ultrafnd_git_amd/csrc/diag/gemm_diag.hip
+++ b/ultrafnd_git_amd/csrc/diag/gemm_diag.hip
@@ -65,10 +65,11 @@
   return UFND_OK;
 }
 
-extern "C" int ufnd_diag_qkv_attention_tiles_stamps(const void* X, const void* Wqkv, const float* bqkv, const int32_t* tiles, const int32_t* ntiles,
-                                                    void* ctx, int cap_tiles, int heads, const ufnd_gemm_ln* ln, unsigned long long* stamps,
-                                                    void* stream_) {
+extern "C" int ufnd_diag_qkv_attention_tiles_hp_stamps(const void* X, const void* Wqkv, const float* bqkv, const int32_t* tiles, const int32_t* ntiles,
+                                                       void* ctx, int cap_tiles, int heads, int heads_per_wg, const ufnd_gemm_ln* ln,
+                                                       unsigned long long* stamps, void* stream_) {
   UFND_REQUIRE(X && Wqkv && ctx && stamps && tiles && ntiles && cap_tiles >= 1 && heads >= 1, "diag qkv_attention_tiles: bad argument");
+  UFND_REQUIRE(heads_per_wg == 1 || (heads_per_wg == 2 && heads % 2 == 0), "diag qkv_attention_tiles: heads=%d heads_per_wg=%d", heads, heads_per_wg);
   const int H = heads * 64;
   GemmArgs a{(const __bf16*)X, (const __bf16*)Wqkv, bqkv, nullptr, nullptr, nullptr, cap_tiles * 256, 3 * H, H, H, H, 0, 0, 0, UFND_ACT_NONE, 0, 0, stamps};
   if (ln && ln->a_stats) {
@@ -82,11 +83,19 @@
   a.att_h = H;
   a.att_scale_log2e = 0.125f * 1.44269504088896340736f;
   a.m_tiles = cap_tiles;
-  a.n_tiles = heads;
+  a.n_tiles = heads / heads_per_wg;
   a.xcd_cols = 1;
-  hipLaunchKernelGGL((gemm_bf16_kernel<256, 192, 4, 2, 3, 2, 16, 0, 1, 1, 2>), dim3(a.m_tiles * a.n_tiles), dim3(512), 0, (hipStream_t)stream_, a);
+  const dim3 grid(a.m_tiles * a.n_tiles);
+  if (heads_per_wg == 2) hipLaunchKernelGGL((gemm_bf16_kernel<256, 192, 4, 2, 3, 2, 16, 0, 1, 1, 2 + 4>), grid, dim3(512), 0, (hipStream_t)stream_, a);
+  else hipLaunchKernelGGL((gemm_bf16_kernel<256, 192, 4, 2, 3, 2, 16, 0, 1, 1, 2>), grid, dim3(512), 0, (hipStream_t)stream_, a);
   UFND_CHECK_LAUNCH();
   return UFND_OK;
+}
+
+extern "C" int ufnd_diag_qkv_attention_tiles_stamps(const void* X, const void* Wqkv, const float* bqkv, const int32_t* tiles, const int32_t* ntiles,
+                                                    void* ctx, int cap_tiles, int heads, const ufnd_gemm_ln* ln, unsigned long long* stamps,
+                                                    void* stream_) {
+  return ufnd_diag_qkv_attention_tiles_hp_stamps(X, Wqkv, bqkv, tiles, ntiles, ctx, cap_tiles, heads, 1, ln, stamps, stream_);
 }
 
 int ufnd_diag_pp_shape_ok(int M, int N, int K);
diff --git a/ultrafnd_git_amd/csrc/gemm_bf16.hip b/ultrafnd_git_amd/csrc/gemm_bf16.hip
--- a/ultrafnd_git_amd/csrc/gemm_bf16.hip
+++ b/ultrafnd_git_amd/csrc/gemm_bf16.hip
@@ -170,40 +170,66 @@
   return ufnd_qkv_attention_bf16_packed(X, Wqkv, bqkv, key_mask, nullptr, ctx, B, L, heads, ldx, ldw, ln, stream_);
 }
 
-extern "C" int ufnd_qkv_attention_bf16_tiles(const void* X, const void* Wqkv, const float* bqkv, const int32_t* tiles, const int32_t* ntiles,
-                                             void* ctx, int cap_tiles, int heads, int ldx, int ldw, const ufnd_gemm_ln* ln, void* stream_) {
+static int qkv_attention_head_tiles(const char* name, int heads, int heads_per_wg, int* n_tiles) {
+  UFND_REQUIRE(heads_per_wg == 1 || heads_per_wg == 2, "%s: heads_per_wg=%d (1 or 2)", name, heads_per_wg);
+  UFND_REQUIRE(heads_per_wg == 1 || heads % 2 == 0, "%s: heads=%d is odd: head pairs (heads_per_wg = 2) need an even head count", name, heads);
+  *n_tiles = heads / heads_per_wg;
+  return UFND_OK;
+}
+
+extern "C" int ufnd_qkv_attention_bf16_tiles_hp(const void* X, const void* Wqkv, const float* bqkv, const int32_t* tiles, const int32_t* ntiles,
+                                                void* ctx, int cap_tiles, int heads, int heads_per_wg, int ldx, int ldw, const ufnd_gemm_ln* ln,
+                                                void* stream_) {
   UFND_REQUIRE(X && Wqkv && ctx && tiles && ntiles, "qkv_attention_tiles: null operand");
   UFND_REQUIRE(heads >= 1 && heads <= 64 && cap_tiles >= 1 && cap_tiles <= (UFND_TEXT_TILE_MAX_B + 1) / 2, "qkv_attention_tiles: cap_tiles=%d heads=%d",
                cap_tiles, heads);
   GemmArgs a;
-  const int rc = qkv_attention_args("qkv_attention_tiles", a, X, Wqkv, bqkv, ctx, cap_tiles * 256, heads, ldx, ldw, ln);
+  int rc = qkv_attention_head_tiles("qkv_attention_tiles", heads, heads_per_wg, &a.n_tiles), n_tiles = a.n_tiles;
+  if (rc != UFND_OK) return rc;
+  rc = qkv_attention_args("qkv_attention_tiles", a, X, Wqkv, bqkv, ctx, cap_tiles * 256, heads, ldx, ldw, ln);
   if (rc != UFND_OK) return rc;
   a.att_bins = tiles;
   a.att_nbins = ntiles;
   a.m_tiles = cap_tiles;
-  a.n_tiles = heads;
+  a.n_tiles = n_tiles;
   a.xcd_cols = 1;
-  hipLaunchKernelGGL((gemm_bf16_kernel<256, 192, 4, 2, 3, 2, 16, 0, 0, 1, 2>), dim3(a.m_tiles * a.n_tiles), dim3(512), 0, (hipStream_t)stream_, a);
-  UFND_CHECK_LAUNCH();
-  return UFND_OK;
-}
-
-extern "C" int ufnd_qkv_attention_bf16_vit(const void* X, const void* Wqkv, const float* bqkv, void* ctx, int N, int T, int heads, int ldx,
-                                           int ldw, const ufnd_gemm_ln* ln, void* stream_) {
+  const dim3 grid(a.m_tiles * a.n_tiles);
+  if (heads_per_wg == 2) hipLaunchKernelGGL((gemm_bf16_kernel<256, 192, 4, 2, 3, 2, 16, 0, 0, 1, 2 + 4>), grid, dim3(512), 0, (hipStream_t)stream_, a);
+  else hipLaunchKernelGGL((gemm_bf16_kernel<256, 192, 4, 2, 3, 2, 16, 0, 0, 1, 2>), grid, dim3(512), 0, (hipStream_t)stream_, a);
+  UFND_CHECK_LAUNCH();
+  return UFND_OK;
+}
+
+extern "C" int ufnd_qkv_attention_bf16_tiles(const void* X, const void* Wqkv, const float* bqkv, const int32_t* tiles, const int32_t* ntiles,
+                                             void* ctx, int cap_tiles, int heads, int ldx, int ldw, const ufnd_gemm_ln* ln, void* stream_) {
+  return ufnd_qkv_attention_bf16_tiles_hp(X, Wqkv, bqkv, tiles, ntiles, ctx, cap_tiles, heads, 1, ldx, ldw, ln, stream_);
+}
+
+extern "C" int ufnd_qkv_attention_bf16_vit_hp(const void* X, const void* Wqkv, const float* bqkv, void* ctx, int N, int T, int heads, int heads_per_wg,
+                                              int ldx, int ldw, const ufnd_gemm_ln* ln, void* stream_) {
   UFND_REQUIRE(X && Wqkv && ctx, "qkv_attention_vit: null operand");
   UFND_REQUIRE(T >= 1 && T <= 64, "qkv_attention_vit: T=%d (this kernel is built for samples of 1 to 64 rows; use ufnd_gemm_bf16[_ln] + "
                "ufnd_attention_bf16 otherwise)", T);
   UFND_REQUIRE(heads >= 1 && heads <= 64 && N >= 1 && (long long)N * T <= (1 << 24), "qkv_attention_vit: N=%d T=%d heads=%d", N, T, heads);
   GemmArgs a;
-  const int rc = qkv_attention_args("qkv_attention_vit", a, X, Wqkv, bqkv, ctx, N * T, heads, ldx, ldw, ln);
+  int rc = qkv_attention_head_tiles("qkv_attention_vit", heads, heads_per_wg, &a.n_tiles), n_tiles = a.n_tiles;
+  if (rc != UFND_OK) return rc;
+  rc = qkv_attention_args("qkv_attention_vit", a, X, Wqkv, bqkv, ctx, N * T, heads, ldx, ldw, ln);
   if (rc != UFND_OK) return rc;
   a.att_t = T;
   a.m_tiles = ufnd_cdiv(N, 256 / T);
-  a.n_tiles = heads;
+  a.n_tiles = n_tiles;
   a.xcd_cols = 1;
-  hipLaunchKernelGGL((gemm_bf16_kernel<256, 192, 4, 2, 3, 2, 16, 0, 0, 1, 1>), dim3(a.m_tiles * a.n_tiles), dim3(512), 0, (hipStream_t)stream_, a);
-  UFND_CHECK_LAUNCH();
-  return UFND_OK;
+  const dim3 grid(a.m_tiles * a.n_tiles);
+  if (heads_per_wg == 2) hipLaunchKernelGGL((gemm_bf16_kernel<256, 192, 4, 2, 3, 2, 16, 0, 0, 1, 1 + 4>), grid, dim3(512), 0, (hipStream_t)stream_, a);
+  else hipLaunchKernelGGL((gemm_bf16_kernel<256, 192, 4, 2, 3, 2, 16, 0, 0, 1, 1>), grid, dim3(512), 0, (hipStream_t)stream_, a);
+  UFND_CHECK_LAUNCH();
+  return UFND_OK;
+}
+
+extern "C" int ufnd_qkv_attention_bf16_vit(const void* X, const void* Wqkv, const float* bqkv, void* ctx, int N, int T, int heads, int ldx,
+                                           int ldw, const ufnd_gemm_ln* ln, void* stream_) {
+  return ufnd_qkv_attention_bf16_vit_hp(X, Wqkv, bqkv, ctx, N, T, heads, 1, ldx, ldw, ln, stream_);
 }
 
 extern "C" int ufnd_gemm_bf16(const void* A, const void* W, const float* bias, const float* residual, void* out_bf16,
diff --git a/ultrafnd_git_amd/csrc/gemm_bf16_kernel.hpp b/ultrafnd_git_amd/csrc/gemm_bf16_kernel.hpp
--- a/ultrafnd_git_amd/csrc/gemm_bf16_kernel.hpp
+++ b/ultrafnd_git_amd/csrc/gemm_bf16_kernel.hpp
@@ -84,9 +84,10 @@
   const int smem = (ring > cbytes ? ring : cbytes) + (LNX ? BM * 8 + 64 : 0);
   return (!ATT && smem <= 80 * 1024 ? 2 : 1) * WM * WN / 4;
 }
-template <int BM, int BN, int WM, int WN, int STA, int STB, int MI, int ABL = 0, int DBG = 0, int LNX = 0, int ATT = 0, int BWD = 0>
-__global__ __launch_bounds__(WM * WN * 64) __attribute__((amdgpu_waves_per_eu(gemm_waves_per_simd(BM, BN, WM, WN, STA, STB, MI, LNX, ATT))))
+template <int BM, int BN, int WM, int WN, int STA, int STB, int MI, int ABL = 0, int DBG = 0, int LNX = 0, int ATT_ = 0, int BWD = 0>
+__global__ __launch_bounds__(WM * WN * 64) __attribute__((amdgpu_waves_per_eu(gemm_waves_per_simd(BM, BN, WM, WN, STA, STB, MI, LNX, ATT_))))
 void gemm_bf16_kernel(const GemmArgs a) {
+  constexpr int ATT = ATT_ & 3, HP = (ATT_ & 4) ? 2 : 1;
   static_assert(!BWD || (!LNX && !ATT && !ABL && !DBG), "backward forms are plain kernels");
   static_assert(MI == 16 || MI == 32, "MFMA shape");
   static_assert(!ATT || (((BM == 128 && BN == 384 && ATT == 1) || (BM == 256 && BN == 192)) && MI == 16 && WM * WN == 8 && LNX == 1 && ATT <= 2),
@@ -94,6 +95,7 @@
   constexpr bool VIT = ATT == 1 && BM == 256;
   constexpr bool TIL = ATT == 2;
   constexpr bool ONEH = VIT || TIL;
+  static_assert(HP == 1 || (HP == 2 && ONEH), "head pairs: the one-head geometries only");
   using acc_t = typename std::conditional<MI == 16, f32x4, f32x16>::type;
   constexpr int AR = MI * MI / 64;
   constexpr int KQ = MI == 16 ? 1 : 2;
@@ -161,6 +163,7 @@
     tn = half * nh + (rem - tm * nh);
   }
   const int m0 = tm * BM, n0 = tn * BN;
+  int hd = tn * HP;
   int arow0 = m0, alen = BM;
   int srow[4] = {0, 0, 0, 0}, scnt[4] = {0, 0, 0, 0}, smeta[4] = {-1, -1, -1, -1};
   const bool slots = ATT == 1 && !VIT && a.att_bins != nullptr;
@@ -212,16 +215,20 @@
     }
     return tr < alen;
   };
-  const int wave = __builtin_amdgcn_readfirstlane(threadIdx.x >> 6), lane = threadIdx.x & 63;
-  const int wm = wave / WN, wn = wave % WN, fr = lane & (MI - 1), g = lane / MI;
+  const int wave = __builtin_amdgcn_readfirstlane(threadIdx.x >> 6);
+  int lane = threadIdx.x & 63;
+  const int wm = wave / WN, wn = wave % WN;
+  int fr = lane & (MI - 1), g = lane / MI;
 
   acc_t acc[MT][NT];
-#pragma unroll
-  for (int i = 0; i < MT; ++i)
-#pragma unroll
-    for (int j = 0; j < NT; ++j)
-#pragma unroll
-      for (int r = 0; r < AR; ++r) acc[i][j][r] = 0.f;
+  if constexpr (HP == 1) {
+#pragma unroll
+    for (int i = 0; i < MT; ++i)
+#pragma unroll
+      for (int j = 0; j < NT; ++j)
+#pragma unroll
+        for (int r = 0; r < AR; ++r) acc[i][j][r] = 0.f;
+  }
 
   int nk = a.K / BK, kbase = 0;
   if constexpr (BWD) {
@@ -231,7 +238,7 @@
       nk = nk - kslice * per < per ? nk - kslice * per : per;
     }
   }
-  const int prow = lane >> 3, ppos = lane & 7;
+  int prow = lane >> 3, ppos = lane & 7;
   int arow_att[ATT ? PWA : 1];
   if constexpr (ATT) {
 #pragma unroll
@@ -262,7 +269,7 @@
       const int c = ppos ^ ((r >> 1) & 7);
       int gr = n0 + r;
       gr = gr < a.N ? gr : a.N - 1;
-      if constexpr (ONEH) gr = (r >> 6) * a.att_h + tn * 64 + (r & 63);
+      if constexpr (ONEH) gr = (r >> 6) * a.att_h + hd * 64 + (r & 63);
       else if constexpr (ATT) gr = (r >> 7) * a.att_h + tn * 128 + (r & 127);
       dma16(a.W + (size_t)gr * a.ldw + k0 + c * 8, buf + p * 1024);
     }
@@ -292,7 +299,7 @@
     }
   }
   float til_kb = 0.0f;
-  if constexpr (TIL) {
+  if constexpr (TIL && HP == 1) {
     if (threadIdx.x < BM) til_kb = __int_as_float(til[UFND_TEXT_TILE_KBIAS + threadIdx.x]);
   }
   int att_mk = 1;
@@ -450,6 +457,31 @@
     }
   };
 
+  [[maybe_unused]] auto write_stamps = [&](size_t slot) {
+    if constexpr (DBG) {
+      asm volatile("s_waitcnt vmcnt(0)" ::: "memory");
+      stamp[6] = __builtin_amdgcn_s_memtime();
+      stamp[7] = __builtin_amdgcn_s_memrealtime();
+      if (threadIdx.x == 0) {
+        constexpr int NS = ATT ? 10 : 8;
+#pragma unroll
+        for (int i = 0; i < NS; ++i) a.stamps[slot * NS + i] = stamp[i];
+      }
+      stamp[0] = stamp[6];
+      stamp[1] = stamp[7];
+    }
+  };
+  [[maybe_unused]] int hh = 0;
+  [[maybe_unused]] int tid = threadIdx.x;
+next_head:
+  if constexpr (HP > 1) {
+#pragma unroll
+    for (int i = 0; i < MT; ++i)
+#pragma unroll
+      for (int j = 0; j < NT; ++j)
+#pragma unroll
+        for (int r = 0; r < AR; ++r) acc[i][j][r] = 0.f;
+  }
   if (STA <= nk) wait_vmcnt<PWA * (STA - 1) + PWB * (STB - 1)>();
   else wait_vmcnt<0>();
   __builtin_amdgcn_sched_barrier(0);
@@ -468,6 +500,14 @@
   __builtin_amdgcn_sched_barrier(0);
   __builtin_amdgcn_s_barrier();
   __builtin_amdgcn_sched_barrier(0);
+  if constexpr (HP > 1) {
+    asm volatile("" : "+v"(lane));
+    lane &= 63;
+    fr = lane & (MI - 1), g = lane / MI, tid = wave * 64 + lane;
+    if constexpr (TIL) {
+      if (hh == 0 && tid < BM) til_kb = __int_as_float(til[UFND_TEXT_TILE_KBIAS + tid]);
+    }
+  }
   if constexpr (DBG) {
     stamp[4] = __builtin_amdgcn_s_memtime();
     stamp[5] = __builtin_amdgcn_s_memrealtime();
@@ -476,7 +516,7 @@
   float bj[NT], csj[NT];
 #pragma unroll
   for (int j = 0; j < NT; ++j) { bj[j] = 0.f; csj[j] = 0.f; }
-  auto gcol = [&](int c) { return ONEH ? (c >> 6) * a.att_h + tn * 64 + (c & 63) : ATT ? (c >> 7) * a.att_h + tn * 128 + (c & 127) : n0 + c; };
+  auto gcol = [&](int c) { return ONEH ? (c >> 6) * a.att_h + hd * 64 + (c & 63) : ATT ? (c >> 7) * a.att_h + tn * 128 + (c & 127) : n0 + c; };
   if (a.bias) {
 #pragma unroll
     for (int j = 0; j < NT; ++j) bj[j] = a.bias[gcol(wn * TN + j * MI + fr)];
@@ -677,7 +717,7 @@
   if constexpr (VIT) {
     const int T = a.att_t;
     float* kbias = reinterpret_cast<float*>(smem + ATT_OFF + 3 * ATT_IMG);
-    if (threadIdx.x < 64) kbias[threadIdx.x] = (int)threadIdx.x < T ? 0.0f : -INFINITY;
+    if (tid < 64 && (HP == 1 || hh == 0)) kbias[tid] = tid < T ? 0.0f : -INFINITY;
     __syncthreads();
     const int g4 = lane >> 4, f16 = lane & 15;
     const char* qimg = smem + ATT_OFF;
@@ -703,14 +743,14 @@
       for (int qt = 0; qt < 2; ++qt) {
         const float inv = attn_finish(l_run[qt]);
         const int q = q0 + qt * 16 + f16;
-        if (q < T) attn_store_ctx(a.att_ctx + (size_t)(arow0 + r0 + q) * a.att_h + tn * 64 + 4 * g4, o, qt, inv);
+        if (q < T) attn_store_ctx(a.att_ctx + (size_t)(arow0 + r0 + q) * a.att_h + hd * 64 + 4 * g4, o, qt, inv);
       }
     }
   } else if constexpr (TIL) {
     constexpr float NEG_MASK = -3.0e38f;
     float* kbias = reinterpret_cast<float*>(smem + ATT_OFF + 3 * ATT_IMG);
     float* wbias = kbias + BM + wave * 128;
-    if (threadIdx.x < BM) kbias[threadIdx.x] = til_kb;
+    if (tid < BM && (HP == 1 || hh == 0)) kbias[tid] = til_kb;
     __syncthreads();
     const int g4 = lane >> 4, f16 = lane & 15;
     const char* qimg = smem + ATT_OFF;
@@ -756,7 +796,7 @@
       for (int qt = 0; qt < 2; ++qt) {
         const float inv = attn_finish(l_run[qt]);
         const int q = q0 + qt * 16 + f16;
-        if (q < n) attn_store_ctx(a.att_ctx + (size_t)(grow0 + q) * a.att_h + tn * 64 + 4 * g4, o, qt, inv);
+        if (q < n) attn_store_ctx(a.att_ctx + (size_t)(grow0 + q) * a.att_h + hd * 64 + 4 * g4, o, qt, inv);
       }
     }
   } else if constexpr (ATT) {
@@ -805,6 +845,29 @@
       if (q < wcnt) attn_store_ctx(a.att_ctx + (size_t)(wrow0 + q) * a.att_h + (tn * 2 + hh) * 64 + 4 * g4, o, qt, inv);
     }
   }
+  if constexpr (HP > 1) {
+    if constexpr (DBG) write_stamps((size_t)blockIdx.x * HP + hh);
+    if (hh + 1 < HP) {
+      asm volatile("s_waitcnt lgkmcnt(0)" ::: "memory");
+      __builtin_amdgcn_sched_barrier(0);
+      __builtin_amdgcn_s_barrier();
+      __builtin_amdgcn_sched_barrier(0);
+      ++hd;
+      asm volatile("" : "+v"(lane));
+      lane &= 63;
+      prow = lane >> 3, ppos = lane & 7, fr = lane & (MI - 1), g = lane / MI;
+#pragma unroll
+      for (int ii = 0; ii < PWA; ++ii) asm volatile("" : "+v"(arow_att[ii]));
+#pragma unroll
+      for (int s = 0; s < STA; ++s) {
+        const int ks = s < nk ? s : nk - 1;
+        if (s < STB) issueB(s, ks);
+        issueA(s, ks);
+      }
+      ++hh;
+      goto next_head;
+    }
+  }
   if constexpr (LNX) {
     if (a.guard && a.a_stats && threadIdx.x == 0) {
       const float* gw = reinterpret_cast<const float*>(smem + STAT_OFF + BM * 8);
@@ -814,16 +877,7 @@
       atomicMax(reinterpret_cast<int*>(a.guard + (blockIdx.x & 1023)), __float_as_int(worst));
     }
   }
-  if constexpr (DBG) {
-    asm volatile("s_waitcnt vmcnt(0)" ::: "memory");
-    stamp[6] = __builtin_amdgcn_s_memtime();
-    stamp[7] = __builtin_amdgcn_s_memrealtime();
-    if (threadIdx.x == 0) {
-      constexpr int NS = ATT ? 10 : 8;
-#pragma unroll
-      for (int i = 0; i < NS; ++i) a.stamps[(size_t)blockIdx.x * NS + i] = stamp[i];
-    }
-  }
+  if constexpr (DBG && HP == 1) write_stamps(blockIdx.x);
 }
 
 }
diff --git a/ultrafnd_git_amd/encoders.py b/ultrafnd_git_amd/encoders.py
--- a/ultrafnd_git_amd/encoders.py
+++ b/ultrafnd_git_amd/encoders.py
@@ -79,6 +79,15 @@
     return len(text_tiles(n_rows))
 
 
+def heads_per_workgroup(one_head_grid: int, heads: int, min_grid: int, exact: bool = False) -> int:
+    del heads
+    if one_head_grid < min_grid:
+        return 1
+    cus = max(1, min_grid - 1)
+    rounds = lambda g: -(-g // cus)
+    return 2 if not exact or 2 * rounds(-(-one_head_grid // 2)) <= rounds(one_head_grid) else 1
+
+
 class _EncoderBase(nn.Module):
 
     FOLD_GUARD_MAX = 4.0
@@ -91,6 +100,7 @@
             raise ValueError("head_dim must be 64 (hidden == heads * 64)")
         self.hidden, self.heads, self.fold_ln, self.residual_dtype = hidden, heads, fold_ln, residual_dtype
         self.tiles: Dict[str, int] = {}
+        self.head_pair_min_grid: Optional[int] = None
         self._guard: Optional[torch.Tensor] = None
         self._w: "OrderedDict[str, torch.Tensor]" = OrderedDict()
         self._packed: Optional[dict] = None
@@ -246,6 +256,11 @@
         L.check(L.lib().ufnd_layernorm(x.data_ptr(), ldx, gamma.data_ptr(), beta.data_ptr(), L.ptr(out_bf16),
                                        L.ptr(out_f32), M, H, eps, L.stream_ptr(x.device)), "ufnd_layernorm")
 
+    def _heads_per_wg(self, row_tiles: int, heads: int, exact: bool) -> int:
+        if self.head_pair_min_grid is None:
+            self.head_pair_min_grid = L.lib().ufnd_device_cu_count() + 1
+        return heads_per_workgroup(row_tiles * heads, heads, self.head_pair_min_grid, exact)
+
     def _qkv_attn(self, A, W, bias, mask_i32, ctx, B, Lq, heads, a_stats=None, colsum=None, eps=1e-5, cu=None, bins=None, nbins=None, tiles=None,
                   ntiles=None):
         ln = None
@@ -256,15 +271,17 @@
         if Lq <= 64:
             if mask_i32 is not None or cu is not None or bins is not None:
                 raise L.UltrafndHipError("_qkv_attn: the short-sample kernel (Lq <= 64) takes no key mask, cu or bins")
-            L.check(L.lib().ufnd_qkv_attention_bf16_vit(A.data_ptr(), W.data_ptr(), L.ptr(bias), ctx.data_ptr(), B, Lq, heads, A.stride(0),
-                                                        W.stride(0), ctypes.byref(ln) if ln is not None else None, L.stream_ptr(A.device)),
-                    "ufnd_qkv_attention_bf16_vit")
+            hp = self._heads_per_wg(-(-B // (256 // Lq)), heads, exact=True)
+            L.check(L.lib().ufnd_qkv_attention_bf16_vit_hp(A.data_ptr(), W.data_ptr(), L.ptr(bias), ctx.data_ptr(), B, Lq, heads, hp, A.stride(0),
+                                                           W.stride(0), ctypes.byref(ln) if ln is not None else None, L.stream_ptr(A.device)),
+                    "ufnd_qkv_attention_bf16_vit_hp")
             return
         if tiles is not None:
-            L.check(L.lib().ufnd_qkv_attention_bf16_tiles(A.data_ptr(), W.data_ptr(), L.ptr(bias), tiles.data_ptr(), ntiles.data_ptr(), ctx.data_ptr(),
-                                                          tiles.shape[0], heads, A.stride(0), W.stride(0),
-                                                          ctypes.byref(ln) if ln is not None else None, L.stream_ptr(A.device)),
-                    "ufnd_qkv_attention_bf16_tiles")
+            hp = self._heads_per_wg(tiles.shape[0], heads, exact=False)
+            L.check(L.lib().ufnd_qkv_attention_bf16_tiles_hp(A.data_ptr(), W.data_ptr(), L.ptr(bias), tiles.data_ptr(), ntiles.data_ptr(),
+                                                             ctx.data_ptr(), tiles.shape[0], heads, hp, A.stride(0), W.stride(0),
+                                                             ctypes.byref(ln) if ln is not None else None, L.stream_ptr(A.device)),
+                    "ufnd_qkv_attention_bf16_tiles_hp")
             return
         L.check(L.lib().ufnd_qkv_attention_bf16_bins(A.data_ptr(), W.data_ptr(), L.ptr(bias), L.ptr(mask_i32), L.ptr(cu), L.ptr(bins),
                                                      L.ptr(nbins), ctx.data_ptr(), B, Lq, heads, A.stride(0), W.stride(0),
```

After: 30730 (median of 6 runs). About the same (+0.6%).
